# franciszzj/OpenPSG

Hardware: AMD Instinct MI355X
Metric: object-pairs/sec (relation-query + LMM decode), 1024² img × 50 masks (higher is better)
Workload: dtype fp32; 1 GPU; C3: 1024x1024, 50 masks, full path incl. LMM autoregressive relation decode (Llama-2-7B shape, top-20 pairs, 16 new tokens each, EOS suppressed); objects=50, pairs_per_image=2450, patches=256, llm_layers=32, mode=fp32s

## Files before the change

### include/psg_hip.h

```cpp
#ifndef PSG_HIP_H
#define PSG_HIP_H

#include <stdint.h>

#ifdef __cplusplus
extern "C" {
#endif

typedef struct psg_ctx psg_ctx;

enum psg_status {
  PSG_OK = 0,
  PSG_ERR_INVALID = -1,
  PSG_ERR_UNSUPPORTED = -2,
  PSG_ERR_HIP = -3,
  PSG_ERR_NO_DEVICE = -4
};

enum psg_dtype { PSG_F32 = 0, PSG_BF16 = 1, PSG_F16 = 2 };

enum psg_empty_policy { PSG_EMPTY_UNIFORM = 0, PSG_EMPTY_UNMASKED = 1 };

enum psg_xattn_variant { PSG_XATTN_MFMA = 0, PSG_XATTN_SIMPLE = 1, PSG_XATTN_MFMA_V1 = 2 };

#define PSG_ABI_VERSION 609
int psg_version(void);
const char* psg_last_error(void);
int psg_create(int device, psg_ctx** out);
int psg_destroy(psg_ctx* ctx);
int psg_device_info(psg_ctx* ctx, int* num_cu, char* arch, int arch_len);

int psg_set_option(psg_ctx* ctx, const char* name, int value);
int psg_get_option(psg_ctx* ctx, const char* name, int* value);

enum psg_trace_kind { PSG_TRACE_NONE = 0, PSG_TRACE_SKINNY_GEMM = 1, PSG_TRACE_CROSS_ATTN = 2, PSG_TRACE_DECODE_LAYER = 3 };
int psg_set_trace_buffer(psg_ctx* ctx, int kind, void* device_buffer, int64_t bytes);

int psg_patch_embed_workspace(psg_ctx*, int C, int Hf, int Wf, int Cout, int patch, int64_t* bytes);
int psg_patch_embed(psg_ctx*, const float* feat, int C, int Hf, int Wf, const float* weight,
                    const float* bias, int Cout, int patch, float* out, float* workspace,
                    int64_t workspace_bytes, void* stream);

int psg_mask_grid(psg_ctx*, const int32_t* pan, int H0, int W0, int img_h, int img_w,
                  int pad_h, int pad_w, int gh, int gw, float* grid, void* stream);

int psg_object_bitmasks(psg_ctx*, const float* grid, int L, const int32_t* object_ids, int N,
                        uint64_t* bits, int words, void* stream);

int psg_qformer_embed(psg_ctx*, const int32_t* ids, int B, int T, const float* word_emb,
                      const float* pos_emb, const float* query_rows, int nq, const float* ln_w,
                      const float* ln_b, float eps, int hidden, void* out, int dtype, void* stream);

int psg_add_layernorm(psg_ctx*, const void* x, const void* residual, const float* bias,
                      const float* gamma, const float* beta, float eps, int64_t rows, int hidden,
                      void* out, int dtype, void* stream);
int psg_add_layernorm_periodic(psg_ctx*, const void* x, const void* residual_table, int table_rows,
                               const float* bias, const float* gamma, const float* beta, float eps,
                               int64_t rows, int hidden, void* out, int dtype, void* stream);
int psg_add_layernorm_indexed(psg_ctx*, const void* x, const void* residual_table, const int32_t* block_index, int group,
                              const float* bias, const float* gamma, const float* beta, float eps, int64_t rows,
                              int hidden, void* out, int dtype, void* stream);
int psg_add_layernorm_res32(psg_ctx*, const void* x, const float* residual, int res_period, const int32_t* res_index,
                            const float* bias, const float* gamma, const float* beta, float eps, int64_t rows,
                            int hidden, void* out16, float* out32, int dtype, void* stream);

int psg_bias_gelu(psg_ctx*, const void* x, const float* bias, int64_t rows, int cols, void* out,
                  int dtype, void* stream);

int psg_qformer_self_attn(psg_ctx*, const void* qkv, const uint8_t* text_mask, int B, int T, int nq,
                          int heads, int query_rows_only, void* out, int dtype, void* stream);

int psg_qformer_self_attn_shared(psg_ctx*, const void* qkv_query, const void* qkv_text,
                                 const uint8_t* text_mask, int B, int T, int nq, int heads, void* out,
                                 int dtype, void* stream);
int psg_qformer_self_attn_cls(psg_ctx*, const void* q_cls, const void* kv, const uint8_t* text_mask, int B, int T,
                              int nq, int heads, void* out, int dtype, void* stream);
int psg_qformer_cls_attn_input(psg_ctx*, const void* x_query, const void* x_text, const int32_t* text_index,
                               const void* g, const uint8_t* text_mask, int B, int T, int nq, int heads, int hidden,
                               void* xbar, int dtype, void* stream);

int psg_qformer_cross_attn(psg_ctx*, const void* q, const void* k, const void* v,
                           const uint64_t* bits, int words, const int32_t* pair_index, int N, int P,
                           int L, int nq, int heads, int empty_policy, int variant, void* out,
                           int dtype, void* stream);
int psg_qformer_cross_attn_indexed(psg_ctx*, const void* q_u, const int32_t* q_index, const void* q_cls, const void* k,
                                   const void* v, const uint64_t* bits, int words, const int32_t* pair_index, int N, int P,
                                   int L, int heads, int empty_policy, void* out, int dtype, void* stream);

int psg_exist_head(psg_ctx*, const void* x, const float* w, const float* b, int P, int nq, int hidden,
                   float* logit, float* prob, int dtype, void* stream);

int psg_topk(psg_ctx*, const float* score, int n, int k, int32_t* out_idx, float* out_val, void* stream);

int psg_multiclass_head(psg_ctx*, const void* x, const float* w, const float* b, int P, int nq, int hidden, int R,
                        const int32_t* pair_index, int N, float* logit, float* prob, int dtype, void* stream);

int psg_topk_large_workspace(psg_ctx*, int n, int k, int64_t* bytes);
int psg_topk_large(psg_ctx*, const float* score, int n, int k, void* workspace, int64_t ws_bytes, int32_t* out_idx,
                   float* out_val, void* stream);

int psg_gather_rows(psg_ctx*, const void* src, int src_dtype, const int32_t* idx, int64_t n, int cols,
                    int64_t src_row_stride, void* dst, int dst_dtype, int64_t dst_row_stride, void* stream);
int psg_gather_pair_rows(psg_ctx*, const void* xq, const void* xt, const int32_t* text_index, const uint8_t* text_mask,
                         const int32_t* pair_index, const int32_t* sel, int K, int first, int count, int slot_off,
                         int nq, int T, int cols, void* out, uint8_t* mask_out, int32_t* pair_out, uint8_t* mine_out,
                         int dtype, void* stream);

int psg_rmsnorm(psg_ctx*, void* resid, const void* delta, int delta_splits, const float* w, float eps,
                int64_t rows, int hidden, void* out, int dtype, int resid_dtype, void* stream);

int psg_rope_kvwrite(psg_ctx*, const void* qkv, int qkv_splits, const int32_t* tok_pair, const int32_t* tok_pos,
                     const int32_t* rope_pos, const float* rope_cos, const float* rope_sin, int64_t rows, int heads,
                     int head_dim, int ctx, void* q_out, void* k_cache, void* v_cache, int dtype, void* stream);

int psg_llm_attn(psg_ctx*, const void* q, const void* k_cache, const void* v_cache,
                 const int32_t* tok_pair, const int32_t* tok_pos, int64_t rows, int heads,
                 int head_dim, int ctx, void* out, int dtype, void* stream);

int psg_prefill_attn(psg_ctx*, const void* q, const void* k_cache, const void* v_cache,
                     const int32_t* tok_pos, int pairs, int rows_per_pair, int heads, int head_dim,
                     int ctx, void* out, int dtype, void* stream);

int psg_prefill_attn_rope(psg_ctx*, const void* qkv, const int32_t* tok_pos, const float* rope_cos,
                          const float* rope_sin, int pairs, int rows_per_pair, int heads, int head_dim,
                          int ctx, void* k_cache, void* v_cache, void* out, int dtype, void* stream);

int psg_decode_attn(psg_ctx*, const void* qkv, int qkv_splits, const int32_t* tok_pair, const int32_t* tok_pos,
                    const float* rope_cos, const float* rope_sin, int rows, int heads, int head_dim, int ctx, void* k_cache,
                    void* v_cache, void* out, int dtype, void* stream);

int psg_rope_kvwrite_gqa(psg_ctx*, const void* qkv, int qkv_splits, const int32_t* tok_pair, const int32_t* tok_pos,
                         const int32_t* rope_pos, const float* rope_cos, const float* rope_sin, int64_t rows, int heads,
                         int kv_heads, int head_dim, int ctx, void* q_out, void* k_cache, void* v_cache, int dtype,
                         void* stream);
int psg_rope_kvwrite_scaled_gqa(psg_ctx*, const float* qkv, const float* row_scale, const float* col_scale,
                                const int32_t* tok_pair, const int32_t* tok_pos, const float* rope_cos,
                                const float* rope_sin, int slices, int64_t rows, int heads, int kv_heads, int head_dim,
                                int ctx, float* q_out, float* k_cache, float* v_cache, void* stream);
int psg_llm_attn_gqa(psg_ctx*, const void* q, const void* k_cache, const void* v_cache, const int32_t* tok_pair,
                     const int32_t* tok_pos, int64_t rows, int heads, int kv_heads, int head_dim, int ctx, void* out,
                     int dtype, void* stream);
int psg_prefill_attn_gqa(psg_ctx*, const void* q, const void* k_cache, const void* v_cache, const int32_t* tok_pos,
                         int pairs, int rows_per_pair, int heads, int kv_heads, int head_dim, int ctx, void* out, int dtype,
                         void* stream);
int psg_prefill_attn_rope_gqa(psg_ctx*, const void* qkv, const int32_t* tok_pos, const float* rope_cos,
                              const float* rope_sin, int pairs, int rows_per_pair, int heads, int kv_heads, int head_dim,
                              int ctx, void* k_cache, void* v_cache, void* out, int dtype, void* stream);
int psg_decode_attn_gqa(psg_ctx*, const void* qkv, int qkv_splits, const int32_t* tok_pair, const int32_t* tok_pos,
                        const float* rope_cos, const float* rope_sin, int rows, int heads, int kv_heads, int head_dim,
                        int ctx, void* k_cache, void* v_cache, void* out, int dtype, void* stream);

int psg_silu_mul(psg_ctx*, const void* gate_up, int splits, int64_t rows, int inter, void* out, int dtype,
                 void* stream);

int psg_skinny_gemm_plan(psg_ctx*, int M, int N, int K, int dtype, int* splits);
int psg_skinny_gemm(psg_ctx*, const void* x, const void* w, float* part, int M, int N, int K,
                    int splits, int dtype, void* stream);
int psg_reduce_partials(psg_ctx*, const float* part, int splits, int64_t n, void* y, int dtype,
                        void* stream);
int psg_split_f16x2(psg_ctx*, const float* x, int64_t rows, int K, int64_t row_stride, void* out2, float* inv_scale,
                    void* stream);
int psg_rmsnorm_split2(psg_ctx*, float* resid, const float* delta, int delta_splits, const float* w, float eps, int64_t rows,
                       int hidden, void* out2, float* inv_scale, void* stream);
int psg_split_gemm_w16_plan(psg_ctx*, int M, int N, int K, int mode, int* slots);
int psg_split_gemm_w16(psg_ctx*, const void* x2, const float* inv_scale, const void* w_f16, float* part, int M, int N, int K,
                       int slots, int mode, void* stream);
int psg_split_gemm_w8_plan(psg_ctx*, int M, int N, int K, int mode, int* slots);
int psg_split_gemm_w8(psg_ctx*, const void* x2, const float* inv_scale, const void* w8, const float* col_scale, float* part,
                      int M, int N, int K, int slots, int mode, void* stream);
int psg_skinny_gemm_w8_plan(psg_ctx*, int M, int N, int K, int dtype, int mode, int* slots);
int psg_skinny_gemm_w8(psg_ctx*, const void* x, const void* w8, const float* col_scale, float* part, int M, int N, int K,
                       int slots, int dtype, int mode, void* stream);
int psg_split_gemm_w4_plan(psg_ctx*, int M, int N, int K, int mode, int* slots);
int psg_split_gemm_w4(psg_ctx*, const void* x2, const float* inv_scale, const void* w4, const void* e_img, const float* col_scale,
                      float* part, int M, int N, int K, int slots, int mode, void* stream);
int psg_skinny_gemm_w4_plan(psg_ctx*, int M, int N, int K, int dtype, int mode, int* slots);
int psg_skinny_gemm_w4(psg_ctx*, const void* x, const void* w4, const void* e_img, const float* col_scale, float* part, int M,
                       int N, int K, int slots, int dtype, int mode, void* stream);
int psg_split_gemm_int4_plan(psg_ctx*, int M, int N, int K, int group, int mode, int* slots);
int psg_split_gemm_int4(psg_ctx*, const void* x2, const float* inv_scale, const void* q_img, const void* g_img, float* part,
                        int M, int N, int K, int group, int slots, int mode, void* stream);
int psg_skinny_gemm_int4_plan(psg_ctx*, int M, int N, int K, int group, int dtype, int mode, int* slots);
int psg_skinny_gemm_int4(psg_ctx*, const void* x, const void* q_img, const void* g_img, float* part, int M, int N, int K,
                         int group, int slots, int dtype, int mode, void* stream);
int psg_batch_gemm_w8_plan(psg_ctx*, int M, int N, int K, int dtype, int mode, int* slots);
int psg_batch_gemm_w8(psg_ctx*, const void* x, const void* w8, const float* col_scale, float* part, int M, int N, int K,
                      int slots, int dtype, int mode, void* stream);
int psg_batch_split_gemm_w8_plan(psg_ctx*, int M, int N, int K, int mode, int* slots);
int psg_batch_split_gemm_w8(psg_ctx*, const void* x2, const float* inv_scale, const void* w8, const float* col_scale,
                            float* part, int M, int N, int K, int slots, int mode, void* stream);
int psg_batch_gemm_w4_plan(psg_ctx*, int M, int N, int K, int dtype, int mode, int* slots);
int psg_batch_gemm_w4(psg_ctx*, const void* x, const void* w4, const void* e_img, const float* col_scale, float* part, int M,
                      int N, int K, int slots, int dtype, int mode, void* stream);
int psg_batch_split_gemm_w4_plan(psg_ctx*, int M, int N, int K, int mode, int* slots);
int psg_batch_split_gemm_w4(psg_ctx*, const void* x2, const float* inv_scale, const void* w4, const void* e_img,
                            const float* col_scale, float* part, int M, int N, int K, int slots, int mode, void* stream);
int psg_expand_w8(psg_ctx*, const void* q, const float* s, void* out, int N, int K, int out_dtype, void* stream);
int psg_expand_w4(psg_ctx*, const void* q, const void* e, const float* s, void* out, int N, int K, int out_dtype, void* stream);
int psg_skinny_gemm_w16(psg_ctx*, const float* x, const void* w_f16, float* part, int M, int N, int K, int splits,
                        void* stream);

int psg_batch_gemm_plan(psg_ctx*, int64_t M, int N, int K, int dtype, int slab_rows, int mode, int* slots);
int psg_batch_gemm(psg_ctx*, const void* x, const void* w, float* part, int64_t M, int N, int K, int slots, int dtype,
                   int slab_rows, int mode, void* stream);

enum psg_prologue_kind { PSG_PRO_NONE = 0, PSG_PRO_RMSNORM = 1, PSG_PRO_DECODE_ATTN = 2, PSG_PRO_SILU_MUL = 3 };
typedef struct psg_prologue {
  int kind;
  int in_splits;
  const void* in;
  void* resid;
  const float* norm_w;
  float eps;
  int heads;
  int ctx;
  const int32_t* tok_pair;
  const int32_t* tok_pos;
  const float* rope_cos;
  const float* rope_sin;
  void* k_cache;
  void* v_cache;
  uint32_t* sync;
} psg_prologue;
int psg_skinny_gemm_fused(psg_ctx*, const psg_prologue* pro, void* x, const void* w, float* part, int M, int N, int K,
                          int splits, int dtype, void* stream);

int psg_decode_layer_workspace(psg_ctx*, int M, int hidden, int inter, int64_t* floats, int64_t* counters);
int psg_decode_layer_supported(psg_ctx*, int M, int hidden, int inter, int heads, int dtype);
int psg_decode_layer(psg_ctx*, void* resid, const void* delta, int delta_splits, const float* ln1, const float* ln2,
                     const void* wqkv, const void* wo, const void* wgu, const void* wdown, const int32_t* tok_pair,
                     const int32_t* tok_pos, const float* rope_cos, const float* rope_sin, int M, int hidden, int inter,
                     int heads, int ctx_len, float eps, void* k_cache, void* v_cache, float* workspace, uint32_t* counters,
                     float* down_part, int dtype, void* stream);
int psg_decode_layers(psg_ctx*, void* resid, const void* delta, int delta_splits, const void* layer_table, int n_layers,
                      const int32_t* tok_pair, const int32_t* tok_pos, const float* rope_cos, const float* rope_sin, int M,
                      int hidden, int inter, int heads, int ctx_len, float eps, float* workspace, uint32_t* counters,
                      float* down_parts, int dtype, void* stream);

int psg_split_f16x3(psg_ctx*, const float* x, int64_t rows, int K, int64_t row_stride, int order, void* out,
                    float* inv_scale, void* stream);
int psg_scale_rows_cols(psg_ctx*, float* y, int64_t rows, int N, const float* row_scale, const float* col_scale,
                        void* stream);

int psg_rmsnorm_split(psg_ctx*, float* resid, const float* delta, const float* delta_row_scale, const float* delta_col_scale,
                      int delta_slices, const float* w, float eps, int64_t rows, int hidden, void* out, float* inv_scale,
                      int planes, void* stream);
int psg_rope_kvwrite_scaled(psg_ctx*, const float* qkv, const float* row_scale, const float* col_scale,
                            const int32_t* tok_pair, const int32_t* tok_pos, const float* rope_cos, const float* rope_sin,
                            int slices, int64_t rows, int heads, int head_dim, int ctx, float* q_out, float* k_cache,
                            float* v_cache, void* stream);
int psg_silu_mul_split(psg_ctx*, const float* gate_up, const float* row_scale, const float* col_scale, int slices, int64_t rows,
                       int inter, void* out, float* inv_scale, int planes, void* stream);

enum psg_epilogue { PSG_EPI_NONE = 0, PSG_EPI_GELU = 1, PSG_EPI_SWIGLU = 2 };
int psg_dense_gemm(psg_ctx*, const void* x, const void* w, const float* bias, int epilogue, void* out, int64_t M,
                   int N, int K, int dtype, void* stream);
int psg_dense_gemm_ex(psg_ctx*, const void* x, const void* w, const float* bias, int epilogue, void* out, int64_t M,
                      int N, int K, int dtype, int out_dtype, const float* row_scale, const float* col_scale,
                      void* stream);
enum psg_tile { PSG_TILE_AUTO = 0, PSG_TILE_256x256 = 1, PSG_TILE_256x192 = 2, PSG_TILE_256x128 = 3, PSG_TILE_256x64 = 4,
                PSG_TILE_128x128 = 5 };
int psg_dense_gemm_tiled(psg_ctx*, const void* x, const void* w, const float* bias, int epilogue, void* out, int64_t M,
                         int N, int K, int dtype, int out_dtype, const float* row_scale, const float* col_scale, int tile,
                         void* stream);
int psg_interleave_gate_up(psg_ctx*, const void* gate_up, void* out, int inter, int K, void* stream);
int psg_dense_gemm_split(psg_ctx*, const void* x2, const void* w2, const float* bias, int epilogue, float* out, int64_t M,
                         int N, int K2, const float* row_scale, const float* col_scale, int tile, void* stream);

int psg_greedy_step(psg_ctx*, const void* logits, int splits, int K, int vocab, int step, int max_new,
                    int eos, int suppress_token, int32_t* tokens, int32_t* done, int32_t* next_ids, int32_t* tok_pos,
                    const void* embed, int embed_dtype, int hidden, void* x_out, int x_dtype, int dtype, void* stream);

int psg_tree_attn(psg_ctx*, const void* q, const void* k_cache, const void* v_cache, const int32_t* row_pair,
                  const int32_t* row_node, const int32_t* prefix_len, const int32_t* anc, int n_int, int max_depth,
                  int trie_base, int64_t rows, int heads, int kv_heads, int pairs, int head_dim, int ctx, void* out,
                  int dtype, void* stream);
int psg_token_logprobs(psg_ctx*, const void* logits, int splits, int64_t rows, int vocab, const int32_t* row_node,
                       const int64_t* row_out, const int32_t* child_off, const int32_t* child_tok, int n_nodes,
                       int n_edges, float* out, int64_t out_len, int dtype, void* stream);

int psg_masked_mean_pool_workspace(psg_ctx*, int C, int Hf, int Wf, int N, int64_t* bytes);
int psg_masked_mean_pool(psg_ctx*, const float* feat, int C, int Hf, int Wf, const int32_t* pan, int H0,
                         int W0, int img_h, int img_w, int pad_h, int pad_w, const int32_t* object_ids,
                         int N, float* out, int32_t* workspace, int64_t workspace_bytes, void* stream);
int psg_masked_split_mean_pool(psg_ctx*, const float* feat, int C, int Hf, int Wf, const int32_t* pan, int H0,
                               int W0, int img_h, int img_w, int pad_h, int pad_w, const int32_t* object_ids, int N,
                               int output_size, float* out, int32_t* workspace, int64_t workspace_bytes, void* stream);

int psg_train_object_bitmasks(psg_ctx*, const uint8_t* thing_masks, int n_thing, const int32_t* sem, int H, int W,
                              const int32_t* is_thing, const int32_t* category, const int32_t* thing_index, int N,
                              int gh, int gw, uint64_t* bits, int words, void* stream);
int psg_bce_with_logits(psg_ctx*, const float* logit, const float* label, int n, float weight, float* out,
                        void* stream);
int psg_cross_entropy_rows(psg_ctx*, const void* logits, int64_t rows, int vocab, const int32_t* labels, float* loss,
                           int dtype, void* stream);

int psg_train_layernorm_fwd(psg_ctx*, const float* x, const float* gamma, const float* beta, float eps, int64_t rows,
                            int hidden, float* y, float* mean, float* rstd, void* stream);
int psg_train_layernorm_bwd(psg_ctx*, const float* x, const float* dy, const float* gamma, const float* mean,
                            const float* rstd, int64_t rows, int hidden, float* dx, float* dgamma, float* dbeta,
                            void* stream);
int psg_train_rmsnorm_fwd(psg_ctx*, const float* x, const float* w, float eps, int64_t rows, int hidden, float* y,
                          float* rstd, void* stream);
int psg_train_rmsnorm_bwd(psg_ctx*, const float* x, const float* dy, const float* w, const float* rstd, int64_t rows,
                          int hidden, float* dx, void* stream);
int psg_train_attn_fwd(psg_ctx*, const float* q, const float* k, const float* v, const uint8_t* keep, int B, int Bk,
                       int H, int Sq, int Sk, int D, int Mq, float scale, const uint8_t* drop, float drop_scale, float* p,
                       float* out, void* stream);
int psg_train_attn_bwd(psg_ctx*, const float* q, const float* k, const float* v, const float* p, const float* dout,
                       int B, int Bk, int H, int Sq, int Sk, int D, float scale, const uint8_t* drop, float drop_scale,
                       float* dq, float* dk, float* dv, void* stream);
int psg_train_gelu_fwd(psg_ctx*, const float* x, int64_t n, float* y, void* stream);
int psg_train_gelu_bwd(psg_ctx*, const float* x, const float* dy, int64_t n, float* dx, void* stream);
int psg_train_silu_mul_fwd(psg_ctx*, const float* gate_up, int64_t rows, int inter, float* y, void* stream);
int psg_train_silu_mul_bwd(psg_ctx*, const float* gate_up, const float* dy, int64_t rows, int inter, float* dgate_up,
                           void* stream);
int psg_train_rope(psg_ctx*, const float* x, const int32_t* pos, const float* rope_cos, const float* rope_sin,
                   int table_rows, int64_t rows, int heads, int head_dim, float sign, float* y, void* stream);
int psg_train_ce_bwd(psg_ctx*, const float* logits, int64_t rows, int vocab, const int32_t* labels, const float* dloss,
                     float* dlogits, void* stream);
int psg_train_bce_bwd(psg_ctx*, const float* logit, const float* label, int n, float weight, const float* dloss,
                      float* dlogit, void* stream);
int psg_train_mlcce_fwd(psg_ctx*, const float* logits, const float* labels, int rows, int R, float* loss, void* stream);
int psg_train_mlcce_bwd(psg_ctx*, const float* logits, const float* labels, int rows, int R, const float* dloss,
                        float* dlogits, void* stream);

int psg_train_bf16_layernorm_fwd(psg_ctx*, const float* x, const float* gamma, const float* beta, float eps, int64_t rows,
                                 int hidden, void* y, float* mean, float* rstd, void* stream);
int psg_train_bf16_layernorm_bwd(psg_ctx*, const float* x, const void* dy, const float* gamma, const float* mean,
                                 const float* rstd, int64_t rows, int hidden, float* dx, float* dgamma, float* dbeta,
                                 void* stream);
int psg_train_bf16_rmsnorm_fwd(psg_ctx*, const float* x, const float* w, float eps, int64_t rows, int hidden, void* y,
                               float* rstd, void* stream);
int psg_train_bf16_rmsnorm_bwd(psg_ctx*, const float* x, const void* dy, const float* w, const float* rstd, int64_t rows,
                               int hidden, float* dx, void* stream);
int psg_train_bf16_gelu_fwd(psg_ctx*, const void* x, int64_t n, void* y, void* stream);
int psg_train_bf16_gelu_bwd(psg_ctx*, const void* x, const void* dy, int64_t n, void* dx, void* stream);
int psg_train_bf16_silu_mul_fwd(psg_ctx*, const void* gate_up, int64_t rows, int inter, void* y, void* stream);
int psg_train_bf16_silu_mul_bwd(psg_ctx*, const void* gate_up, const void* dy, int64_t rows, int inter, void* dgate_up,
                                void* stream);
int psg_train_bf16_rope(psg_ctx*, const void* x, const int32_t* pos, const float* rope_cos, const float* rope_sin,
                        int table_rows, int64_t rows, int heads, int head_dim, float sign, void* y, void* stream);
int psg_train_bf16_attn_fwd(psg_ctx*, const void* q, const void* k, const void* v, const uint8_t* keep, int B, int Bk, int H,
                            int Sq, int Sk, int D, int Mq, float scale, const uint8_t* drop, float drop_scale, void* out,
                            float* lse, void* stream);
int psg_train_bf16_attn_bwd(psg_ctx*, const void* q, const void* k, const void* v, const uint8_t* keep, const void* dout,
                            const float* lse, int B, int Bk, int H, int Sq, int Sk, int D, int Mq, float scale,
                            const uint8_t* drop, float drop_scale, void* dq, void* dk, void* dv, float* delta, void* stream);

int psg_bilinear_scores(psg_ctx*, const float* sub, const float* obj, int B, int N, int R, int C, float* pred,
                        void* stream);

#ifdef __cplusplus
}
#endif
#endif
```

### openpsg_amd/_lib.py

```python
from __future__ import annotations

import ctypes as C
import os

_HERE = os.path.dirname(os.path.abspath(__file__))
LIB_PATH = os.path.join(_HERE, "libpsg_hip.so")

PSG_ABI_VERSION = 609
PSG_F32, PSG_BF16, PSG_F16 = 0, 1, 2
PSG_EMPTY_UNIFORM, PSG_EMPTY_UNMASKED = 0, 1
PSG_XATTN_MFMA, PSG_XATTN_SIMPLE, PSG_XATTN_MFMA_V1 = 0, 1, 2
PSG_TRACE_NONE, PSG_TRACE_SKINNY_GEMM, PSG_TRACE_CROSS_ATTN, PSG_TRACE_DECODE_LAYER = 0, 1, 2, 3


class PsgHipError(RuntimeError):
    pass


_vp, _i, _i64, _f = C.c_void_p, C.c_int, C.c_int64, C.c_float

PSG_PRO_NONE, PSG_PRO_RMSNORM, PSG_PRO_DECODE_ATTN, PSG_PRO_SILU_MUL = 0, 1, 2, 3


class Prologue(C.Structure):
    _fields_ = [("kind", _i), ("in_splits", _i), ("input", _vp), ("resid", _vp), ("norm_w", _vp), ("eps", _f),
                ("heads", _i), ("ctx", _i), ("tok_pair", _vp), ("tok_pos", _vp), ("rope_cos", _vp), ("rope_sin", _vp),
                ("k_cache", _vp), ("v_cache", _vp), ("sync", _vp)]

SIGNATURES = {
    "psg_version": [],
    "psg_create": [_i, C.POINTER(_vp)],
    "psg_destroy": [_vp],
    "psg_device_info": [_vp, C.POINTER(_i), C.c_char_p, _i],
    "psg_set_option": [_vp, C.c_char_p, _i],
    "psg_get_option": [_vp, C.c_char_p, C.POINTER(_i)],
    "psg_set_trace_buffer": [_vp, _i, _vp, _i64],
    "psg_patch_embed_workspace": [_vp, _i, _i, _i, _i, _i, C.POINTER(_i64)],
    "psg_patch_embed": [_vp, _vp, _i, _i, _i, _vp, _vp, _i, _i, _vp, _vp, _i64, _vp],
    "psg_mask_grid": [_vp, _vp, _i, _i, _i, _i, _i, _i, _i, _i, _vp, _vp],
    "psg_object_bitmasks": [_vp, _vp, _i, _vp, _i, _vp, _i, _vp],
    "psg_qformer_embed": [_vp, _vp, _i, _i, _vp, _vp, _vp, _i, _vp, _vp, _f, _i, _vp, _i, _vp],
    "psg_add_layernorm": [_vp, _vp, _vp, _vp, _vp, _vp, _f, _i64, _i, _vp, _i, _vp],
    "psg_add_layernorm_periodic": [_vp, _vp, _vp, _i, _vp, _vp, _vp, _f, _i64, _i, _vp, _i, _vp],
    "psg_add_layernorm_indexed": [_vp, _vp, _vp, _vp, _i, _vp, _vp, _vp, _f, _i64, _i, _vp, _i, _vp],
    "psg_add_layernorm_res32": [_vp, _vp, _vp, _i, _vp, _vp, _vp, _vp, _f, _i64, _i, _vp, _vp, _i, _vp],
    "psg_bias_gelu": [_vp, _vp, _vp, _i64, _i, _vp, _i, _vp],
    "psg_qformer_self_attn": [_vp, _vp, _vp, _i, _i, _i, _i, _i, _vp, _i, _vp],
    "psg_qformer_self_attn_cls": [_vp, _vp, _vp, _vp, _i, _i, _i, _i, _vp, _i, _vp],
    "psg_qformer_cls_attn_input": [_vp, _vp, _vp, _vp, _vp, _vp, _i, _i, _i, _i, _i, _vp, _i, _vp],
    "psg_qformer_self_attn_shared": [_vp, _vp, _vp, _vp, _i, _i, _i, _i, _vp, _i, _vp],
    "psg_qformer_cross_attn": [_vp, _vp, _vp, _vp, _vp, _i, _vp, _i, _i, _i, _i, _i, _i, _i, _vp, _i, _vp],
    "psg_exist_head": [_vp, _vp, _vp, _vp, _i, _i, _i, _vp, _vp, _i, _vp],
    "psg_topk": [_vp, _vp, _i, _i, _vp, _vp, _vp],
    "psg_multiclass_head": [_vp, _vp, _vp, _vp, _i, _i, _i, _i, _vp, _i, _vp, _vp, _i, _vp],
    "psg_topk_large_workspace": [_vp, _i, _i, C.POINTER(_i64)],
    "psg_topk_large": [_vp, _vp, _i, _i, _vp, _i64, _vp, _vp, _vp],
    "psg_gather_rows": [_vp, _vp, _i, _vp, _i64, _i, _i64, _vp, _i, _i64, _vp],
    "psg_gather_pair_rows": [_vp, _vp, _vp, _vp, _vp, _vp, _vp, _i, _i, _i, _i, _i, _i, _i, _vp, _vp, _vp, _vp, _i, _vp],
    "psg_rmsnorm": [_vp, _vp, _vp, _i, _vp, _f, _i64, _i, _vp, _i, _i, _vp],
    "psg_rope_kvwrite": [_vp, _vp, _i, _vp, _vp, _vp, _vp, _vp, _i64, _i, _i, _i, _vp, _vp, _vp, _i, _vp],
    "psg_train_object_bitmasks": [_vp, _vp, _i, _vp, _i, _i, _vp, _vp, _vp, _i, _i, _i, _vp, _i, _vp],
    "psg_bce_with_logits": [_vp, _vp, _vp, _i, _f, _vp, _vp],
    "psg_cross_entropy_rows": [_vp, _vp, _i64, _i, _vp, _vp, _i, _vp],
    "psg_llm_attn": [_vp, _vp, _vp, _vp, _vp, _vp, _i64, _i, _i, _i, _vp, _i, _vp],
    "psg_prefill_attn": [_vp, _vp, _vp, _vp, _vp, _i, _i, _i, _i, _i, _vp, _i, _vp],
    "psg_prefill_attn_rope": [_vp, _vp, _vp, _vp, _vp, _i, _i, _i, _i, _i, _vp, _vp, _vp, _i, _vp],
    "psg_decode_attn": [_vp, _vp, _i, _vp, _vp, _vp, _vp, _i, _i, _i, _i, _vp, _vp, _vp, _i, _vp],
    "psg_rope_kvwrite_gqa": [_vp, _vp, _i, _vp, _vp, _vp, _vp, _vp, _i64, _i, _i, _i, _i, _vp, _vp, _vp, _i, _vp],
    "psg_rope_kvwrite_scaled_gqa": [_vp, _vp, _vp, _vp, _vp, _vp, _vp, _vp, _i, _i64, _i, _i, _i, _i, _vp, _vp, _vp, _vp],
    "psg_llm_attn_gqa": [_vp, _vp, _vp, _vp, _vp, _vp, _i64, _i, _i, _i, _i, _vp, _i, _vp],
    "psg_prefill_attn_gqa": [_vp, _vp, _vp, _vp, _vp, _i, _i, _i, _i, _i, _i, _vp, _i, _vp],
    "psg_prefill_attn_rope_gqa": [_vp, _vp, _vp, _vp, _vp, _i, _i, _i, _i, _i, _i, _vp, _vp, _vp, _i, _vp],
    "psg_decode_attn_gqa": [_vp, _vp, _i, _vp, _vp, _vp, _vp, _i, _i, _i, _i, _i, _vp, _vp, _vp, _i, _vp],
    "psg_silu_mul": [_vp, _vp, _i, _i64, _i, _vp, _i, _vp],
    "psg_skinny_gemm_plan": [_vp, _i, _i, _i, _i, C.POINTER(_i)],
    "psg_skinny_gemm": [_vp, _vp, _vp, _vp, _i, _i, _i, _i, _i, _vp],
    "psg_batch_gemm_plan": [_vp, _i64, _i, _i, _i, _i, _i, C.POINTER(_i)],
    "psg_batch_gemm": [_vp, _vp, _vp, _vp, _i64, _i, _i, _i, _i, _i, _i, _vp],
    "psg_split_f16x2": [_vp, _vp, _i64, _i, _i64, _vp, _vp, _vp],
    "psg_rmsnorm_split2": [_vp, _vp, _vp, _i, _vp, _f, _i64, _i, _vp, _vp, _vp],
    "psg_split_gemm_w16_plan": [_vp, _i, _i, _i, _i, C.POINTER(_i)],
    "psg_split_gemm_w16": [_vp, _vp, _vp, _vp, _vp, _i, _i, _i, _i, _i, _vp],
    "psg_split_gemm_w8_plan": [_vp, _i, _i, _i, _i, C.POINTER(_i)],
    "psg_split_gemm_w8": [_vp, _vp, _vp, _vp, _vp, _vp, _i, _i, _i, _i, _i, _vp],
    "psg_skinny_gemm_w8_plan": [_vp, _i, _i, _i, _i, _i, C.POINTER(_i)],
    "psg_skinny_gemm_w8": [_vp, _vp, _vp, _vp, _vp, _i, _i, _i, _i, _i, _i, _vp],
    "psg_split_gemm_w4_plan": [_vp, _i, _i, _i, _i, C.POINTER(_i)],
    "psg_split_gemm_w4": [_vp, _vp, _vp, _vp, _vp, _vp, _vp, _i, _i, _i, _i, _i, _vp],
    "psg_skinny_gemm_w4_plan": [_vp, _i, _i, _i, _i, _i, C.POINTER(_i)],
    "psg_skinny_gemm_w4": [_vp, _vp, _vp, _vp, _vp, _vp, _i, _i, _i, _i, _i, _i, _vp],
    "psg_batch_gemm_w8_plan": [_vp, _i, _i, _i, _i, _i, C.POINTER(_i)],
    "psg_batch_gemm_w8": [_vp, _vp, _vp, _vp, _vp, _i, _i, _i, _i, _i, _i, _vp],
    "psg_batch_split_gemm_w8_plan": [_vp, _i, _i, _i, _i, C.POINTER(_i)],
    "psg_batch_split_gemm_w8": [_vp, _vp, _vp, _vp, _vp, _vp, _i, _i, _i, _i, _i, _vp],
    "psg_split_gemm_int4_plan": [_vp, _i, _i, _i, _i, _i, C.POINTER(_i)],
    "psg_split_gemm_int4": [_vp, _vp, _vp, _vp, _vp, _vp, _i, _i, _i, _i, _i, _i, _vp],
    "psg_skinny_gemm_int4_plan": [_vp, _i, _i, _i, _i, _i, _i, C.POINTER(_i)],
    "psg_skinny_gemm_int4": [_vp, _vp, _vp, _vp, _vp, _i, _i, _i, _i, _i, _i, _i, _vp],
    "psg_batch_gemm_w4_plan": [_vp, _i, _i, _i, _i, _i, C.POINTER(_i)],
    "psg_batch_gemm_w4": [_vp, _vp, _vp, _vp, _vp, _vp, _i, _i, _i, _i, _i, _i, _vp],
    "psg_batch_split_gemm_w4_plan": [_vp, _i, _i, _i, _i, C.POINTER(_i)],
    "psg_batch_split_gemm_w4": [_vp, _vp, _vp, _vp, _vp, _vp, _vp, _i, _i, _i, _i, _i, _vp],
    "psg_expand_w8": [_vp, _vp, _vp, _vp, _i, _i, _i, _vp],
    "psg_expand_w4": [_vp, _vp, _vp, _vp, _vp, _i, _i, _i, _vp],
    "psg_qformer_cross_attn_indexed": [_vp, _vp, _vp, _vp, _vp, _vp, _vp, _i, _vp, _i, _i, _i, _i, _i, _vp, _i, _vp],
    "psg_skinny_gemm_w16": [_vp, _vp, _vp, _vp, _i, _i, _i, _i, _vp],
    "psg_skinny_gemm_fused": [_vp, _vp, _vp, _vp, _vp, _i, _i, _i, _i, _i, _vp],
    "psg_rmsnorm_split": [_vp, _vp, _vp, _vp, _vp, _i, _vp, _f, _i64, _i, _vp, _vp, _i, _vp],
    "psg_rope_kvwrite_scaled": [_vp, _vp, _vp, _vp, _vp, _vp, _vp, _vp, _i, _i64, _i, _i, _i, _vp, _vp, _vp, _vp],
    "psg_silu_mul_split": [_vp, _vp, _vp, _vp, _i, _i64, _i, _vp, _vp, _i, _vp],
    "psg_decode_layer_workspace": [_vp, _i, _i, _i, C.POINTER(_i64), C.POINTER(_i64)],
    "psg_decode_layer_supported": [_vp, _i, _i, _i, _i, _i],
    "psg_decode_layers": [_vp, _vp, _vp, _i, _vp, _i, _vp, _vp, _vp, _vp, _i, _i, _i, _i, _i, _f, _vp, _vp, _vp, _i, _vp],
    "psg_decode_layer": [_vp, _vp, _vp, _i, _vp, _vp, _vp, _vp, _vp, _vp, _vp, _vp, _vp, _vp, _i, _i, _i, _i, _i, _f,
                         _vp, _vp, _vp, _vp, _vp, _i, _vp],
    "psg_reduce_partials": [_vp, _vp, _i, _i64, _vp, _i, _vp],
    "psg_masked_mean_pool_workspace": [_vp, _i, _i, _i, _i, C.POINTER(_i64)],
    "psg_masked_mean_pool": [_vp, _vp, _i, _i, _i, _vp, _i, _i, _i, _i, _i, _i, _vp, _i, _vp, _vp, _i64, _vp],
    "psg_masked_split_mean_pool": [_vp, _vp, _i, _i, _i, _vp, _i, _i, _i, _i, _i, _i, _vp, _i, _i, _vp, _vp, _i64, _vp],
    "psg_bilinear_scores": [_vp, _vp, _vp, _i, _i, _i, _i, _vp, _vp],
    "psg_dense_gemm": [_vp, _vp, _vp, _vp, _i, _vp, _i64, _i, _i, _i, _vp],
    "psg_dense_gemm_ex": [_vp, _vp, _vp, _vp, _i, _vp, _i64, _i, _i, _i, _i, _vp, _vp, _vp],
    "psg_dense_gemm_tiled": [_vp, _vp, _vp, _vp, _i, _vp, _i64, _i, _i, _i, _i, _vp, _vp, _i, _vp],
    "psg_interleave_gate_up": [_vp, _vp, _vp, _i, _i, _vp],
    "psg_dense_gemm_split": [_vp, _vp, _vp, _vp, _i, _vp, _i64, _i, _i, _vp, _vp, _i, _vp],
    "psg_train_layernorm_fwd": [_vp, _vp, _vp, _vp, _f, _i64, _i, _vp, _vp, _vp, _vp],
    "psg_train_layernorm_bwd": [_vp, _vp, _vp, _vp, _vp, _vp, _i64, _i, _vp, _vp, _vp, _vp],
    "psg_train_rmsnorm_fwd": [_vp, _vp, _vp, _f, _i64, _i, _vp, _vp, _vp],
    "psg_train_rmsnorm_bwd": [_vp, _vp, _vp, _vp, _vp, _i64, _i, _vp, _vp],
    "psg_split_f16x3": [_vp, _vp, _i64, _i, _i64, _i, _vp, _vp, _vp],
    "psg_scale_rows_cols": [_vp, _vp, _i64, _i, _vp, _vp, _vp],
    "psg_train_attn_fwd": [_vp, _vp, _vp, _vp, _vp, _i, _i, _i, _i, _i, _i, _i, _f, _vp, _f, _vp, _vp, _vp],
    "psg_train_attn_bwd": [_vp, _vp, _vp, _vp, _vp, _vp, _i, _i, _i, _i, _i, _i, _f, _vp, _f, _vp, _vp, _vp, _vp],
    "psg_train_gelu_fwd": [_vp, _vp, _i64, _vp, _vp],
    "psg_train_gelu_bwd": [_vp, _vp, _vp, _i64, _vp, _vp],
    "psg_train_silu_mul_fwd": [_vp, _vp, _i64, _i, _vp, _vp],
    "psg_train_silu_mul_bwd": [_vp, _vp, _vp, _i64, _i, _vp, _vp],
    "psg_train_rope": [_vp, _vp, _vp, _vp, _vp, _i, _i64, _i, _i, _f, _vp, _vp],
    "psg_train_ce_bwd": [_vp, _vp, _i64, _i, _vp, _vp, _vp, _vp],
    "psg_train_bce_bwd": [_vp, _vp, _vp, _i, _f, _vp, _vp, _vp],
    "psg_train_mlcce_fwd": [_vp, _vp, _vp, _i, _i, _vp, _vp],
    "psg_train_mlcce_bwd": [_vp, _vp, _vp, _i, _i, _vp, _vp, _vp],
    "psg_train_bf16_layernorm_fwd": [_vp, _vp, _vp, _vp, _f, _i64, _i, _vp, _vp, _vp, _vp],
    "psg_train_bf16_layernorm_bwd": [_vp, _vp, _vp, _vp, _vp, _vp, _i64, _i, _vp, _vp, _vp, _vp],
    "psg_train_bf16_rmsnorm_fwd": [_vp, _vp, _vp, _f, _i64, _i, _vp, _vp, _vp],
    "psg_train_bf16_rmsnorm_bwd": [_vp, _vp, _vp, _vp, _vp, _i64, _i, _vp, _vp],
    "psg_train_bf16_gelu_fwd": [_vp, _vp, _i64, _vp, _vp],
    "psg_train_bf16_gelu_bwd": [_vp, _vp, _vp, _i64, _vp, _vp],
    "psg_train_bf16_silu_mul_fwd": [_vp, _vp, _i64, _i, _vp, _vp],
    "psg_train_bf16_silu_mul_bwd": [_vp, _vp, _vp, _i64, _i, _vp, _vp],
    "psg_train_bf16_rope": [_vp, _vp, _vp, _vp, _vp, _i, _i64, _i, _i, _f, _vp, _vp],
    "psg_train_bf16_attn_fwd": [_vp, _vp, _vp, _vp, _vp, _i, _i, _i, _i, _i, _i, _i, _f, _vp, _f, _vp, _vp, _vp],
    "psg_train_bf16_attn_bwd": [_vp, _vp, _vp, _vp, _vp, _vp, _vp, _i, _i, _i, _i, _i, _i, _i, _f, _vp, _f, _vp, _vp, _vp,
                                _vp, _vp],
    "psg_greedy_step": [_vp, _vp, _i, _i, _i, _i, _i, _i, _i, _vp, _vp, _vp, _vp, _vp, _i, _i, _vp, _i, _i, _vp],
    "psg_tree_attn": [_vp, _vp, _vp, _vp, _vp, _vp, _vp, _vp, _i, _i, _i, _i64, _i, _i, _i, _i, _i, _vp, _i, _vp],
    "psg_token_logprobs": [_vp, _vp, _i, _i64, _i, _vp, _vp, _vp, _vp, _i, _i, _vp, _i64, _i, _vp],
}

_lib = None
_ctx = {}


def load():
    global _lib
    if _lib is not None:
        return _lib
    import torch
    if not os.path.exists(LIB_PATH):
        raise PsgHipError(
            f"{LIB_PATH} is missing: build it with `python -m openpsg_amd.csrc.build` "
            "(hipcc --offload-arch=gfx950). There is no CPU fallback for this path.")
    lib = C.CDLL(LIB_PATH)
    lib.psg_last_error.restype = C.c_char_p
    lib.psg_last_error.argtypes = []
    for name, argtypes in SIGNATURES.items():
        fn = getattr(lib, name, None)
        if fn is None:
            raise PsgHipError(f"{LIB_PATH} does not export {name}; rebuild the library")
        fn.restype = _i
        fn.argtypes = argtypes
    built = lib.psg_version()
    if built != PSG_ABI_VERSION:
        raise PsgHipError(f"{LIB_PATH} was built with ABI version {built}, this binding is written against "
                          f"{PSG_ABI_VERSION} (include/psg_hip.h): rebuild with `python -m openpsg_amd.csrc.build --force`")
    _lib = lib
    return lib


def last_error() -> str:
    return load().psg_last_error().decode("utf-8", "replace")


def check(rc: int, what: str):
    if rc != 0:
        raise PsgHipError(f"{what} failed (status {rc}): {last_error()}")


def ctx(device_index: int):
    if device_index not in _ctx:
        lib = load()
        h = _vp()
        check(lib.psg_create(int(device_index), C.byref(h)), "psg_create")
        _ctx[device_index] = h
    return _ctx[device_index]


def device_info(device_index: int):
    n = _i(0)
    buf = C.create_string_buffer(64)
    check(load().psg_device_info(ctx(device_index), C.byref(n), buf, 64), "psg_device_info")
    return n.value, buf.value.decode()


def set_option(device_index: int, name: str, value: int):
    check(load().psg_set_option(ctx(device_index), name.encode(), int(value)), f"psg_set_option({name})")


def get_option(device_index: int, name: str) -> int:
    v = _i(0)
    check(load().psg_get_option(ctx(device_index), name.encode(), C.byref(v)), f"psg_get_option({name})")
    return v.value


def set_trace_buffer(device_index: int, kind: int, tensor=None):
    if tensor is None or kind == PSG_TRACE_NONE:
        check(load().psg_set_trace_buffer(ctx(device_index), PSG_TRACE_NONE, None, 0), "psg_set_trace_buffer")
    else:
        check(load().psg_set_trace_buffer(ctx(device_index), int(kind), tensor.data_ptr(),
                                          tensor.numel() * tensor.element_size()), "psg_set_trace_buffer")
```

### openpsg_amd/csrc/build.py

```python
from __future__ import annotations

import argparse
import os
import subprocess
import sys

HERE = os.path.dirname(os.path.abspath(__file__))
PKG = os.path.dirname(HERE)
LIB = os.path.join(PKG, "libpsg_hip.so")
SOURCES = ["psg_core.hip", "psg_rowops.hip", "psg_attn.hip", "psg_attn_f32.hip", "psg_xattn_mfma.hip", "psg_xattn_dma.hip", "psg_gemm.hip", "psg_gemm_f32.hip", "psg_batch_gemm.hip", "psg_gemm_w8.hip", "psg_gemm_w4.hip", "psg_gemm_int4.hip", "psg_batch_gemm_q.hip", "psg_expand.hip", "psg_decode_layer.hip", "psg_split.hip", "psg_dense_gemm.hip", "psg_patch_embed.hip", "psg_selfattn_mfma.hip", "psg_prefill_attn_mfma.hip", "psg_pool.hip", "psg_train.hip", "psg_train_bwd.hip", "psg_train_bf16.hip", "psg_tree.hip"]
HEADERS = ["psg_common.h", "psg_wave.h", "psg_decode_math.h", "psg_train_rows.h", "psg_xattn_tile.h", os.path.join("..", "..", "include", "psg_hip.h")]


def _hipcc() -> str:
    for cand in (os.environ.get("HIPCC"), "/opt/rocm/bin/hipcc", "hipcc"):
        if cand and (os.path.isabs(cand) and os.path.exists(cand) or not os.path.isabs(cand)):
            return cand
    raise RuntimeError("hipcc not found")


def needs_build() -> bool:
    if not os.path.exists(LIB):
        return True
    t = os.path.getmtime(LIB)
    deps = [os.path.join(HERE, s) for s in SOURCES + HEADERS if os.path.exists(os.path.join(HERE, s))]
    return any(os.path.getmtime(d) > t for d in deps)


def build(force: bool = False, save_temps: bool = False, verbose: bool = True) -> str:
    if not force and not needs_build():
        return LIB
    from concurrent.futures import ThreadPoolExecutor
    obj_dir = os.path.join(HERE, "_obj")
    os.makedirs(obj_dir, exist_ok=True)
    flags = ["--offload-arch=gfx950", "-O3", "-std=c++17", "-fPIC", "-fno-gpu-rdc", "-Wno-unused-result"]
    if save_temps:
        os.makedirs(os.path.join(HERE, "_temps"), exist_ok=True)
        flags += ["-save-temps=obj", "-Rpass-analysis=kernel-resource-usage"]
    hdr_t = max(os.path.getmtime(os.path.join(HERE, h)) for h in HEADERS)
    jobs, objs = [], []
    for s in SOURCES:
        src = os.path.join(HERE, s)
        if not os.path.exists(src):
            continue
        obj = os.path.join(obj_dir, os.path.splitext(s)[0] + ".o")
        objs.append(obj)
        if force or save_temps or not os.path.exists(obj) or os.path.getmtime(obj) < max(os.path.getmtime(src), hdr_t):
            jobs.append([_hipcc()] + flags + ["-c", src, "-o", obj])

    def run(cmd):
        if verbose:
            print(" ".join(cmd), flush=True)
        subprocess.run(cmd, check=True, cwd=HERE)
    with ThreadPoolExecutor(max_workers=min(8, max(1, (os.cpu_count() or 2) - 1))) as ex:
        list(ex.map(run, jobs))
    run([_hipcc(), "--offload-arch=gfx950", "-shared", "-fPIC", "-fno-gpu-rdc", "-o", LIB] + objs)
    return LIB


if __name__ == "__main__":
    ap = argparse.ArgumentParser()
    ap.add_argument("--force", action="store_true")
    ap.add_argument("--save-temps", action="store_true")
    a = ap.parse_args()
    print(build(force=a.force, save_temps=a.save_temps))
```

### openpsg_amd/csrc/psg_core.hip

```cpp
#include <ctype.h>
#include <stdarg.h>
#include <stdlib.h>

#include "psg_common.h"

static thread_local char g_err[512] = "";

void psg_set_error(const char* fmt, ...) {
  va_list ap;
  va_start(ap, fmt);
  vsnprintf(g_err, sizeof(g_err), fmt, ap);
  va_end(ap);
}

extern "C" const char* psg_last_error(void) { return g_err; }
extern "C" int psg_version(void) { return PSG_ABI_VERSION; }

struct OptName {
  const char* name;
  int psg_opts::*field;
};
static const OptName kOpts[] = {
    {"skinny_splits", &psg_opts::skinny_splits},       {"skinny_balance", &psg_opts::skinny_balance},
    {"skinny_wg_per_cu", &psg_opts::skinny_wg_per_cu}, {"skinny_dma", &psg_opts::skinny_dma},
    {"skinny_nt", &psg_opts::skinny_nt},               {"skinny_xdma", &psg_opts::skinny_xdma},
    {"skinny_wide", &psg_opts::skinny_wide},           {"skinny_f32_slots", &psg_opts::skinny_f32_slots},
    {"skinny_f32_waves", &psg_opts::skinny_f32_waves}, {"decode_persistent", &psg_opts::decode_persistent},
    {"llm_fuse_split", &psg_opts::llm_fuse_split},
    {"split_i2", &psg_opts::split_i2},
    {"qformer_split_cls_input_space", &psg_opts::qformer_split_cls_input_space},
    {"wt_stores", &psg_opts::wt_stores},
    {"selfattn_scalar", &psg_opts::selfattn_scalar},   {"decode_attn_1wave", &psg_opts::decode_attn_1wave},
    {"xattn_dma", &psg_opts::xattn_dma},               {"xattn_waves", &psg_opts::xattn_waves},
    {"dense_gemm_var", &psg_opts::dense_gemm_var},     {"qformer_own_gemm", &psg_opts::qformer_own_gemm},
    {"ln_half_wave", &psg_opts::ln_half_wave},         {"xattn_poll", &psg_opts::xattn_poll},
    {"xattn_wt", &psg_opts::xattn_wt},
    {"xattn_dynamic", &psg_opts::xattn_dynamic},
    {"llm_w16", &psg_opts::llm_w16},                   {"decode_gqa_qparts", &psg_opts::decode_gqa_qparts},
    {"batch_gemm_bn", &psg_opts::batch_gemm_bn},       {"decode_batch_gemm", &psg_opts::decode_batch_gemm},
    {"batch_gemm_var", &psg_opts::batch_gemm_var},     {"batch_gemm_mode", &psg_opts::batch_gemm_mode},
    {"batch_gemm_grid", &psg_opts::batch_gemm_grid},
    {"qformer_share_qkv", &psg_opts::qformer_share_qkv},
    {"qformer_cls_input_space", &psg_opts::qformer_cls_input_space},
    {"qformer_dedup_prompts", &psg_opts::qformer_dedup_prompts},
    {"llm_fuse_rmsnorm", &psg_opts::llm_fuse_rmsnorm}, {"prefill_attn_scalar", &psg_opts::prefill_attn_scalar},
};

static int parse_opt(const char* name, const char* text) {
  int a = 0, b = 0, c = 3;
  if (!strcmp(name, "skinny_dma") && sscanf(text, "%dx%dx%d", &a, &b, &c) >= 2) return a * 100 + b * 10 + c;
  return atoi(text);
}

extern "C" int psg_set_option(psg_ctx* ctx, const char* name, int value) {
  PSG_REQUIRE(ctx && name, PSG_ERR_INVALID, "psg_set_option: NULL argument");
  for (const OptName& o : kOpts)
    if (!strcmp(o.name, name)) {
      ctx->opt.*(o.field) = value;
      return PSG_OK;
    }
  psg_set_error("psg_set_option: unknown option '%s'", name);
  return PSG_ERR_INVALID;
}

extern "C" int psg_get_option(psg_ctx* ctx, const char* name, int* value) {
  PSG_REQUIRE(ctx && name && value, PSG_ERR_INVALID, "psg_get_option: NULL argument");
  for (const OptName& o : kOpts)
    if (!strcmp(o.name, name)) {
      *value = ctx->opt.*(o.field);
      return PSG_OK;
    }
  psg_set_error("psg_get_option: unknown option '%s'", name);
  return PSG_ERR_INVALID;
}

extern "C" int psg_set_trace_buffer(psg_ctx* ctx, int kind, void* device_buffer, int64_t bytes) {
  PSG_REQUIRE(ctx, PSG_ERR_INVALID, "psg_set_trace_buffer: ctx is NULL");
  PSG_REQUIRE(kind == PSG_TRACE_NONE || (device_buffer && bytes >= 8), PSG_ERR_INVALID,
              "psg_set_trace_buffer: kind=%d needs a device buffer", kind);
  ctx->trace_kind = kind;
  ctx->trace = kind == PSG_TRACE_NONE ? nullptr : (long long*)device_buffer;
  ctx->trace_words = kind == PSG_TRACE_NONE ? 0 : bytes / 8;
  return PSG_OK;
}

extern "C" int psg_create(int device, psg_ctx** out) {
  PSG_REQUIRE(out != nullptr, PSG_ERR_INVALID, "psg_create: out is NULL");
  int n = 0;
  hipError_t e = hipGetDeviceCount(&n);
  if (e != hipSuccess || n <= 0) {
    psg_set_error("psg_create: no HIP device visible (%s)", e == hipSuccess ? "count=0" : hipGetErrorString(e));
    return PSG_ERR_NO_DEVICE;
  }
  PSG_REQUIRE(device >= 0 && device < n, PSG_ERR_INVALID, "psg_create: device %d out of range [0,%d)", device, n);
  hipDeviceProp_t prop;
  e = hipGetDeviceProperties(&prop, device);
  if (e != hipSuccess) {
    psg_set_error("psg_create: hipGetDeviceProperties: %s", hipGetErrorString(e));
    return PSG_ERR_HIP;
  }
  psg_ctx* c = new psg_ctx();
  for (const OptName& o : kOpts) {
    std::string env = "PSG_";
    for (const char* q = o.name; *q; ++q) env += (char)toupper(*q);
    if (const char* e = getenv(env.c_str())) c->opt.*(o.field) = parse_opt(o.name, e);
  }
  c->device = device;
  c->num_cu = prop.multiProcessorCount;
  strncpy(c->arch, prop.gcnArchName, sizeof(c->arch) - 1);
  c->arch[sizeof(c->arch) - 1] = 0;
  *out = c;
  return PSG_OK;
}

extern "C" int psg_destroy(psg_ctx* ctx) {
  delete ctx;
  return PSG_OK;
}

extern "C" int psg_device_info(psg_ctx* ctx, int* num_cu, char* arch, int arch_len) {
  PSG_REQUIRE(ctx != nullptr, PSG_ERR_INVALID, "psg_device_info: ctx is NULL");
  if (num_cu) *num_cu = ctx->num_cu;
  if (arch && arch_len > 0) {
    strncpy(arch, ctx->arch, arch_len - 1);
    arch[arch_len - 1] = 0;
  }
  return PSG_OK;
}

__global__ void mask_grid_kernel(const int32_t* __restrict__ pan, int H0, int W0, int img_h, int img_w,
                                 int pad_h, int pad_w, int gh, int gw, float* __restrict__ grid) {
  int idx = blockIdx.x * blockDim.x + threadIdx.x;
  if (idx >= gh * gw) return;
  int r = idx / gw, c = idx % gw;
  const float sy2 = (float)pad_h / (float)gh, sx2 = (float)pad_w / (float)gw;
  const float sy1 = (float)H0 / (float)img_h, sx1 = (float)W0 / (float)img_w;
  int y1 = min((int)floorf((float)r * sy2), pad_h - 1);
  int x1 = min((int)floorf((float)c * sx2), pad_w - 1);
  float v = 0.0f;
  if (y1 < img_h && x1 < img_w) {
    int y0 = min((int)floorf((float)y1 * sy1), H0 - 1);
    int x0 = min((int)floorf((float)x1 * sx1), W0 - 1);
    v = (float)pan[(int64_t)y0 * W0 + x0];
  }
  grid[idx] = v;
}

extern "C" int psg_mask_grid(psg_ctx* ctx, const int32_t* pan, int H0, int W0, int img_h, int img_w, int pad_h,
                             int pad_w, int gh, int gw, float* grid, void* stream) {
  PSG_REQUIRE(ctx && pan && grid, PSG_ERR_INVALID, "psg_mask_grid: NULL argument");
  PSG_REQUIRE(H0 > 0 && W0 > 0 && img_h > 0 && img_w > 0 && pad_h >= img_h && pad_w >= img_w && gh > 0 && gw > 0,
              PSG_ERR_INVALID, "psg_mask_grid: bad shapes ori %dx%d img %dx%d pad %dx%d grid %dx%d", H0, W0, img_h,
              img_w, pad_h, pad_w, gh, gw);
  int n = gh * gw;
  mask_grid_kernel<<<(n + 255) / 256, 256, 0, (hipStream_t)stream>>>(pan, H0, W0, img_h, img_w, pad_h, pad_w, gh, gw,
                                                                     grid);
  PSG_CHECK_LAUNCH("psg_mask_grid");
  return PSG_OK;
}

__global__ void object_bitmasks_kernel(const float* __restrict__ grid, int L, const int32_t* __restrict__ ids, int N,
                                       uint64_t* __restrict__ bits, int words) {
  int wave = (blockIdx.x * blockDim.x + threadIdx.x) >> 6;
  int lane = threadIdx.x & 63;
  if (wave >= N * words) return;
  int n = wave / words, w = wave % words;
  int l = w * 64 + lane;
  bool hit = (l < L) && (grid[l] == (float)ids[n]);
  unsigned long long m = __ballot(hit);
  if (lane == 0) bits[(int64_t)n * words + w] = (uint64_t)m;
}

extern "C" int psg_object_bitmasks(psg_ctx* ctx, const float* grid, int L, const int32_t* object_ids, int N,
                                   uint64_t* bits, int words, void* stream) {
  PSG_REQUIRE(ctx && grid && object_ids && bits, PSG_ERR_INVALID, "psg_object_bitmasks: NULL argument");
  PSG_REQUIRE(L > 0 && N > 0 && words * 64 >= L, PSG_ERR_INVALID, "psg_object_bitmasks: L=%d N=%d words=%d", L, N,
              words);
  int waves = N * words;
  int blocks = (waves + 3) / 4;
  object_bitmasks_kernel<<<blocks, 256, 0, (hipStream_t)stream>>>(grid, L, object_ids, N, bits, words);
  PSG_CHECK_LAUNCH("psg_object_bitmasks");
  return PSG_OK;
}

__device__ __forceinline__ bool topk_better(float a, int ia, float b, int ib) {
  return (a > b) || (a == b && ia < ib);
}

__global__ void __launch_bounds__(1024) topk_kernel(const float* __restrict__ score, int n, int k,
                                                    int32_t* __restrict__ out_idx, float* __restrict__ out_val) {
  __shared__ float s_val[16];
  __shared__ int s_idx[16];
  __shared__ float prev_val;
  __shared__ int prev_idx;
  const int tid = threadIdx.x, lane = tid & 63, wid = tid >> 6;
  if (tid == 0) {
    prev_val = INFINITY;
    prev_idx = -1;
  }
  __syncthreads();
  for (int round = 0; round < k; ++round) {
    const float pv = prev_val;
    const int pi = prev_idx;
    float best = -INFINITY;
    int bi = 0x7fffffff;
    for (int i = tid; i < n; i += blockDim.x) {
      float v = score[i];
      if (v != v) v = -INFINITY;
      bool after = (v < pv) || (v == pv && i > pi);
      if (after && topk_better(v, i, best, bi)) {
        best = v;
        bi = i;
      }
    }
#pragma unroll
    for (int o = 32; o > 0; o >>= 1) {
      float ov = __shfl_xor(best, o, 64);
      int oi = __shfl_xor(bi, o, 64);
      if (topk_better(ov, oi, best, bi)) {
        best = ov;
        bi = oi;
      }
    }
    if (lane == 0) {
// ... 331 lines not shown
```

### openpsg_amd/csrc/psg_dense_gemm.hip

```cpp
#include "psg_common.h"
#include "psg_wave.h"

#define DG_BK 64

__device__ __forceinline__ float dg_gelu(float v) {
  const float x = v * 0.70710678118654752440f;
  const float ax = fabsf(x);
  const float t = __builtin_amdgcn_rcpf(fmaf(0.3275911f, ax, 1.0f));
  float poly = fmaf(1.061405429f, t, -1.453152027f);
  poly = fmaf(poly, t, 1.421413741f);
  poly = fmaf(poly, t, -0.284496736f);
  poly = fmaf(poly, t, 0.254829592f);
  const float e = __builtin_amdgcn_exp2f(-1.4426950408889634f * ax * ax);
  const float erf_abs = fmaf(-poly * t, e, 1.0f);
  return 0.5f * v * (1.0f + copysignf(erf_abs, x));
}

template <typename E, int EPI, int VAR, int OUT32, int WM, int WN, int TI, int TJ, int SPL = 0>
__global__ void __launch_bounds__(WM * WN * 64, (WM * WN >= 8 ? 2 : 1))
dense_gemm_kernel(const uint16_t* __restrict__ x, const uint16_t* __restrict__ w, const float* __restrict__ bias,
                  uint16_t* __restrict__ out, int M, int N, int K, const float* __restrict__ row_scale,
                  const float* __restrict__ col_scale) {
  using v8 = typename E::v8;
  constexpr int NW = WM * WN, BM = WM * TI * 32, BN = WN * TJ * 32;
  constexpr int A_BYTES = BM * 128, BUF_BYTES = (BM + BN) * 128;
  constexpr int AI = BM / 8 / NW, BI = BN / 8 / NW;
  static_assert(BM % (8 * NW) == 0 && BN % (8 * NW) == 0, "tile rows must split into 8-row DMA instructions per wave");
  constexpr bool GELU = EPI == PSG_EPI_GELU, SWIGLU = EPI == PSG_EPI_SWIGLU;
  static_assert(!(SWIGLU && OUT32), "the SwiGLU epilogue writes the 16-bit activation");
  extern __shared__ __attribute__((aligned(16))) unsigned char smem[];
  const int tid = threadIdx.x, lane = tid & 63;
  const int wid = __builtin_amdgcn_readfirstlane(tid >> 6);
  const uint32_t smem_lds = (uint32_t)(uintptr_t)(__attribute__((address_space(3))) unsigned char*)smem;
  const int NB = (N + BN - 1) / BN, MB = (M + BM - 1) / BM;
  const int MB8 = (MB + 7) / 8 * 8, NB8 = (NB + 7) / 8 * 8;
  const int ntile = MB >= 8 ? MB8 * NB : MB * NB8;
  const int wm = wid / WN, wn = wid % WN;
  auto tile_mn = [&](int t, int& mb, int& nb) {
    const int xcd = t & 7, idx = t >> 3;
    if (MB < 8) {
      mb = idx % MB;
      nb = (idx / MB) * 8 + xcd;
      return;
    }
    mb = (idx / NB) * 8 + xcd;
    nb = idx % NB;
  };

  const int srow = lane >> 3, sslot = lane & 7;
  auto stage_x = [&](int m0, int kt, int buf) {
    unsigned char* ab = smem + buf * BUF_BYTES;
#pragma unroll
    for (int i = 0; i < AI; ++i) {
      const int r = (wid * AI + i) * 8 + srow;
      const int piece = sslot ^ ((r >> 1) & 7);
      int gr = m0 + r;
      gr = gr < M ? gr : M - 1;
      __builtin_amdgcn_global_load_lds(
          (const __attribute__((address_space(1))) void*)(x + (int64_t)gr * K + kt * DG_BK + piece * 8),
          (__attribute__((address_space(3))) void*)(ab + (wid * AI + i) * 1024), 16, 0, 0);
    }
  };
  auto stage_w = [&](int n0, int kt, int buf) {
    unsigned char* ab = smem + buf * BUF_BYTES + A_BYTES;
#pragma unroll
    for (int i = 0; i < BI; ++i) {
      const int r = (wid * BI + i) * 8 + srow;
      const int piece = sslot ^ ((r >> 1) & 7);
      int gr = n0 + r;
      gr = gr < N ? gr : N - 1;
      __builtin_amdgcn_global_load_lds(
          (const __attribute__((address_space(1))) void*)(w + (int64_t)gr * K + kt * DG_BK + piece * 8),
          (__attribute__((address_space(3))) void*)(ab + (wid * BI + i) * 1024), 16, 0, 0);
    }
  };

  const int l31 = lane & 31, hi = lane >> 5;
  const int nk = K / DG_BK;
  int t = blockIdx.x, mb, nb;
  for (;; t += gridDim.x) {
    if (t >= ntile) return;
    tile_mn(t, mb, nb);
    if (mb < MB && nb < NB) break;
  }
  int par = 0;
  stage_x(mb * BM, 0, 0);
  stage_w(nb * BN, 0, 0);
  uint32_t arow[TI], brow[TJ], aswz[TI], bswz[TJ];
#pragma unroll
  for (int i = 0; i < TI; ++i) {
    const int r = wm * (TI * 32) + i * 32 + l31;
    arow[i] = (uint32_t)(r * 128);
    aswz[i] = (uint32_t)((r >> 1) & 7);
  }
#pragma unroll
  for (int j = 0; j < TJ; ++j) {
    const int r = wn * (TJ * 32) + j * 32 + l31;
    brow[j] = (uint32_t)(A_BYTES + r * 128);
    bswz[j] = (uint32_t)((r >> 1) & 7);
  }
  union Frag {
    psg_u32x4 u;
    v8 v;
  };
  for (;;) {
    const int m0 = mb * BM, n0 = nb * BN;
    int tn = t + gridDim.x, mbn = 0, nbn = 0;
    for (; tn < ntile; tn += gridDim.x) {
      tile_mn(tn, mbn, nbn);
      if (mbn < MB && nbn < NB) break;
    }
    const bool has_next = tn < ntile;

    psg_f32x16 acc[TI][TJ];
#pragma unroll
    for (int i = 0; i < TI; ++i)
#pragma unroll
      for (int j = 0; j < TJ; ++j) acc[i][j] = (psg_f32x16){0};

    for (int kt = 0; kt < nk; ++kt) {
      const int buf = par;
      par ^= 1;
      const bool more_k = kt + 1 < nk;
      const bool pf = VAR != 2 && (more_k || has_next);
      const int pm0 = more_k ? m0 : mbn * BM, pn0 = more_k ? n0 : nbn * BN, pkt = more_k ? kt + 1 : 0;
      psg_vmwait<0>();
      psg_lds_barrier();
      const uint32_t base = smem_lds + (uint32_t)(buf * BUF_BYTES);
      Frag af[2][TI], bf[2][TJ];
      auto read_frags = [&](int sub, Frag (&a_)[TI], Frag (&b_)[TJ]) {
        const uint32_t piece = (uint32_t)(2 * sub + hi);
#pragma unroll
        for (int j = 0; j < TJ; ++j) b_[j].u = psg_lds_read128(base + brow[j] + ((piece ^ bswz[j]) << 4));
#pragma unroll
        for (int i = 0; i < TI; ++i) a_[i].u = psg_lds_read128(base + arow[i] + ((piece ^ aswz[i]) << 4));
      };
#define DG_MMA(AF, BF)                                                                            \
  _Pragma("unroll") for (int i = 0; i < TI; ++i) _Pragma("unroll") for (int j = 0; j < TJ; ++j) {  \
    if (VAR == 1) {                                                                               \
      asm volatile("" ::"v"(BF[j].u), "v"(AF[i].u));                                              \
    } else {                                                                                      \
      acc[i][j] = E::mfma32(BF[j].v, AF[i].v, acc[i][j]);          \
    }                                                                                             \
  }
      if constexpr (SPL) {
        Frag bl[2][TJ];
        auto read_a = [&](int sub, Frag (&a_)[TI]) {
          const uint32_t piece = (uint32_t)(2 * sub + hi);
#pragma unroll
          for (int i = 0; i < TI; ++i) a_[i].u = psg_lds_read128(base + arow[i] + ((piece ^ aswz[i]) << 4));
        };
        auto read_b = [&](int sub, Frag (&b_)[TJ]) {
          const uint32_t piece = (uint32_t)(2 * sub + hi);
#pragma unroll
          for (int j = 0; j < TJ; ++j) b_[j].u = psg_lds_read128(base + brow[j] + ((piece ^ bswz[j]) << 4));
        };
        read_frags(0, af[0], bf[0]);
        read_frags(1, af[1], bf[1]);
        if (pf) stage_x(pm0, pkt, buf ^ 1);
        psg_lgkmwait<TI + TJ>();
        __builtin_amdgcn_sched_barrier(0);
        __builtin_amdgcn_s_setprio(1);
        DG_MMA(af[0], bf[0])
        __builtin_amdgcn_sched_barrier(0);
        read_b(2, bl[0]);
        if (pf) stage_w(pn0, pkt, buf ^ 1);
        psg_lgkmwait<TJ>();
        __builtin_amdgcn_sched_barrier(0);
        DG_MMA(af[1], bf[1])
        __builtin_amdgcn_sched_barrier(0);
        read_b(3, bl[1]);
        psg_lgkmwait<TJ>();
        __builtin_amdgcn_sched_barrier(0);
        DG_MMA(af[0], bl[0])
        __builtin_amdgcn_sched_barrier(0);
        read_a(2, af[0]);
        psg_lgkmwait<TI>();
        __builtin_amdgcn_sched_barrier(0);
        DG_MMA(af[1], bl[1])
        __builtin_amdgcn_sched_barrier(0);
        read_a(3, af[1]);
        psg_lgkmwait<TI>();
        __builtin_amdgcn_sched_barrier(0);
        DG_MMA(af[0], bf[0])
        psg_lgkmwait<0>();
        __builtin_amdgcn_sched_barrier(0);
        DG_MMA(af[1], bf[1])
        __builtin_amdgcn_s_setprio(0);
      } else {
      read_frags(0, af[0], bf[0]);
      read_frags(1, af[1], bf[1]);
      if (pf) stage_x(pm0, pkt, buf ^ 1);
      psg_lgkmwait<TI + TJ>();
      __builtin_amdgcn_sched_barrier(0);
      __builtin_amdgcn_s_setprio(1);
      DG_MMA(af[0], bf[0])
      __builtin_amdgcn_sched_barrier(0);
      read_frags(2, af[0], bf[0]);
      if (pf) stage_w(pn0, pkt, buf ^ 1);
      psg_lgkmwait<TI + TJ>();
      __builtin_amdgcn_sched_barrier(0);
      DG_MMA(af[1], bf[1])
      __builtin_amdgcn_sched_barrier(0);
      read_frags(3, af[1], bf[1]);
      psg_lgkmwait<TI + TJ>();
      __builtin_amdgcn_sched_barrier(0);
      DG_MMA(af[0], bf[0])
      psg_lgkmwait<0>();
      __builtin_amdgcn_sched_barrier(0);
      DG_MMA(af[1], bf[1])
      __builtin_amdgcn_s_setprio(0);
      }
#undef DG_MMA
    }

    const int cw = n0 + wn * (TJ * 32);
    if constexpr (SWIGLU) {
      const int No = N >> 1;
#pragma unroll
      for (int i = 0; i < TI; ++i) {
        const int m = m0 + wm * (TI * 32) + i * 32 + l31;
#pragma unroll
        for (int j = 0; j < TJ; ++j) {
          uint32_t pk[2][2];
#pragma unroll
          for (int p = 0; p < 2; ++p) {
            uint16_t h[4];
#pragma unroll
            for (int e = 0; e < 4; ++e) {
              const float g = E::to_f32(E::from_f32(acc[i][j][8 * p + e]));
              const float u = E::to_f32(E::from_f32(acc[i][j][8 * p + 4 + e]));
              const float sg = E::to_f32(E::from_f32(g / (1.0f + expf(-g))));
              h[e] = E::from_f32(sg * u);
            }
            pk[p][0] = (uint32_t)h[0] | ((uint32_t)h[1] << 16);
            pk[p][1] = (uint32_t)h[2] | ((uint32_t)h[3] << 16);
          }
          auto r0 = __builtin_amdgcn_permlane32_swap(pk[0][0], pk[1][0], false, false);
          auto r1 = __builtin_amdgcn_permlane32_swap(pk[0][1], pk[1][1], false, false);
          const int nin = cw + j * 32 + 16 * hi;
          if (m < M && nin + 16 <= N)
            *reinterpret_cast<uint4*>(out + (int64_t)m * No + (nin >> 1)) = make_uint4(r0[0], r1[0], r0[1], r1[1]);
        }
      }
    } else {
    float4 bv[TJ][4];
#pragma unroll
    for (int j = 0; j < TJ; ++j)
#pragma unroll
      for (int q = 0; q < 4; ++q) {
        const int n = cw + j * 32 + 8 * q + 4 * hi;
        bv[j][q] = (bias && n + 4 <= N) ? *reinterpret_cast<const float4*>(bias + n) : make_float4(0.f, 0.f, 0.f, 0.f);
      }
    if constexpr (OUT32) {
      float* out32 = reinterpret_cast<float*>(out);
      float4 cs[TJ][4];
#pragma unroll
      for (int j = 0; j < TJ; ++j)
#pragma unroll
        for (int q = 0; q < 4; ++q) {
          const int n = cw + j * 32 + 8 * q + 4 * hi;
          cs[j][q] = (col_scale && n + 4 <= N) ? *reinterpret_cast<const float4*>(col_scale + n)
                                               : make_float4(1.f, 1.f, 1.f, 1.f);
        }
#pragma unroll
      for (int i = 0; i < TI; ++i) {
        const int m = m0 + wm * (TI * 32) + i * 32 + l31;
        const float rs = (row_scale && m < M) ? row_scale[m] : 1.f;
#pragma unroll
        for (int j = 0; j < TJ; ++j)
#pragma unroll
          for (int q = 0; q < 4; ++q) {
            float v[4] = {acc[i][j][4 * q] * (rs * cs[j][q].x) + bv[j][q].x, acc[i][j][4 * q + 1] * (rs * cs[j][q].y) + bv[j][q].y,
                          acc[i][j][4 * q + 2] * (rs * cs[j][q].z) + bv[j][q].z, acc[i][j][4 * q + 3] * (rs * cs[j][q].w) + bv[j][q].w};
            if (GELU) {
#pragma unroll
              for (int e = 0; e < 4; ++e) v[e] = dg_gelu(v[e]);
            }
            const int n = cw + j * 32 + 8 * q + 4 * hi;
            if (m < M && n + 4 <= N)
              *reinterpret_cast<float4*>(out32 + (int64_t)m * N + n) = make_float4(v[0], v[1], v[2], v[3]);
          }
      }
    } else {
#pragma unroll
    for (int i = 0; i < TI; ++i) {
      const int m = m0 + wm * (TI * 32) + i * 32 + l31;
#pragma unroll
      for (int j = 0; j < TJ; ++j) {
        uint32_t pk[4][2];
#pragma unroll
        for (int q = 0; q < 4; ++q) {
          float v[4] = {acc[i][j][4 * q] + bv[j][q].x, acc[i][j][4 * q + 1] + bv[j][q].y,
                        acc[i][j][4 * q + 2] + bv[j][q].z, acc[i][j][4 * q + 3] + bv[j][q].w};
          if (GELU) {
#pragma unroll
            for (int e = 0; e < 4; ++e) v[e] = dg_gelu(v[e]);
          }
          pk[q][0] = (uint32_t)E::from_f32(v[0]) | ((uint32_t)E::from_f32(v[1]) << 16);
          pk[q][1] = (uint32_t)E::from_f32(v[2]) | ((uint32_t)E::from_f32(v[3]) << 16);
        }
#pragma unroll
        for (int q2 = 0; q2 < 2; ++q2) {
          uint32_t a0 = pk[2 * q2][0], a1 = pk[2 * q2][1], b0 = pk[2 * q2 + 1][0], b1 = pk[2 * q2 + 1][1];
          auto r0 = __builtin_amdgcn_permlane32_swap(a0, b0, false, false);
          auto r1 = __builtin_amdgcn_permlane32_swap(a1, b1, false, false);
          const int n = cw + j * 32 + 16 * q2 + 8 * hi;
          if (m < M && n + 8 <= N)
            *reinterpret_cast<uint4*>(out + (int64_t)m * N + n) = make_uint4(r0[0], r1[0], r0[1], r1[1]);
        }
      }
    }
    }
    }
    if (!has_next) return;
    t = tn;
    mb = mbn;
    nb = nbn;
  }
}

struct dg_geom {
  int id, wm, wn, ti, tj;
};
static const dg_geom DG_GEOMS[] = {
    {PSG_TILE_256x256, 2, 4, 4, 2}, {PSG_TILE_256x192, 4, 2, 2, 3}, {PSG_TILE_256x128, 4, 2, 2, 2},
    {PSG_TILE_256x64, 8, 1, 1, 2},  {PSG_TILE_128x128, 2, 2, 2, 2},
};

template <typename E, int EPI, int VAR, int OUT32, int WM, int WN, int TI, int TJ, int SPL = 0>
static int dg_launch(psg_ctx* ctx, const void* x, const void* w, const float* bias, void* out, int64_t M, int N, int K,
                     const float* row_scale, const float* col_scale, void* stream) {
  constexpr int BM = WM * TI * 32, BN = WN * TJ * 32;
  const int NB = (N + BN - 1) / BN, MB = (int)((M + BM - 1) / BM);
  const int ntile = MB >= 8 ? (MB + 7) / 8 * 8 * NB : MB * ((NB + 7) / 8 * 8);
  int grid_i = ctx->num_cu / 8 * 8;
  if (grid_i > ntile) grid_i = ntile;
  const size_t lds = 2 * (size_t)(BM + BN) * 128;
  auto k = dense_gemm_kernel<E, EPI, VAR, OUT32, WM, WN, TI, TJ, SPL>;
  hipError_t e = hipFuncSetAttribute((const void*)k, hipFuncAttributeMaxDynamicSharedMemorySize, (int)lds);
  if (e != hipSuccess) {
    psg_set_error("psg_dense_gemm: hipFuncSetAttribute: %s", hipGetErrorString(e));
    return PSG_ERR_HIP;
  }
  k<<<(unsigned)grid_i, WM * WN * 64, lds, (hipStream_t)stream>>>((const uint16_t*)x, (const uint16_t*)w, bias,
                                                                   (uint16_t*)out, (int)M, N, K, row_scale, col_scale);
  PSG_CHECK_LAUNCH("psg_dense_gemm");
  return PSG_OK;
}

static int dg_auto_tile(const psg_ctx* ctx, int64_t M, int N, bool o32 = false) {
  int best = PSG_TILE_256x256;
  double best_cost = 1e300;
  const int cus = ctx->num_cu / 8 * 8;
  for (const dg_geom& g : DG_GEOMS) {
    if (g.id == PSG_TILE_128x128) continue;
    if (o32 && g.id == PSG_TILE_256x192) continue;
    const int BM = g.wm * g.ti * 32, BN = g.wn * g.tj * 32;
    const int64_t tiles = ((M + BM - 1) / BM) * ((N + BN - 1) / BN);
    const int64_t rounds = (tiles + cus - 1) / cus;
    const double pen = BN >= 256 ? 1.0 : BN >= 192 ? 1.04 : BN >= 128 ? 1.1 : 1.5;
    const double cost = (double)rounds * BM * BN * pen;
    if (cost < best_cost * 0.999) {
      best_cost = cost;
      best = g.id;
    }
  }
  return best;
}

extern "C" int psg_dense_gemm_tiled(psg_ctx* ctx, const void* x, const void* w, const float* bias, int epilogue,
                                    void* out, int64_t M, int N, int K, int dtype, int out_dtype, const float* row_scale,
                                    const float* col_scale, int tile, void* stream);
extern "C" int psg_dense_gemm_ex(psg_ctx* ctx, const void* x, const void* w, const float* bias, int epilogue, void* out,
                                 int64_t M, int N, int K, int dtype, int out_dtype, const float* row_scale,
                                 const float* col_scale, void* stream) {
  return psg_dense_gemm_tiled(ctx, x, w, bias, epilogue, out, M, N, K, dtype, out_dtype, row_scale, col_scale,
                              PSG_TILE_256x256, stream);
}
extern "C" int psg_dense_gemm(psg_ctx* ctx, const void* x, const void* w, const float* bias, int epilogue, void* out,
                              int64_t M, int N, int K, int dtype, void* stream) {
  return psg_dense_gemm_tiled(ctx, x, w, bias, epilogue, out, M, N, K, dtype, dtype, nullptr, nullptr,
                              PSG_TILE_256x256, stream);
}

extern "C" int psg_dense_gemm_tiled(psg_ctx* ctx, const void* x, const void* w, const float* bias, int epilogue,
                                    void* out, int64_t M, int N, int K, int dtype, int out_dtype, const float* row_scale,
                                    const float* col_scale, int tile, void* stream) {
  PSG_REQUIRE(ctx && x && w && out, PSG_ERR_INVALID, "psg_dense_gemm: NULL argument");
  PSG_REQUIRE(out_dtype == dtype || out_dtype == PSG_F32, PSG_ERR_UNSUPPORTED,
              "psg_dense_gemm: output dtype %d (the operand dtype %d or fp32)", out_dtype, dtype);
  PSG_REQUIRE(out_dtype == PSG_F32 || (!row_scale && !col_scale), PSG_ERR_UNSUPPORTED,
              "psg_dense_gemm: row / column scales need the fp32 output");
  PSG_REQUIRE(M >= 0 && N > 0 && K > 0 && M < (1ll << 31), PSG_ERR_INVALID, "psg_dense_gemm: M=%lld N=%d K=%d",
              (long long)M, N, K);
  PSG_REQUIRE(N % 16 == 0 && K % DG_BK == 0, PSG_ERR_UNSUPPORTED,
              "psg_dense_gemm: N=%d must be a multiple of 16 and K=%d of %d", N, K, DG_BK);
  PSG_REQUIRE(epilogue == PSG_EPI_NONE || epilogue == PSG_EPI_GELU || epilogue == PSG_EPI_SWIGLU, PSG_ERR_INVALID,
              "psg_dense_gemm: epilogue=%d", epilogue);
  PSG_REQUIRE(epilogue != PSG_EPI_SWIGLU || (out_dtype == dtype && !bias), PSG_ERR_UNSUPPORTED,
              "psg_dense_gemm: the SwiGLU epilogue takes no bias and writes the operand dtype");
  if (M == 0) return PSG_OK;
  if (tile == PSG_TILE_AUTO) tile = dg_auto_tile(ctx, M, N, out_dtype == PSG_F32 && dtype != PSG_F32);
  const int var = ctx->opt.dense_gemm_var;
  const bool o32 = out_dtype == PSG_F32 && dtype != PSG_F32;
  PSG_REQUIRE(tile == PSG_TILE_256x256 || var == 0, PSG_ERR_UNSUPPORTED, "psg_dense_gemm: ablation builds exist for the 256 x 256 tile");
  PSG_REQUIRE(tile == PSG_TILE_256x256 || epilogue != PSG_EPI_GELU || o32, PSG_ERR_UNSUPPORTED,
              "psg_dense_gemm: tile %d with the GELU epilogue is built for the fp32 output (the split products)", tile);
  PSG_REQUIRE(!(o32 && tile == PSG_TILE_256x192), PSG_ERR_UNSUPPORTED, "psg_dense_gemm: the 256 x 192 tile has no fp32 output");
#define DGL(EPI, V, O, WM, WN, TI, TJ) \
  return dg_launch<E, EPI, V, O, WM, WN, TI, TJ>(ctx, x, w, bias, out, M, N, K, row_scale, col_scale, stream)
#define DG_TILE(WM, WN, TI, TJ)                                                        \
  PSG_DISPATCH_E16(dtype, "psg_dense_gemm", if (epilogue == PSG_EPI_SWIGLU) DGL(PSG_EPI_SWIGLU, 0, 0, WM, WN, TI, TJ); \
                   else DGL(PSG_EPI_NONE, 0, 0, WM, WN, TI, TJ))
#define DG_TILE32(WM, WN, TI, TJ)                                                      \
  PSG_DISPATCH_E16(dtype, "psg_dense_gemm", if (epilogue == PSG_EPI_GELU) DGL(PSG_EPI_GELU, 0, 1, WM, WN, TI, TJ); \
                   else DGL(PSG_EPI_NONE, 0, 1, WM, WN, TI, TJ))
  switch (tile) {
    case PSG_TILE_256x256:
      if (o32) {
        PSG_REQUIRE(epilogue != PSG_EPI_SWIGLU, PSG_ERR_UNSUPPORTED, "psg_dense_gemm: SwiGLU with fp32 output");
        PSG_DISPATCH_E16(dtype, "psg_dense_gemm",
                         if (epilogue == PSG_EPI_GELU) DGL(PSG_EPI_GELU, 0, 1, 2, 4, 4, 2); else DGL(PSG_EPI_NONE, 0, 1, 2, 4, 4, 2));
      } else {
        PSG_DISPATCH_E16(dtype, "psg_dense_gemm",
                         if (var == 1) DGL(PSG_EPI_NONE, 1, 0, 2, 4, 4, 2); else if (var == 2) DGL(PSG_EPI_NONE, 2, 0, 2, 4, 4, 2);
                         else if (epilogue == PSG_EPI_GELU) DGL(PSG_EPI_GELU, 0, 0, 2, 4, 4, 2);
                         else if (epilogue == PSG_EPI_SWIGLU) DGL(PSG_EPI_SWIGLU, 0, 0, 2, 4, 4, 2);
                         else DGL(PSG_EPI_NONE, 0, 0, 2, 4, 4, 2));
      }
      break;
    case PSG_TILE_256x192: DG_TILE(4, 2, 2, 3); break;
    case PSG_TILE_256x128:
      if (o32) { PSG_REQUIRE(epilogue != PSG_EPI_SWIGLU, PSG_ERR_UNSUPPORTED, "psg_dense_gemm: SwiGLU with fp32 output"); DG_TILE32(4, 2, 2, 2); }
      else DG_TILE(4, 2, 2, 2);
      break;
    case PSG_TILE_256x64:
      if (o32) { PSG_REQUIRE(epilogue != PSG_EPI_SWIGLU, PSG_ERR_UNSUPPORTED, "psg_dense_gemm: SwiGLU with fp32 output"); DG_TILE32(8, 1, 1, 2); }
      else DG_TILE(8, 1, 1, 2);
      break;
    case PSG_TILE_128x128:
      if (o32) { PSG_REQUIRE(epilogue != PSG_EPI_SWIGLU, PSG_ERR_UNSUPPORTED, "psg_dense_gemm: SwiGLU with fp32 output"); DG_TILE32(2, 2, 2, 2); }
      else DG_TILE(2, 2, 2, 2);
      break;
    default: break;
  }
#undef DG_TILE
#undef DG_TILE32
#undef DGL
  psg_set_error("psg_dense_gemm: unknown tile %d", tile);
  return PSG_ERR_INVALID;
}

extern "C" int psg_dense_gemm_split(psg_ctx* ctx, const void* x2, const void* w2, const float* bias, int epilogue, float* out,
                                    int64_t M, int N, int K2, const float* row_scale, const float* col_scale, int tile,
                                    void* stream) {
  PSG_REQUIRE(ctx && x2 && w2 && out && row_scale && col_scale, PSG_ERR_INVALID, "psg_dense_gemm_split: NULL argument");
  PSG_REQUIRE(M >= 0 && N > 0 && K2 > 0 && M < (1ll << 31), PSG_ERR_INVALID, "psg_dense_gemm_split: M=%lld N=%d K2=%d",
              (long long)M, N, K2);
  PSG_REQUIRE(N % 16 == 0 && K2 % DG_BK == 0, PSG_ERR_UNSUPPORTED,
              "psg_dense_gemm_split: N=%d must be a multiple of 16 and K2=%d (= 2 K) of %d", N, K2, DG_BK);
  PSG_REQUIRE(epilogue == PSG_EPI_NONE || epilogue == PSG_EPI_GELU, PSG_ERR_INVALID, "psg_dense_gemm_split: epilogue=%d",
              epilogue);
  if (M == 0) return PSG_OK;
  if (tile == PSG_TILE_AUTO) tile = dg_auto_tile(ctx, M, N, true);
  const void* x = x2;
  const void* w = w2;
  const int K = K2;
#define DGS(WM, WN, TI, TJ)                                                                                              \
  do {                                                                                                                   \
    if (epilogue == PSG_EPI_GELU)                                                                                        \
      return dg_launch<EF16, PSG_EPI_GELU, 0, 1, WM, WN, TI, TJ, 1>(ctx, x, w, bias, out, M, N, K, row_scale, col_scale, stream); \
    return dg_launch<EF16, PSG_EPI_NONE, 0, 1, WM, WN, TI, TJ, 1>(ctx, x, w, bias, out, M, N, K, row_scale, col_scale, stream);   \
  } while (0)
  switch (tile) {
    case PSG_TILE_256x256: DGS(2, 4, 4, 2);
    case PSG_TILE_256x128: DGS(4, 2, 2, 2);
    case PSG_TILE_256x64: DGS(8, 1, 1, 2);
    case PSG_TILE_128x128: DGS(2, 2, 2, 2);
    default: break;
  }
#undef DGS
  psg_set_error("psg_dense_gemm_split: tile %d (256x256, 256x128, 256x64, 128x128 or auto)", tile);
  return PSG_ERR_INVALID;
}

__global__ void __launch_bounds__(256) interleave_gate_up_kernel(const uint16_t* __restrict__ gu, uint16_t* __restrict__ out,
                                                                 int inter, int K) {
  const int orow = blockIdx.x;
  const int p = orow >> 4, r = orow & 15;
  const int srow = r < 8 ? 8 * p + r : inter + 8 * p + (r - 8);
  const uint4* s = reinterpret_cast<const uint4*>(gu + (int64_t)srow * K);
  uint4* d = reinterpret_cast<uint4*>(out + (int64_t)orow * K);
  for (int c = threadIdx.x; c < K / 8; c += 256) d[c] = s[c];
}

extern "C" int psg_interleave_gate_up(psg_ctx* ctx, const void* gate_up, void* out, int inter, int K, void* stream) {
  PSG_REQUIRE(ctx && gate_up && out, PSG_ERR_INVALID, "psg_interleave_gate_up: NULL argument");
  PSG_REQUIRE(inter > 0 && inter % 8 == 0 && K > 0 && K % 8 == 0, PSG_ERR_UNSUPPORTED,
              "psg_interleave_gate_up: inter=%d and K=%d must be multiples of 8", inter, K);
  interleave_gate_up_kernel<<<2 * inter, 256, 0, (hipStream_t)stream>>>((const uint16_t*)gate_up, (uint16_t*)out, inter, K);
  PSG_CHECK_LAUNCH("psg_interleave_gate_up");
  return PSG_OK;
}
```

### openpsg_amd/csrc/psg_rowops.hip

```cpp
#include <type_traits>

#include "psg_common.h"
#include "psg_decode_math.h"

template <int NCH>
__device__ __forceinline__ void ln_row(float (&v)[NCH][4], int hidden, float eps, const float* __restrict__ gamma,
                                       const float* __restrict__ beta, int lane) {
  float s = 0.f;
#pragma unroll
  for (int c = 0; c < NCH; ++c) s += (v[c][0] + v[c][1]) + (v[c][2] + v[c][3]);
  const float mean = wave_sum(s) / (float)hidden;
  float q = 0.f;
#pragma unroll
  for (int c = 0; c < NCH; ++c)
#pragma unroll
    for (int e = 0; e < 4; ++e) {
      float d = v[c][e] - mean;
      q += d * d;
    }
  const float rstd = 1.0f / sqrtf(wave_sum(q) / (float)hidden + eps);
#pragma unroll
  for (int c = 0; c < NCH; ++c) {
    const int col = c * 256 + lane * 4;
    const float4 g = *reinterpret_cast<const float4*>(gamma + col);
    const float4 b = *reinterpret_cast<const float4*>(beta + col);
    v[c][0] = (v[c][0] - mean) * rstd * g.x + b.x;
    v[c][1] = (v[c][1] - mean) * rstd * g.y + b.y;
    v[c][2] = (v[c][2] - mean) * rstd * g.z + b.z;
    v[c][3] = (v[c][3] - mean) * rstd * g.w + b.w;
  }
}

template <typename T, int NCH>
__global__ void qformer_embed_kernel(const int32_t* __restrict__ ids, int B, int Tt, const float* __restrict__ word,
                                     const float* __restrict__ pos, const float* __restrict__ query, int nq,
                                     const float* __restrict__ gamma, const float* __restrict__ beta, float eps,
                                     int hidden, T* __restrict__ out) {
  const int64_t row = ((int64_t)blockIdx.x * blockDim.x + threadIdx.x) >> 6;
  const int lane = threadIdx.x & 63;
  const int64_t nqrows = (int64_t)B * nq;
  if (row >= nqrows + (int64_t)B * Tt) return;
  float v[NCH][4];
  if (row < nqrows) {
    const int r = (int)(row % nq);
#pragma unroll
    for (int c = 0; c < NCH; ++c) Act<float>::ld4(query, (int64_t)r * hidden + c * 256 + lane * 4, v[c]);
  } else {
    const int64_t tr = row - nqrows;
    const int t = (int)(tr % Tt);
    const int id = ids[tr];
#pragma unroll
    for (int c = 0; c < NCH; ++c) {
      float a[4], b[4];
      Act<float>::ld4(word, (int64_t)id * hidden + c * 256 + lane * 4, a);
      Act<float>::ld4(pos, (int64_t)t * hidden + c * 256 + lane * 4, b);
#pragma unroll
      for (int e = 0; e < 4; ++e) v[c][e] = a[e] + b[e];
    }
  }
  ln_row<NCH>(v, hidden, eps, gamma, beta, lane);
#pragma unroll
  for (int c = 0; c < NCH; ++c) Act<T>::st4(out, row * hidden + c * 256 + lane * 4, v[c]);
}

extern "C" int psg_qformer_embed(psg_ctx* ctx, const int32_t* ids, int B, int T_, const float* word_emb,
                                 const float* pos_emb, const float* query_rows, int nq, const float* ln_w,
                                 const float* ln_b, float eps, int hidden, void* out, int dtype, void* stream) {
  PSG_REQUIRE(ctx && word_emb && pos_emb && query_rows && ln_w && ln_b && out && (ids || T_ == 0), PSG_ERR_INVALID,
              "psg_qformer_embed: NULL argument");
  PSG_REQUIRE(hidden == 768, PSG_ERR_UNSUPPORTED, "psg_qformer_embed: hidden=%d (kernel is built for 768)", hidden);
  PSG_REQUIRE(B > 0 && T_ >= 0 && nq >= 0 && nq + T_ > 0, PSG_ERR_INVALID, "psg_qformer_embed: B=%d T=%d nq=%d", B, T_,
              nq);
  int64_t rows = (int64_t)B * (nq + T_);
  dim3 grid((unsigned)((rows + 3) / 4));
  PSG_DISPATCH_DTYPE(dtype, "psg_qformer_embed",
                     (qformer_embed_kernel<T, 3><<<grid, 256, 0, (hipStream_t)stream>>>(
                         ids, B, T_, word_emb, pos_emb, query_rows, nq, ln_w, ln_b, eps, hidden, (T*)out)));
  PSG_CHECK_LAUNCH("psg_qformer_embed");
  return PSG_OK;
}

template <typename T, int NCH>
__global__ void add_layernorm_kernel(const T* __restrict__ x, const T* __restrict__ res, const float* __restrict__ bias,
                                     const float* __restrict__ gamma, const float* __restrict__ beta, float eps,
                                     int64_t rows, int hidden, T* __restrict__ out, int res_period,
                                     const int32_t* __restrict__ res_index) {
  const int64_t row = ((int64_t)blockIdx.x * blockDim.x + threadIdx.x) >> 6;
  const int lane = threadIdx.x & 63;
  if (row >= rows) return;
  int64_t rrow = res_period > 0 ? row % res_period : row;
  if (res_index) rrow += (int64_t)res_index[row / res_period] * res_period;
  float v[NCH][4];
#pragma unroll
  for (int c = 0; c < NCH; ++c) {
    const int col = c * 256 + lane * 4;
    Act<T>::ld4(x, row * hidden + col, v[c]);
    if (bias) {
      const float4 b = *reinterpret_cast<const float4*>(bias + col);
      v[c][0] += b.x; v[c][1] += b.y; v[c][2] += b.z; v[c][3] += b.w;
    }
    if (res) {
      float r[4];
      Act<T>::ld4(res, rrow * hidden + col, r);
#pragma unroll
      for (int e = 0; e < 4; ++e) v[c][e] += r[e];
    }
  }
  ln_row<NCH>(v, hidden, eps, gamma, beta, lane);
#pragma unroll
  for (int c = 0; c < NCH; ++c) Act<T>::st4(out, row * hidden + c * 256 + lane * 4, v[c]);
}

template <typename E>
__global__ void __launch_bounds__(256) add_layernorm16_kernel(const uint16_t* __restrict__ x, const uint16_t* __restrict__ res,
                                                              const float* __restrict__ bias, const float* __restrict__ gamma,
                                                              const float* __restrict__ beta, float eps, int64_t rows,
                                                              uint16_t* __restrict__ out, int res_period,
                                                              const int32_t* __restrict__ res_index) {
  constexpr int H = 768;
  const int lane = threadIdx.x & 63, hl = lane & 31;
  int64_t row = ((((int64_t)blockIdx.x * blockDim.x + threadIdx.x) >> 6) << 1) + (lane >> 5);
  const bool live = row < rows;
  if (!live) row = rows - 1;
  int64_t rrow = res_period > 0 ? row % res_period : row;
  if (res_index) rrow += (int64_t)res_index[row / res_period] * res_period;
  float v[3][8];
  uint4 xw[3], rw[3];
#pragma unroll
  for (int c = 0; c < 3; ++c) {
    const int col = (c * 32 + hl) * 8;
    xw[c] = *reinterpret_cast<const uint4*>(x + row * H + col);
    if (res) rw[c] = *reinterpret_cast<const uint4*>(res + rrow * H + col);
  }
  auto unpack = [](const uint4& w, float (&f)[8]) {
    const uint32_t u[4] = {w.x, w.y, w.z, w.w};
#pragma unroll
    for (int i = 0; i < 4; ++i) {
      f[2 * i] = E::to_f32((uint16_t)(u[i] & 0xffffu));
      f[2 * i + 1] = E::to_f32((uint16_t)(u[i] >> 16));
    }
  };
  float s = 0.f;
#pragma unroll
  for (int c = 0; c < 3; ++c) {
    const int col = (c * 32 + hl) * 8;
    unpack(xw[c], v[c]);
    if (bias) {
      const float4 b0 = *reinterpret_cast<const float4*>(bias + col), b1 = *reinterpret_cast<const float4*>(bias + col + 4);
      v[c][0] += b0.x; v[c][1] += b0.y; v[c][2] += b0.z; v[c][3] += b0.w;
      v[c][4] += b1.x; v[c][5] += b1.y; v[c][6] += b1.z; v[c][7] += b1.w;
    }
    if (res) {
      float r[8];
      unpack(rw[c], r);
#pragma unroll
      for (int e = 0; e < 8; ++e) v[c][e] += r[e];
    }
#pragma unroll
    for (int e = 0; e < 8; ++e) s += v[c][e];
  }
  auto half_sum = [&](float t) {
    t += psg_dpp<0x111, 0xf>(0.f, t);
    t += psg_dpp<0x112, 0xf>(0.f, t);
    t += psg_dpp<0x114, 0xf>(0.f, t);
    t += psg_dpp<0x118, 0xf>(0.f, t);
    t += psg_dpp<0x142, 0xa>(0.f, t);
    const float lo = __builtin_bit_cast(float, __builtin_amdgcn_readlane(__builtin_bit_cast(int, t), 31));
    const float hi = __builtin_bit_cast(float, __builtin_amdgcn_readlane(__builtin_bit_cast(int, t), 63));
    return lane < 32 ? lo : hi;
  };
  const float mean = half_sum(s) * (1.0f / H);
  float q = 0.f;
#pragma unroll
  for (int c = 0; c < 3; ++c)
#pragma unroll
    for (int e = 0; e < 8; ++e) {
      const float d = v[c][e] - mean;
      q += d * d;
    }
  const float rstd = 1.0f / sqrtf(half_sum(q) * (1.0f / H) + eps);
#pragma unroll
  for (int c = 0; c < 3; ++c) {
    const int col = (c * 32 + hl) * 8;
    const float4 g0 = *reinterpret_cast<const float4*>(gamma + col), g1 = *reinterpret_cast<const float4*>(gamma + col + 4);
    const float4 b0 = *reinterpret_cast<const float4*>(beta + col), b1 = *reinterpret_cast<const float4*>(beta + col + 4);
    const float g[8] = {g0.x, g0.y, g0.z, g0.w, g1.x, g1.y, g1.z, g1.w};
    const float b[8] = {b0.x, b0.y, b0.z, b0.w, b1.x, b1.y, b1.z, b1.w};
    float o[8];
#pragma unroll
    for (int e = 0; e < 8; ++e) o[e] = (v[c][e] - mean) * rstd * g[e] + b[e];
    if (live)
      *reinterpret_cast<uint4*>(out + row * H + col) =
          make_uint4(E::pack(o[0], o[1]), E::pack(o[2], o[3]), E::pack(o[4], o[5]), E::pack(o[6], o[7]));
  }
}

template <typename E>
__global__ void __launch_bounds__(256) add_layernorm_res32_kernel(const uint16_t* __restrict__ x, const float* __restrict__ res,
                                                                  const float* __restrict__ bias, const float* __restrict__ gamma,
                                                                  const float* __restrict__ beta, float eps, int64_t rows,
                                                                  uint16_t* __restrict__ out16, float* __restrict__ out32,
                                                                  int res_period, const int32_t* __restrict__ res_index) {
  constexpr int H = 768;
  const int64_t row = ((int64_t)blockIdx.x * blockDim.x + threadIdx.x) >> 6;
  const int lane = threadIdx.x & 63;
  if (row >= rows) return;
  int64_t rrow = res_period > 0 ? row % res_period : row;
  if (res_index) rrow += (int64_t)res_index[row / res_period] * res_period;
  float v[3][4];
  uint2 xw[3];
  float4 rw[3];
#pragma unroll
  for (int c = 0; c < 3; ++c) {
    const int col = c * 256 + lane * 4;
    xw[c] = *reinterpret_cast<const uint2*>(x + row * H + col);
    if (res) rw[c] = *reinterpret_cast<const float4*>(res + rrow * H + col);
  }
#pragma unroll
  for (int c = 0; c < 3; ++c) {
    const int col = c * 256 + lane * 4;
    v[c][0] = E::to_f32((uint16_t)(xw[c].x & 0xffffu));
    v[c][1] = E::to_f32((uint16_t)(xw[c].x >> 16));
    v[c][2] = E::to_f32((uint16_t)(xw[c].y & 0xffffu));
    v[c][3] = E::to_f32((uint16_t)(xw[c].y >> 16));
    if (bias) {
      const float4 b = *reinterpret_cast<const float4*>(bias + col);
      v[c][0] += b.x; v[c][1] += b.y; v[c][2] += b.z; v[c][3] += b.w;
    }
    if (res) {
      v[c][0] += rw[c].x; v[c][1] += rw[c].y; v[c][2] += rw[c].z; v[c][3] += rw[c].w;
    }
  }
  ln_row<3>(v, H, eps, gamma, beta, lane);
#pragma unroll
  for (int c = 0; c < 3; ++c) {
    const int col = c * 256 + lane * 4;
    if (out32) *reinterpret_cast<float4*>(out32 + row * H + col) = make_float4(v[c][0], v[c][1], v[c][2], v[c][3]);
    if (out16)
      *reinterpret_cast<uint2*>(out16 + row * H + col) = make_uint2(E::pack(v[c][0], v[c][1]), E::pack(v[c][2], v[c][3]));
  }
}

extern "C" int psg_add_layernorm_res32(psg_ctx* ctx, const void* x, const float* residual, int res_period,
                                       const int32_t* res_index, const float* bias, const float* gamma, const float* beta,
                                       float eps, int64_t rows, int hidden, void* out16, float* out32, int dtype,
                                       void* stream) {
  PSG_REQUIRE(ctx && x && gamma && beta && (out16 || out32), PSG_ERR_INVALID, "psg_add_layernorm_res32: NULL argument");
  PSG_REQUIRE(hidden == 768, PSG_ERR_UNSUPPORTED, "psg_add_layernorm_res32: hidden=%d (kernel is built for 768)", hidden);
  PSG_REQUIRE(res_period >= 0 && (!res_index || (res_period > 0 && rows % res_period == 0)), PSG_ERR_INVALID,
              "psg_add_layernorm_res32: res_period=%d rows=%lld", res_period, (long long)rows);
  if (rows == 0) return PSG_OK;
  dim3 grid((unsigned)((rows + 3) / 4));
  PSG_DISPATCH_E16(dtype, "psg_add_layernorm_res32",
                   (add_layernorm_res32_kernel<E><<<grid, 256, 0, (hipStream_t)stream>>>(
                       (const uint16_t*)x, residual, bias, gamma, beta, eps, rows, (uint16_t*)out16, out32, res_period,
                       res_index)));
  PSG_CHECK_LAUNCH("psg_add_layernorm_res32");
  return PSG_OK;
}

static int add_layernorm_launch(const char* who, psg_ctx* ctx, const void* x, const void* residual, int res_period,
                                const int32_t* res_index, const float* bias, const float* gamma, const float* beta, float eps, int64_t rows,
                                int hidden, void* out, int dtype, void* stream) {
  PSG_REQUIRE(ctx && x && gamma && beta && out, PSG_ERR_INVALID, "%s: NULL argument", who);
  PSG_REQUIRE(hidden == 768, PSG_ERR_UNSUPPORTED, "%s: hidden=%d (kernel is built for 768)", who, hidden);
  if (rows == 0) return PSG_OK;
  if ((dtype == PSG_BF16 || dtype == PSG_F16) && ctx->opt.ln_half_wave) {
    dim3 grid16((unsigned)((rows + 7) / 8));
    PSG_DISPATCH_E16(dtype, who,
                     (add_layernorm16_kernel<E><<<grid16, 256, 0, (hipStream_t)stream>>>(
                         (const uint16_t*)x, (const uint16_t*)residual, bias, gamma, beta, eps, rows, (uint16_t*)out,
                         res_period, res_index)));
    PSG_CHECK_LAUNCH(who);
    return PSG_OK;
  }
  dim3 grid((unsigned)((rows + 3) / 4));
  PSG_DISPATCH_DTYPE(dtype, who,
                     (add_layernorm_kernel<T, 3><<<grid, 256, 0, (hipStream_t)stream>>>(
                         (const T*)x, (const T*)residual, bias, gamma, beta, eps, rows, hidden, (T*)out, res_period,
                         res_index)));
  PSG_CHECK_LAUNCH(who);
  return PSG_OK;
}

extern "C" int psg_add_layernorm(psg_ctx* ctx, const void* x, const void* residual, const float* bias,
                                 const float* gamma, const float* beta, float eps, int64_t rows, int hidden, void* out,
                                 int dtype, void* stream) {
  return add_layernorm_launch("psg_add_layernorm", ctx, x, residual, 0, nullptr, bias, gamma, beta, eps, rows, hidden, out,
                              dtype, stream);
}

extern "C" int psg_add_layernorm_periodic(psg_ctx* ctx, const void* x, const void* residual_table, int table_rows,
                                          const float* bias, const float* gamma, const float* beta, float eps,
                                          int64_t rows, int hidden, void* out, int dtype, void* stream) {
  PSG_REQUIRE(residual_table && table_rows > 0, PSG_ERR_INVALID, "psg_add_layernorm_periodic: table_rows=%d", table_rows);
  return add_layernorm_launch("psg_add_layernorm_periodic", ctx, x, residual_table, table_rows, nullptr, bias, gamma, beta,
                              eps, rows, hidden, out, dtype, stream);
}

extern "C" int psg_add_layernorm_indexed(psg_ctx* ctx, const void* x, const void* residual_table, const int32_t* block_index,
                                         int group, const float* bias, const float* gamma, const float* beta, float eps,
                                         int64_t rows, int hidden, void* out, int dtype, void* stream) {
  PSG_REQUIRE(residual_table && block_index && group > 0 && rows % group == 0, PSG_ERR_INVALID,
              "psg_add_layernorm_indexed: group=%d rows=%lld", group, (long long)rows);
  return add_layernorm_launch("psg_add_layernorm_indexed", ctx, x, residual_table, group, block_index, bias, gamma, beta,
                              eps, rows, hidden, out, dtype, stream);
}

template <typename T>
__global__ void bias_gelu_kernel(const T* __restrict__ x, const float* __restrict__ bias, int64_t n4, int cols,
                                 T* __restrict__ out) {
  for (int64_t i = (int64_t)blockIdx.x * blockDim.x + threadIdx.x; i < n4; i += (int64_t)gridDim.x * blockDim.x) {
    float v[4];
    Act<T>::ld4(x, i * 4, v);
    if (bias) {
      const int col = (int)((i * 4) % cols);
      const float4 b = *reinterpret_cast<const float4*>(bias + col);
      v[0] += b.x; v[1] += b.y; v[2] += b.z; v[3] += b.w;
    }
#pragma unroll
    for (int e = 0; e < 4; ++e) v[e] = 0.5f * v[e] * (1.0f + erff(v[e] * 0.70710678118654752440f));
    Act<T>::st4(out, i * 4, v);
  }
}

__device__ __forceinline__ float gelu_erf_as(float v) {
  const float x = v * 0.70710678118654752440f;
  const float ax = fabsf(x);
  const float t = __builtin_amdgcn_rcpf(fmaf(0.3275911f, ax, 1.0f));
  float poly = fmaf(1.061405429f, t, -1.453152027f);
  poly = fmaf(poly, t, 1.421413741f);
  poly = fmaf(poly, t, -0.284496736f);
  poly = fmaf(poly, t, 0.254829592f);
  const float e = __builtin_amdgcn_exp2f(-1.4426950408889634f * ax * ax);
  const float erf_abs = fmaf(-poly * t, e, 1.0f);
  return 0.5f * v * (1.0f + copysignf(erf_abs, x));
}

template <typename E>
__global__ void __launch_bounds__(256) bias_gelu_rows_bf16_kernel(const uint16_t* __restrict__ x,
                                                                   const float* __restrict__ bias, int64_t rows,
                                                                   int cols, uint16_t* __restrict__ out) {
  const int c = (blockIdx.x * 256 + threadIdx.x) * 8;
  if (c >= cols) return;
  float b[8] = {0, 0, 0, 0, 0, 0, 0, 0};
  if (bias) {
    *reinterpret_cast<float4*>(b) = *reinterpret_cast<const float4*>(bias + c);
    *reinterpret_cast<float4*>(b + 4) = *reinterpret_cast<const float4*>(bias + c + 4);
  }
  for (int64_t r = blockIdx.y; r < rows; r += gridDim.y) {
    const uint4 xv = *reinterpret_cast<const uint4*>(x + r * cols + c);
    const uint32_t xw[4] = {xv.x, xv.y, xv.z, xv.w};
    uint32_t ow[4];
#pragma unroll
    for (int e = 0; e < 4; ++e) {
      const float v0 = E::to_f32((uint16_t)(xw[e] & 0xffffu)) + b[2 * e];
      const float v1 = E::to_f32((uint16_t)(xw[e] >> 16)) + b[2 * e + 1];
      ow[e] = (uint32_t)E::from_f32(gelu_erf_as(v0)) | ((uint32_t)E::from_f32(gelu_erf_as(v1)) << 16);
    }
    *reinterpret_cast<uint4*>(out + r * cols + c) = make_uint4(ow[0], ow[1], ow[2], ow[3]);
  }
}

extern "C" int psg_bias_gelu(psg_ctx* ctx, const void* x, const float* bias, int64_t rows, int cols, void* out,
                             int dtype, void* stream) {
  PSG_REQUIRE(ctx && x && out, PSG_ERR_INVALID, "psg_bias_gelu: NULL argument");
  PSG_REQUIRE(cols > 0 && cols % 4 == 0, PSG_ERR_INVALID, "psg_bias_gelu: cols=%d must be a multiple of 4", cols);
  if (rows == 0) return PSG_OK;
  if ((dtype == PSG_BF16 || dtype == PSG_F16) && rows >= 256 && cols % 8 == 0) {
    const dim3 grid((unsigned)((cols / 8 + 255) / 256), (unsigned)(rows < 16384 ? rows : 16384));
    PSG_DISPATCH_E16(dtype, "psg_bias_gelu",
                     (bias_gelu_rows_bf16_kernel<E><<<grid, 256, 0, (hipStream_t)stream>>>(
                         (const uint16_t*)x, bias, rows, cols, (uint16_t*)out)));
    PSG_CHECK_LAUNCH("psg_bias_gelu");
    return PSG_OK;
  }
  int64_t n4 = rows * cols / 4;
  int64_t blocks = (n4 + 255) / 256;
  if (blocks > 256 * 16) blocks = 256 * 16;
  PSG_DISPATCH_DTYPE(dtype, "psg_bias_gelu",
                     (bias_gelu_kernel<T><<<(unsigned)blocks, 256, 0, (hipStream_t)stream>>>((const T*)x, bias, n4,
                                                                                           cols, (T*)out)));
  PSG_CHECK_LAUNCH("psg_bias_gelu");
  return PSG_OK;
}

template <typename T>
__global__ void exist_head_kernel(const T* __restrict__ x, const float* __restrict__ w, const float* __restrict__ b,
                                  int P, int nq, int hidden, float* __restrict__ logit, float* __restrict__ prob) {
  const int p = (int)(((int64_t)blockIdx.x * blockDim.x + threadIdx.x) >> 6);
  const int lane = threadIdx.x & 63;
  if (p >= P) return;
  const int64_t base = (int64_t)p * nq * hidden;
  float acc = 0.f;
  for (int c = lane * 4; c < hidden; c += 256) {
    float v[4];
    Act<T>::ld4(x, base + c, v);
    const float4 ww = *reinterpret_cast<const float4*>(w + c);
    acc += v[0] * ww.x + v[1] * ww.y + v[2] * ww.z + v[3] * ww.w;
  }
  acc = wave_sum(acc);
  if (lane == 0) {
    const float l = acc + b[0];
    logit[p] = l;
    if (prob) prob[p] = 1.0f / (1.0f + expf(-l));
  }
}

extern "C" int psg_exist_head(psg_ctx* ctx, const void* x, const float* w, const float* b, int P, int nq, int hidden,
                              float* logit, float* prob, int dtype, void* stream) {
  PSG_REQUIRE(hidden % 4 == 0 && P >= 0 && nq > 0, PSG_ERR_INVALID, "psg_exist_head: P=%d nq=%d hidden=%d", P, nq,
              hidden);
  PSG_REQUIRE(ctx && w && b, PSG_ERR_INVALID, "psg_exist_head: NULL argument");
  if (P == 0) return PSG_OK;
  PSG_REQUIRE(x && logit, PSG_ERR_INVALID, "psg_exist_head: NULL argument");
  PSG_DISPATCH_DTYPE(dtype, "psg_exist_head",
                     (exist_head_kernel<T><<<(P + 3) / 4, 256, 0, (hipStream_t)stream>>>((const T*)x, w, b, P, nq,
                                                                                       hidden, logit, prob)));
  PSG_CHECK_LAUNCH("psg_exist_head");
  return PSG_OK;
}

constexpr int MC_TP = 64, MC_KC = 64, MC_RMAX = 128;
template <typename T, int CG>
__global__ void __launch_bounds__(256) multiclass_head_kernel(const T* __restrict__ x, const float* __restrict__ w,
                                                              const float* __restrict__ b, int P, int nq, int hidden,
                                                              int R, const int32_t* __restrict__ pair_index, int N,
                                                              float* __restrict__ logit, float* __restrict__ prob) {
  __shared__ float xs[MC_KC][MC_TP + 4];
  __shared__ float ws[MC_KC][CG * 16 + 1];
  const int tid = threadIdx.x, tx = tid & 15, ty = tid >> 4;
  const int p0 = blockIdx.x * MC_TP;
  float acc[4][CG];
#pragma unroll
  for (int a = 0; a < 4; ++a)
#pragma unroll
    for (int c = 0; c < CG; ++c) acc[a][c] = 0.f;
  for (int k0 = 0; k0 < hidden; k0 += MC_KC) {
    for (int e = tid; e < MC_TP * (MC_KC / 4); e += 256) {
      const int pp = e / (MC_KC / 4), cc = (e % (MC_KC / 4)) * 4;
      float v[4] = {0.f, 0.f, 0.f, 0.f};
      if (p0 + pp < P) Act<T>::ld4(x, (int64_t)(p0 + pp) * nq * hidden + k0 + cc, v);
#pragma unroll
      for (int u = 0; u < 4; ++u) xs[cc + u][pp] = v[u];
    }
    for (int e = tid; e < CG * 16 * (MC_KC / 4); e += 256) {
      const int r = e / (MC_KC / 4), cc = (e % (MC_KC / 4)) * 4;
      float4 v = make_float4(0.f, 0.f, 0.f, 0.f);
      if (r < R) v = *reinterpret_cast<const float4*>(w + (int64_t)r * hidden + k0 + cc);
      ws[cc][r] = v.x;
      ws[cc + 1][r] = v.y;
      ws[cc + 2][r] = v.z;
      ws[cc + 3][r] = v.w;
    }
    __syncthreads();
#pragma unroll 8
    for (int kk = 0; kk < MC_KC; ++kk) {
      const float4 xv = *reinterpret_cast<const float4*>(&xs[kk][ty * 4]);
#pragma unroll
// ... 560 lines not shown
```

### openpsg_amd/csrc/psg_split.hip

```cpp
#include "psg_common.h"

#define SP_ORDER_HHL 0
#define SP_ORDER_HLH 1
#define SP_ORDER_I2 2

__global__ void __launch_bounds__(256) split_f16x3_kernel(const float* __restrict__ x, int64_t row_stride, int K, int order,
                                                          uint16_t* __restrict__ out, float* __restrict__ inv_scale) {
  __shared__ float s_max[4];
  const int64_t row = blockIdx.x;
  const float* xr = x + row * row_stride;
  const int tid = threadIdx.x;
  float mx = 0.f;
  for (int c = tid * 4; c < K; c += 256 * 4) {
    const float4 v = *reinterpret_cast<const float4*>(xr + c);
    mx = fmaxf(fmaxf(mx, fmaxf(fabsf(v.x), fabsf(v.y))), fmaxf(fabsf(v.z), fabsf(v.w)));
  }
  mx = wave_max(mx);
  if ((tid & 63) == 0) s_max[tid >> 6] = mx;
  __syncthreads();
  mx = fmaxf(fmaxf(s_max[0], s_max[1]), fmaxf(s_max[2], s_max[3]));
  int e = (int)((__float_as_uint(mx) >> 23) & 255u) - 127;
  if (!(mx > 0.f) || e == 128) e = 13;
  int se = 127 + 13 - e;
  se = se < 1 ? 1 : (se > 253 ? 253 : se);
  const float scale = __uint_as_float((uint32_t)se << 23);
  if (tid == 0) inv_scale[row] = __uint_as_float((uint32_t)(254 - se) << 23);
  uint16_t* o0 = out + row * (order == SP_ORDER_I2 ? 2 : 3) * (int64_t)K;
  uint16_t* oh2 = o0 + (order == SP_ORDER_HHL ? K : 2 * (int64_t)K);
  uint16_t* ol = o0 + (order == SP_ORDER_HHL ? 2 * (int64_t)K : K);
  for (int c = tid * 4; c < K; c += 256 * 4) {
    const float4 v = *reinterpret_cast<const float4*>(xr + c);
    const float s[4] = {v.x * scale, v.y * scale, v.z * scale, v.w * scale};
    ushort4 h, l;
    uint16_t* hp = &h.x;
    uint16_t* lp = &l.x;
#pragma unroll
    for (int i = 0; i < 4; ++i) {
      const uint16_t hb = f32_to_f16(s[i]);
      hp[i] = hb;
      lp[i] = f32_to_f16(s[i] - f16_to_f32(hb));
    }
    if (order == SP_ORDER_I2) {
      uint16_t* ob = o0 + (c >> 5) * 64 + (c & 31);
      *reinterpret_cast<ushort4*>(ob) = h;
      *reinterpret_cast<ushort4*>(ob + 32) = l;
      continue;
    }
    *reinterpret_cast<ushort4*>(o0 + c) = h;
    *reinterpret_cast<ushort4*>(oh2 + c) = h;
    *reinterpret_cast<ushort4*>(ol + c) = l;
  }
}

extern "C" int psg_split_f16x3(psg_ctx* ctx, const float* x, int64_t rows, int K, int64_t row_stride, int order,
                               void* out, float* inv_scale, void* stream) {
  PSG_REQUIRE(ctx && x && out && inv_scale, PSG_ERR_INVALID, "psg_split_f16x3: NULL argument");
  PSG_REQUIRE(rows >= 0 && K > 0 && K % 4 == 0 && row_stride >= K && row_stride % 4 == 0 &&
                  (order == SP_ORDER_HHL || order == SP_ORDER_HLH || (order == SP_ORDER_I2 && K % 32 == 0)) &&
                  rows < (1ll << 31),
              PSG_ERR_INVALID, "psg_split_f16x3: rows=%lld K=%d stride=%lld order=%d", (long long)rows, K,
              (long long)row_stride, order);
  if (rows == 0) return PSG_OK;
  split_f16x3_kernel<<<(unsigned)rows, 256, 0, (hipStream_t)stream>>>(x, row_stride, K, order, (uint16_t*)out, inv_scale);
  PSG_CHECK_LAUNCH("psg_split_f16x3");
  return PSG_OK;
}

__global__ void __launch_bounds__(256) split_f16x2_kernel(const float* __restrict__ x, int64_t row_stride, int K, int64_t rows,
                                                          uint16_t* __restrict__ out, float* __restrict__ inv_scale) {
  __shared__ float s_max[4];
  const int64_t row = blockIdx.x;
  const float* xr = x + row * row_stride;
  const int tid = threadIdx.x;
  float mx = 0.f;
  for (int c = tid * 4; c < K; c += 256 * 4) {
    const float4 v = *reinterpret_cast<const float4*>(xr + c);
    mx = fmaxf(fmaxf(mx, fmaxf(fabsf(v.x), fabsf(v.y))), fmaxf(fabsf(v.z), fabsf(v.w)));
  }
  mx = wave_max(mx);
  if ((tid & 63) == 0) s_max[tid >> 6] = mx;
  __syncthreads();
  mx = fmaxf(fmaxf(s_max[0], s_max[1]), fmaxf(s_max[2], s_max[3]));
  int e = (int)((__float_as_uint(mx) >> 23) & 255u) - 127;
  if (!(mx > 0.f) || e == 128) e = 13;
  int se = 127 + 13 - e;
  se = se < 1 ? 1 : (se > 253 ? 253 : se);
  const float scale = __uint_as_float((uint32_t)se << 23);
  if (tid == 0) inv_scale[row] = __uint_as_float((uint32_t)(254 - se) << 23);
  uint16_t* oh = out + row * (int64_t)K;
  uint16_t* ol = out + (rows + row) * (int64_t)K;
  for (int c = tid * 4; c < K; c += 256 * 4) {
    const float4 v = *reinterpret_cast<const float4*>(xr + c);
    const float s[4] = {v.x * scale, v.y * scale, v.z * scale, v.w * scale};
    ushort4 h, l;
    uint16_t* hp = &h.x;
    uint16_t* lp = &l.x;
#pragma unroll
    for (int i = 0; i < 4; ++i) {
      const uint16_t hb = f32_to_f16(s[i]);
      hp[i] = hb;
      lp[i] = f32_to_f16(s[i] - f16_to_f32(hb));
    }
    *reinterpret_cast<ushort4*>(oh + c) = h;
    *reinterpret_cast<ushort4*>(ol + c) = l;
  }
}

__device__ __forceinline__ float sp_row_scale(float mx, float* inv_scale_out);
__device__ __forceinline__ void sp_store2(uint16_t* oh, uint16_t* ol, int c, const float (&x)[4], float scale, int wt = 0);
template <int NCH>
__global__ void __launch_bounds__(1024) split_f16x2_small_kernel(const float* __restrict__ x, int64_t row_stride, int K,
                                                                 int64_t rows, uint16_t* __restrict__ out,
                                                                 float* __restrict__ inv_scale, int wt) {
  __shared__ float s_max[16];
  const int64_t row = blockIdx.x;
  const float* xr = x + row * row_stride;
  const int tid = threadIdx.x;
  float v[NCH][4];
  float mx = 0.f;
#pragma unroll
  for (int c = 0; c < NCH; ++c) {
    const int col = (c * 1024 + tid) * 4;
    if (col < K) {
      const float4 t = *reinterpret_cast<const float4*>(xr + col);
      v[c][0] = t.x; v[c][1] = t.y; v[c][2] = t.z; v[c][3] = t.w;
      mx = fmaxf(fmaxf(mx, fmaxf(fabsf(t.x), fabsf(t.y))), fmaxf(fabsf(t.z), fabsf(t.w)));
    }
  }
  mx = wave_max(mx);
  if ((tid & 63) == 0) s_max[tid >> 6] = mx;
  __syncthreads();
  mx = 0.f;
  for (int i = 0; i < 16; ++i) mx = fmaxf(mx, s_max[i]);
  const float scale = sp_row_scale(mx, tid == 0 ? inv_scale + row : nullptr);
  uint16_t* oh = out + row * (int64_t)K;
  uint16_t* ol = out + (rows + row) * (int64_t)K;
#pragma unroll
  for (int c = 0; c < NCH; ++c) {
    const int col = (c * 1024 + tid) * 4;
    if (col < K) sp_store2(oh, ol, col, v[c], scale, wt);
  }
}

extern "C" int psg_split_f16x2(psg_ctx* ctx, const float* x, int64_t rows, int K, int64_t row_stride, void* out,
                               float* inv_scale, void* stream) {
  PSG_REQUIRE(ctx && x && out && inv_scale, PSG_ERR_INVALID, "psg_split_f16x2: NULL argument");
  PSG_REQUIRE(rows >= 0 && K > 0 && K % 4 == 0 && row_stride >= K && row_stride % 4 == 0 && rows < (1ll << 31),
              PSG_ERR_INVALID, "psg_split_f16x2: rows=%lld K=%d stride=%lld", (long long)rows, K, (long long)row_stride);
  if (rows == 0) return PSG_OK;
  if (rows <= 64 && K <= 16384) {
    hipStream_t st = (hipStream_t)stream;
    if (K <= 4096) split_f16x2_small_kernel<1><<<(unsigned)rows, 1024, 0, st>>>(x, row_stride, K, rows, (uint16_t*)out, inv_scale, (ctx->opt.wt_stores >> 2) & 1);
    else if (K <= 12288) split_f16x2_small_kernel<3><<<(unsigned)rows, 1024, 0, st>>>(x, row_stride, K, rows, (uint16_t*)out, inv_scale, (ctx->opt.wt_stores >> 2) & 1);
    else split_f16x2_small_kernel<4><<<(unsigned)rows, 1024, 0, st>>>(x, row_stride, K, rows, (uint16_t*)out, inv_scale, (ctx->opt.wt_stores >> 2) & 1);
    PSG_CHECK_LAUNCH("psg_split_f16x2");
    return PSG_OK;
  }
  split_f16x2_kernel<<<(unsigned)rows, 256, 0, (hipStream_t)stream>>>(x, row_stride, K, rows, (uint16_t*)out, inv_scale);
  PSG_CHECK_LAUNCH("psg_split_f16x2");
  return PSG_OK;
}

__global__ void __launch_bounds__(256) scale_rows_cols_kernel(float* __restrict__ y, int64_t rows, int N,
                                                              const float* __restrict__ row_scale,
                                                              const float* __restrict__ col_scale) {
  const int64_t n4 = N / 4;
  for (int64_t i = (int64_t)blockIdx.x * blockDim.x + threadIdx.x; i < rows * n4; i += (int64_t)gridDim.x * blockDim.x) {
    const int64_t m = i / n4;
    const int c = (int)(i - m * n4) * 4;
    const float rs = row_scale[m];
    const float4 cs = *reinterpret_cast<const float4*>(col_scale + c);
    float4 v = *reinterpret_cast<float4*>(y + m * N + c);
    v.x *= rs * cs.x; v.y *= rs * cs.y; v.z *= rs * cs.z; v.w *= rs * cs.w;
    *reinterpret_cast<float4*>(y + m * N + c) = v;
  }
}

extern "C" int psg_scale_rows_cols(psg_ctx* ctx, float* y, int64_t rows, int N, const float* row_scale,
                                   const float* col_scale, void* stream) {
  PSG_REQUIRE(ctx && y && row_scale && col_scale, PSG_ERR_INVALID, "psg_scale_rows_cols: NULL argument");
  PSG_REQUIRE(rows >= 0 && N > 0 && N % 4 == 0, PSG_ERR_INVALID, "psg_scale_rows_cols: rows=%lld N=%d", (long long)rows, N);
  if (rows == 0) return PSG_OK;
  int64_t blocks = (rows * (N / 4) + 255) / 256;
  if (blocks > 4096) blocks = 4096;
  scale_rows_cols_kernel<<<(unsigned)blocks, 256, 0, (hipStream_t)stream>>>(y, rows, N, row_scale, col_scale);
  PSG_CHECK_LAUNCH("psg_scale_rows_cols");
  return PSG_OK;
}

#include "psg_decode_math.h"

__device__ __forceinline__ float sp_row_scale(float mx, float* inv_scale_out) {
  int e = (int)((__float_as_uint(mx) >> 23) & 255u) - 127;
  if (!(mx > 0.f) || e == 128) e = 13;
  int se = 127 + 13 - e;
  se = se < 1 ? 1 : (se > 253 ? 253 : se);
  if (inv_scale_out) *inv_scale_out = __uint_as_float((uint32_t)(254 - se) << 23);
  return __uint_as_float((uint32_t)se << 23);
}
__device__ __forceinline__ void sp_store2(uint16_t* oh, uint16_t* ol, int c, const float (&x)[4], float scale, int wt);
__device__ __forceinline__ void sp_store3(uint16_t* o0, int K, int c, const float (&x)[4], float scale) {
  ushort4 h, l;
  uint16_t* hp = &h.x;
  uint16_t* lp = &l.x;
#pragma unroll
  for (int i = 0; i < 4; ++i) {
    const float s = x[i] * scale;
    const uint16_t hb = f32_to_f16(s);
    hp[i] = hb;
    lp[i] = f32_to_f16(s - f16_to_f32(hb));
  }
  *reinterpret_cast<ushort4*>(o0 + c) = h;
  *reinterpret_cast<ushort4*>(o0 + K + c) = h;
  *reinterpret_cast<ushort4*>(o0 + 2 * (int64_t)K + c) = l;
}

template <int NCH, int NTHR>
__global__ void __launch_bounds__(NTHR) rmsnorm_split_kernel(float* __restrict__ resid, const float* __restrict__ delta,
                                                            const float* __restrict__ d_rs, const float* __restrict__ d_cs,
                                                            const float* __restrict__ w, float eps, int hidden,
                                                            uint16_t* __restrict__ out3, float* __restrict__ inv_scale,
                                                            int dslices, int64_t dstride, int planes) {
  __shared__ float s_part[NTHR / 64], s_max[NTHR / 64];
  const int64_t row = blockIdx.x;
  const int tid = threadIdx.x, lane = tid & 63, wid = tid >> 6;
  float v[NCH][4];
  float4 g[NCH];
  const float rs = delta ? d_rs[row] : 0.f;
#pragma unroll
  for (int c = 0; c < NCH; ++c) {
    const int col = (c * NTHR + tid) * 4;
    if (col < hidden) {
      const float4 r = *reinterpret_cast<const float4*>(resid + row * hidden + col);
      g[c] = *reinterpret_cast<const float4*>(w + col);
      v[c][0] = r.x; v[c][1] = r.y; v[c][2] = r.z; v[c][3] = r.w;
      if (delta) {
        float4 d = *reinterpret_cast<const float4*>(delta + row * hidden + col);
        for (int sl = 1; sl < dslices; ++sl) {
          const float4 e = *reinterpret_cast<const float4*>(delta + sl * dstride + row * hidden + col);
          d.x += e.x; d.y += e.y; d.z += e.z; d.w += e.w;
        }
        const float4 cs = *reinterpret_cast<const float4*>(d_cs + col);
        v[c][0] += d.x * (rs * cs.x); v[c][1] += d.y * (rs * cs.y); v[c][2] += d.z * (rs * cs.z); v[c][3] += d.w * (rs * cs.w);
      }
    }
  }
  float ss = 0.f;
#pragma unroll
  for (int c = 0; c < NCH; ++c)
    if ((c * NTHR + tid) * 4 < hidden) ss = psg_sumsq4(v[c], ss);
  ss = wave_sum(ss);
  if (lane == 0) s_part[wid] = ss;
  __syncthreads();
  ss = 0.f;
  for (int i = 0; i < NTHR / 64; ++i) ss += s_part[i];
  const float inv = 1.0f / sqrtf(ss / (float)hidden + eps);
  float x[NCH][4];
  float mx = 0.f;
#pragma unroll
  for (int c = 0; c < NCH; ++c) {
    const int col = (c * NTHR + tid) * 4;
    if (col < hidden) {
      if (delta) *reinterpret_cast<float4*>(resid + row * hidden + col) = make_float4(v[c][0], v[c][1], v[c][2], v[c][3]);
      x[c][0] = g[c].x * (v[c][0] * inv); x[c][1] = g[c].y * (v[c][1] * inv);
      x[c][2] = g[c].z * (v[c][2] * inv); x[c][3] = g[c].w * (v[c][3] * inv);
      mx = fmaxf(fmaxf(mx, fmaxf(fabsf(x[c][0]), fabsf(x[c][1]))), fmaxf(fabsf(x[c][2]), fabsf(x[c][3])));
    }
  }
  mx = wave_max(mx);
  if (lane == 0) s_max[wid] = mx;
  __syncthreads();
  mx = s_max[0];
#pragma unroll
  for (int i = 1; i < NTHR / 64; ++i) mx = fmaxf(mx, s_max[i]);
  const float scale = sp_row_scale(mx, tid == 0 ? inv_scale + row : nullptr);
  uint16_t* o0 = out3 + row * 3 * (int64_t)hidden;
  uint16_t* oh = out3 + row * (int64_t)hidden;
  uint16_t* ol = oh + dstride;
#pragma unroll
  for (int c = 0; c < NCH; ++c) {
    const int col = (c * NTHR + tid) * 4;
    if (col < hidden) {
      if (planes == 2) sp_store2(oh, ol, col, x[c], scale);
      else sp_store3(o0, hidden, col, x[c], scale);
    }
  }
}

extern "C" int psg_rmsnorm_split(psg_ctx* ctx, float* resid, const float* delta, const float* delta_row_scale,
                                 const float* delta_col_scale, int delta_slices, const float* w, float eps, int64_t rows,
                                 int hidden, void* out3, float* inv_scale, int planes, void* stream) {
  PSG_REQUIRE(ctx && resid && w && out3 && inv_scale && (!delta || (delta_row_scale && delta_col_scale)), PSG_ERR_INVALID,
              "psg_rmsnorm_split: NULL argument");
  PSG_REQUIRE(hidden % 4 == 0 && hidden > 0 && hidden <= 8192 && rows >= 0 && rows < (1ll << 31), PSG_ERR_UNSUPPORTED,
              "psg_rmsnorm_split: hidden=%d rows=%lld", hidden, (long long)rows);
  if (rows == 0) return PSG_OK;
  const int nthr = (rows <= 64 && hidden >= 4096) ? 1024 : 256;
  const int nch = (hidden + 4 * nthr - 1) / (4 * nthr);
  hipStream_t st = (hipStream_t)stream;
#define RNS(N, T)                                                                                                   \
  rmsnorm_split_kernel<N, T><<<(unsigned)rows, T, 0, st>>>(resid, delta, delta_row_scale, delta_col_scale, w, eps, hidden, \
                                                          (uint16_t*)out3, inv_scale, delta_slices, rows * (int64_t)hidden, planes)
  if (nthr == 1024) {
    if (nch <= 1) RNS(1, 1024);
    else RNS(2, 1024);
  } else switch (nch) {
    case 1: RNS(1, 256); break;
    case 2: RNS(2, 256); break;
    case 3: RNS(3, 256); break;
    case 4: RNS(4, 256); break;
    case 5: RNS(5, 256); break;
    case 6: RNS(6, 256); break;
    case 7: RNS(7, 256); break;
    default: RNS(8, 256); break;
  }
#undef RNS
  PSG_CHECK_LAUNCH("psg_rmsnorm_split");
  return PSG_OK;
}

#define SP_MAXCH 16
__global__ void __launch_bounds__(256) silu_mul_split_kernel(const float* __restrict__ gu, const float* __restrict__ rsv,
                                                             const float* __restrict__ csv, int inter,
                                                             uint16_t* __restrict__ out3, float* __restrict__ inv_scale,
                                                             int slices, int64_t rows, int planes) {
  __shared__ float s_max[4];
  const int64_t row = blockIdx.x;
  const int tid = threadIdx.x, lane = tid & 63, wid = tid >> 6;
  const float rs = rsv[row];
  const float* gr = gu + row * 2 * (int64_t)inter;
  float o[SP_MAXCH][4];
  float mx = 0.f;
#pragma unroll
  for (int c = 0; c < SP_MAXCH; ++c) {
    const int col = (c * 256 + tid) * 4;
    if (col < inter) {
      float4 g4 = *reinterpret_cast<const float4*>(gr + col), u4 = *reinterpret_cast<const float4*>(gr + inter + col);
      for (int sl = 1; sl < slices; ++sl) {
        const float* gs = gr + sl * rows * 2 * (int64_t)inter;
        const float4 g5 = *reinterpret_cast<const float4*>(gs + col), u5 = *reinterpret_cast<const float4*>(gs + inter + col);
        g4.x += g5.x; g4.y += g5.y; g4.z += g5.z; g4.w += g5.w;
        u4.x += u5.x; u4.y += u5.y; u4.z += u5.z; u4.w += u5.w;
      }
      const float4 cg = *reinterpret_cast<const float4*>(csv + col), cu = *reinterpret_cast<const float4*>(csv + inter + col);
      const float g[4] = {g4.x * (rs * cg.x), g4.y * (rs * cg.y), g4.z * (rs * cg.z), g4.w * (rs * cg.w)};
      const float u[4] = {u4.x * (rs * cu.x), u4.y * (rs * cu.y), u4.z * (rs * cu.z), u4.w * (rs * cu.w)};
#pragma unroll
      for (int e = 0; e < 4; ++e) {
        const float s = g[e] / (1.0f + expf(-g[e]));
        o[c][e] = s * u[e];
        mx = fmaxf(mx, fabsf(o[c][e]));
      }
// ... 236 lines not shown
```

### openpsg_amd/csrc/psg_wave.h

```cpp
#pragma once
#include "psg_common.h"

template <int N_>
__device__ __forceinline__ void psg_vmwait() {
  asm volatile("s_waitcnt vmcnt(%0)" ::"n"(N_) : "memory");
}
template <int N_>
__device__ __forceinline__ void psg_lgkmwait() {
  asm volatile("s_waitcnt lgkmcnt(%0)" ::"n"(N_) : "memory");
}
__device__ __forceinline__ void psg_lds_barrier() { asm volatile("s_waitcnt lgkmcnt(0)\n\ts_barrier" ::: "memory"); }

template <int PER, int MAXN>
struct PsgDmaWait {
  static __device__ __forceinline__ void go(int newer) {
    if (newer >= MAXN) psg_vmwait<(MAXN * PER < 63 ? MAXN * PER : 63)>();
    else PsgDmaWait<PER, MAXN - 1>::go(newer);
  }
};
template <int PER>
struct PsgDmaWait<PER, 0> {
  static __device__ __forceinline__ void go(int) { psg_vmwait<0>(); }
};

__device__ __forceinline__ psg_u32x4 psg_lds_read128(uint32_t a) {
  psg_u32x4 v;
  asm volatile("ds_read_b128 %0, %1" : "=v"(v) : "v"(a) : "memory");
  return v;
}
__device__ __forceinline__ uint32_t psg_lds_read32(uint32_t a) {
  uint32_t v;
  asm volatile("ds_read_b32 %0, %1" : "=v"(v) : "v"(a) : "memory");
  return v;
}
__device__ __forceinline__ psg_u32x2 psg_lds_read64(uint32_t a) {
  psg_u32x2 v;
  asm volatile("ds_read_b64 %0, %1" : "=v"(v) : "v"(a) : "memory");
  return v;
}
__device__ __forceinline__ void psg_lds_write64(uint32_t a, psg_u32x2 v) {
  asm volatile("ds_write_b64 %0, %1" ::"v"(a), "v"(v) : "memory");
}
__device__ __forceinline__ void psg_lds_write32(uint32_t a, uint32_t v) {
  asm volatile("ds_write_b32 %0, %1" ::"v"(a), "v"(v) : "memory");
}
__device__ __forceinline__ psg_f32x4 psg_lds_read128_wait(uint32_t a) {
  psg_f32x4 v;
  asm volatile("ds_read_b128 %0, %1\n\ts_waitcnt lgkmcnt(0)" : "=v"(v) : "v"(a) : "memory");
  return v;
}
__device__ __forceinline__ void psg_lds_write128_mfma(uint32_t a, psg_f32x4 v) {
  asm volatile("s_nop 15\n\tds_write_b128 %0, %1" ::"v"(a), "v"(v) : "memory");
}

__device__ __forceinline__ float psg_xchg32_max(float x) {
  const auto r = __builtin_amdgcn_permlane32_swap(__float_as_uint(x), __float_as_uint(x), false, false);
  return fmaxf(__uint_as_float(r[0]), __uint_as_float(r[1]));
}
__device__ __forceinline__ float psg_xchg32_sum(float x) {
  const auto r = __builtin_amdgcn_permlane32_swap(__float_as_uint(x), __float_as_uint(x), false, false);
  return __uint_as_float(r[0]) + __uint_as_float(r[1]);
}
template <int NOP16 = 3, int NOP32 = 3>
__device__ __forceinline__ float psg_rows4_sum(float v) {
  float a = v, b = v;
  asm volatile("s_nop %2\n\tv_permlane16_swap_b32 %0, %1" : "+v"(a), "+v"(b) : "n"(NOP16));
  const float s = a + b;
  float c = s, d = s;
  asm volatile("s_nop %2\n\tv_permlane32_swap_b32 %0, %1" : "+v"(c), "+v"(d) : "n"(NOP32));
  return c + d;
}
__device__ __forceinline__ float psg_rows4_sum_mfma(float v) { return psg_rows4_sum<7, 1>(v); }
__device__ __forceinline__ float psg_rows4_max(float v) {
  float a = v, b = v;
  asm volatile("s_nop 3\n\tv_permlane16_swap_b32 %0, %1" : "+v"(a), "+v"(b));
  const float s = fmaxf(a, b);
  float c = s, d = s;
  asm volatile("s_nop 3\n\tv_permlane32_swap_b32 %0, %1" : "+v"(c), "+v"(d));
  return fmaxf(c, d);
}
```

### openpsg_amd/ops.py

```python
from __future__ import annotations

import torch

from . import _lib
from ._lib import PSG_PRO_RMSNORM, PSG_PRO_DECODE_ATTN, PSG_PRO_SILU_MUL
from ._lib import (PSG_BF16, PSG_F16, PSG_F32, PSG_EMPTY_UNIFORM, PSG_EMPTY_UNMASKED, PSG_XATTN_MFMA,
                   PSG_XATTN_SIMPLE, PsgHipError, check)

_DT = {torch.float32: PSG_F32, torch.bfloat16: PSG_BF16, torch.float16: PSG_F16}


def _dt(t: torch.Tensor) -> int:
    try:
        return _DT[t.dtype]
    except KeyError:
        raise PsgHipError(f"unsupported activation dtype {t.dtype}") from None


def _p(t, dtype=None, name="tensor"):
    if t is None:
        return None
    if not t.is_cuda:
        raise PsgHipError(f"{name} must live in HBM (got a {t.device} tensor); this path has no CPU fallback")
    if not t.is_contiguous():
# ... 908 lines not shown
                    M, N, K, mode)


def batch_split_gemm_w4(x2, inv_scale, w4, e_img, col_scale, mode=0) -> Partials:
    M, K = _x2_args("batch_split_gemm_w4", x2, inv_scale)
    N = _w4_args("batch_split_gemm_w4", w4, e_img, col_scale, K)
    return _batch_q("batch_split_gemm_w4", x2, True,
                    (_p(x2), _p(inv_scale), _p(w4, name="w4"), _p(e_img, name="e_img"), _p(col_scale)), M, N, K, mode)


def skinny_gemm_fused(kind, x_out, w, sync, *, inp=None, resid=None, norm_w=None, eps=0.0, attn=None, splits=None):
    import ctypes
    from ._lib import Prologue
    lib, ctx, st = _env(x_out)
    M, K = x_out.shape
    N = w.shape[0]
    assert w.shape[1] == K and w.dtype == x_out.dtype and sync.dtype == torch.int32 and sync.numel() >= 2
    if splits is None:
        s = ctypes.c_int(0)
        check(lib.psg_skinny_gemm_plan(ctx, M, N, K, _dt(x_out), ctypes.byref(s)), "psg_skinny_gemm_plan")
        splits = s.value
    pro = Prologue()
    pro.kind = int(kind)
    if inp is not None:
        pro.input, pro.in_splits = _in(inp, x_out.dtype)
    if resid is not None:
        pro.resid = _p(resid, x_out.dtype)
        pro.norm_w = _p(norm_w, torch.float32)
        pro.eps = float(eps)
    if attn is not None:
        tok_pair, tok_pos, rope, heads, ctx_len, kc, vc = attn
        pro.tok_pair, pro.tok_pos = _p(tok_pair, torch.int32), _p(tok_pos, torch.int32)
        pro.rope_cos, pro.rope_sin = _p(rope[0], torch.float32), _p(rope[1], torch.float32)
        pro.heads, pro.ctx = int(heads), int(ctx_len)
        pro.k_cache, pro.v_cache = _p(kc, x_out.dtype), _p(vc, x_out.dtype)
    pro.sync = sync.data_ptr()
    part = torch.empty((splits, M, N), device=x_out.device, dtype=torch.float32)
    check(lib.psg_skinny_gemm_fused(ctx, ctypes.byref(pro), _p(x_out), _p(w), _p(part), M, N, K, splits, _dt(x_out), st),
          "psg_skinny_gemm_fused")
    return Partials(part)


def masked_mean_pool(feat, pan, img_hw, pad_hw, object_ids):
    import ctypes
    lib, ctx, st = _env(feat)
    _, Cc, Hf, Wf = feat.shape
    N = object_ids.numel()
    nbytes = ctypes.c_int64(0)
    check(lib.psg_masked_mean_pool_workspace(ctx, Cc, Hf, Wf, N, ctypes.byref(nbytes)),
          "psg_masked_mean_pool_workspace")
    ws = torch.empty(nbytes.value // 4, device=feat.device, dtype=torch.int32)
    out = torch.empty((N, Cc), device=feat.device, dtype=torch.float32)
    check(lib.psg_masked_mean_pool(ctx, _p(feat, torch.float32), Cc, Hf, Wf, _p(pan, torch.int32, "pan_results"),
                                   pan.shape[0], pan.shape[1], int(img_hw[0]), int(img_hw[1]), int(pad_hw[0]),
                                   int(pad_hw[1]), _p(object_ids, torch.int32), N, _p(out), _p(ws), nbytes.value, st),
          "psg_masked_mean_pool")
    return out


def masked_split_mean_pool(feat, pan, img_hw, pad_hw, object_ids, output_size):
    import ctypes
    lib, ctx, st = _env(feat)
    _, Cc, Hf, Wf = feat.shape
    N = object_ids.numel()
    nbytes = ctypes.c_int64(0)
    check(lib.psg_masked_mean_pool_workspace(ctx, Cc, Hf, Wf, N, ctypes.byref(nbytes)), "psg_masked_mean_pool_workspace")
    ws = torch.empty(nbytes.value // 4, device=feat.device, dtype=torch.int32)
    out = torch.empty((N, int(output_size), Cc), device=feat.device, dtype=torch.float32)
    check(lib.psg_masked_split_mean_pool(ctx, _p(feat, torch.float32), Cc, Hf, Wf, _p(pan, torch.int32, "pan_results"),
                                         pan.shape[0], pan.shape[1], int(img_hw[0]), int(img_hw[1]), int(pad_hw[0]),
                                         int(pad_hw[1]), _p(object_ids, torch.int32), N, int(output_size), _p(out), _p(ws),
                                         nbytes.value, st), "psg_masked_split_mean_pool")
    return out


def bilinear_scores(sub, obj, num_relations):
    lib, ctx, st = _env(sub)
    B, N, RC = sub.shape
    assert obj.shape == sub.shape and RC % num_relations == 0
    pred = torch.empty((B, num_relations, N, N), device=sub.device, dtype=torch.float32)
    check(lib.psg_bilinear_scores(ctx, _p(sub, torch.float32, "sub"), _p(obj, torch.float32, "obj"), B, N,
                                  num_relations, RC // num_relations, _p(pred), st), "psg_bilinear_scores")
    return pred


def train_object_bitmasks(thing_masks, sem, is_thing, category, thing_index, grid_hw):
    lib, ctx, st = _env(sem)
    H, W = sem.shape
    N = is_thing.numel()
    gh, gw = int(grid_hw[0]), int(grid_hw[1])
    words = (gh * gw + 63) // 64
    bits = torch.empty((N, words), device=sem.device, dtype=torch.int64)
    n_thing = 0 if thing_masks is None else thing_masks.shape[0]
    if n_thing and tuple(thing_masks.shape[1:]) != (H, W):
        raise PsgHipError(f"train_object_bitmasks: thing masks are {tuple(thing_masks.shape[1:])}, the semantic map is "
                          f"{(H, W)}; both must be at the padded image resolution (V4:371-399)")
    check(lib.psg_train_object_bitmasks(ctx, _p(thing_masks, torch.uint8, "thing_masks") if n_thing else None, n_thing,
                                        _p(sem, torch.int32, "sem"), H, W, _p(is_thing, torch.int32),
                                        _p(category, torch.int32), _p(thing_index, torch.int32), N, gh, gw, _p(bits),
                                        words, st), "psg_train_object_bitmasks")
    return bits


def bce_with_logits(logit, label, weight=1.0):
    lib, ctx, st = _env(logit)
    out = torch.empty(1, device=logit.device, dtype=torch.float32)
    check(lib.psg_bce_with_logits(ctx, _p(logit, torch.float32, "logit"), _p(label, torch.float32, "label"),
                                  logit.numel(), float(weight), _p(out), st), "psg_bce_with_logits")
    return out[0]


def cross_entropy_rows(logits, labels):
    lib, ctx, st = _env(logits)
    rows, vocab = logits.shape
    loss = torch.empty(rows, device=logits.device, dtype=torch.float32)
    check(lib.psg_cross_entropy_rows(ctx, _p(logits), rows, vocab, _p(labels, torch.int32, "labels"), _p(loss),
                                     _dt(logits), st), "psg_cross_entropy_rows")
    return loss


TILES = {"auto": 0, "256x256": 1, "256x192": 2, "256x128": 3, "256x64": 4, "128x128": 5}


def dense_gemm(x, w, bias=None, gelu=False, out=None, out_dtype=None, row_scale=None, col_scale=None, tile="256x256",
               swiglu=False):
    lib, ctx, st = _env(x)
    M, K = x.shape
    N = w.shape[0]
    assert w.shape[1] == K and w.dtype == x.dtype
    odt = x.dtype if out_dtype is None else out_dtype
    out = torch.empty((M, N // 2 if swiglu else N), device=x.device, dtype=odt) if out is None else out
    assert out.shape == (M, N // 2 if swiglu else N)
    assert not (swiglu and gelu)
    check(lib.psg_dense_gemm_tiled(ctx, _p(x, name="x"), _p(w, name="w"), _p(bias, torch.float32, "bias"),
                                   2 if swiglu else 1 if gelu else 0, _p(out, odt), M, N, K, _dt(x), _DT[odt],
                                   _p(row_scale, torch.float32, "row_scale"), _p(col_scale, torch.float32, "col_scale"),
                                   TILES[tile], st), "psg_dense_gemm")
    return out


def dense_gemm_split(x2, w2, bias, row_scale, col_scale, gelu=False, out=None, tile="auto"):
    lib, ctx, st = _env(x2)
    M, K2 = x2.shape
    N = w2.shape[0]
    assert w2.shape[1] == K2 and x2.dtype == torch.float16 and w2.dtype == torch.float16
    out = torch.empty((M, N), device=x2.device, dtype=torch.float32) if out is None else out
    assert out.shape == (M, N) and out.dtype == torch.float32
    check(lib.psg_dense_gemm_split(ctx, _p(x2, name="x2"), _p(w2, name="w2"), _p(bias, torch.float32, "bias"),
                                   1 if gelu else 0, _p(out, torch.float32), M, N, K2, _p(row_scale, torch.float32, "row_scale"),
                                   _p(col_scale, torch.float32, "col_scale"), TILES[tile], st), "psg_dense_gemm_split")
    return out


def interleave_gate_up(w_gate_up):
    lib, ctx, st = _env(w_gate_up)
    n2, K = w_gate_up.shape
    out = torch.empty_like(w_gate_up)
    check(lib.psg_interleave_gate_up(ctx, _p(w_gate_up, name="gate_up"), _p(out), n2 // 2, K, st), "psg_interleave_gate_up")
    return out


def split_f16x3(x, weights=False):
    lib, ctx, st = _env(x)
    assert x.dim() == 2 and x.dtype == torch.float32 and x.stride(1) == 1
    rows, K = x.shape
    out = torch.empty((rows, 3 * K), device=x.device, dtype=torch.float16)
    inv = torch.empty(rows, device=x.device, dtype=torch.float32)
    check(lib.psg_split_f16x3(ctx, x.data_ptr(), rows, K, x.stride(0), 1 if weights else 0, _p(out), _p(inv), st),
          "psg_split_f16x3")
    return out, inv


def split_f16i2(x):
    lib, ctx, st = _env(x)
    assert x.dim() == 2 and x.dtype == torch.float32 and x.stride(1) == 1 and x.shape[1] % 32 == 0
    rows, K = x.shape
    out = torch.empty((rows, 2 * K), device=x.device, dtype=torch.float16)
    inv = torch.empty(rows, device=x.device, dtype=torch.float32)
    check(lib.psg_split_f16x3(ctx, x.data_ptr(), rows, K, x.stride(0), 2, _p(out), _p(inv), st), "psg_split_f16x3")
    return out, inv


def scale_rows_cols(y, row_scale, col_scale):
    lib, ctx, st = _env(y)
    rows, N = y.shape
    assert row_scale.numel() == rows and col_scale.numel() == N
    check(lib.psg_scale_rows_cols(ctx, _p(y, torch.float32, "y"), rows, N, _p(row_scale, torch.float32),
                                  _p(col_scale, torch.float32), st), "psg_scale_rows_cols")
    return y


class Scaled:
    __slots__ = ("y", "row_scale", "col_scale")

    def __init__(self, y, row_scale, col_scale):
        assert y.dtype == torch.float32 and y.dim() in (2, 3) and y.is_contiguous()
        assert row_scale.numel() == y.shape[-2] and col_scale.numel() == y.shape[-1]
        self.y, self.row_scale, self.col_scale = y, row_scale, col_scale

    def dense(self):
        y = self.y if self.y.dim() == 2 else self.y.sum(0)
        return scale_rows_cols(y, self.row_scale, self.col_scale)


def rmsnorm_split(resid, delta, w, eps, planes=3):
    lib, ctx, st = _env(resid)
    rows, hidden = resid.shape
    out = torch.empty((rows, 3 * hidden) if planes == 3 else (2, rows, hidden), device=resid.device, dtype=torch.float16)
    inv = torch.empty(rows, device=resid.device, dtype=torch.float32)
    dp, rp, cp = (None, None, None) if delta is None else (_p(delta.y), _p(delta.row_scale, torch.float32),
                                                           _p(delta.col_scale, torch.float32))
    nsl = 1 if delta is None or delta.y.dim() == 2 else delta.y.shape[0]
    assert delta is None or delta.y.shape[-2:] == (rows, hidden)
    check(lib.psg_rmsnorm_split(ctx, _p(resid, torch.float32, "resid"), dp, rp, cp, nsl, _p(w, torch.float32), float(eps),
                                rows, hidden, _p(out), _p(inv), int(planes), st), "psg_rmsnorm_split")
    return out, inv


def rope_kvwrite_scaled(qkv, tok_pair, tok_pos, rope, heads, head_dim, ctx_len, q_out, k_cache, v_cache, kv_heads=None):
    lib, ctx, st = _env(q_out)
    rows = q_out.shape[0]
    kv = heads if kv_heads is None else int(kv_heads)
    assert isinstance(qkv, Scaled) and qkv.y.shape[-2:] == (rows, (heads + 2 * kv) * head_dim)
    nsl = 1 if qkv.y.dim() == 2 else qkv.y.shape[0]
    if _gqa(heads, kv_heads):
        check(lib.psg_rope_kvwrite_scaled_gqa(ctx, _p(qkv.y), _p(qkv.row_scale, torch.float32),
                                              _p(qkv.col_scale, torch.float32), _p(tok_pair, torch.int32),
                                              _p(tok_pos, torch.int32), _p(rope[0], torch.float32),
                                              _p(rope[1], torch.float32), nsl, rows, heads, kv, head_dim, ctx_len,
                                              _p(q_out, torch.float32), _p(k_cache, torch.float32),
                                              _p(v_cache, torch.float32), st), "psg_rope_kvwrite_scaled_gqa")
        return
    check(lib.psg_rope_kvwrite_scaled(ctx, _p(qkv.y), _p(qkv.row_scale, torch.float32), _p(qkv.col_scale, torch.float32),
                                      _p(tok_pair, torch.int32), _p(tok_pos, torch.int32), _p(rope[0], torch.float32),
                                      _p(rope[1], torch.float32), nsl, rows, heads, head_dim, ctx_len, _p(q_out, torch.float32),
                                      _p(k_cache, torch.float32), _p(v_cache, torch.float32), st), "psg_rope_kvwrite_scaled")


def silu_mul_split(gate_up, inter, planes=3):
    lib, ctx, st = _env(gate_up.y)
    rows = gate_up.y.shape[-2]
    nsl = 1 if gate_up.y.dim() == 2 else gate_up.y.shape[0]
    assert gate_up.y.shape[-1] == 2 * inter
    out = torch.empty((rows, 3 * inter) if planes == 3 else (2, rows, inter), device=gate_up.y.device, dtype=torch.float16)
    inv = torch.empty(rows, device=gate_up.y.device, dtype=torch.float32)
    check(lib.psg_silu_mul_split(ctx, _p(gate_up.y), _p(gate_up.row_scale, torch.float32), _p(gate_up.col_scale, torch.float32),
                                 nsl, rows, inter, _p(out), _p(inv), int(planes), st), "psg_silu_mul_split")
    return out, inv
```

### openpsg_amd/qformer.py

```python
from __future__ import annotations

import torch
import torch.nn.functional as F

from . import _lib, ops
from ._lib import PSG_EMPTY_UNIFORM, PSG_EMPTY_UNMASKED, PsgHipError
from .config import PSGConfig


class RelationQueryEngine:
    def __init__(self, weights: dict, cfg: PSGConfig, device, dtype=torch.bfloat16, xattn_variant=None, resid_dtype=None,
                 split=False):
        if dtype not in (torch.float32, torch.bfloat16, torch.float16):
            raise PsgHipError(f"activation dtype must be float32, bfloat16 or float16, got {dtype}")
        self.cfg, self.device, self.dtype = cfg, torch.device(device), dtype
        self.res32 = resid_dtype == torch.float32 and dtype != torch.float32
        self.split = bool(split) and dtype == torch.float32
        self.split_i2 = bool(_lib.get_option(self.device.index or 0, "split_i2")) if self.split else False
        self._split_w, self._bias32 = {}, {}
        self.own_gemm = int(_lib.get_option(self.device.index or 0, "qformer_own_gemm"))
        self.xattn_variant = xattn_variant
        self._xidx_cache = {}
        self.index_xattn = True
        q = cfg.qformer
        f32 = lambda k: weights[k].to(device=self.device, dtype=torch.float32).contiguous()
        act = lambda t: t.to(device=self.device, dtype=dtype).contiguous()
        pre = "relation_qformer.embeddings."
        self.word_emb = f32(pre + "word_embeddings.weight")
        self.pos_emb = f32(pre + "position_embeddings.weight")
        self.emb_ln = (f32(pre + "layernorm.weight"), f32(pre + "layernorm.bias"))
        self.query_rows = torch.cat([f32("rel_cls_query")[0], f32("relation_query")[0]], dim=0).contiguous()
        self.patch_w = f32("patch_embed.proj.weight")
        self.patch_b = f32("patch_embed.proj.bias")
        self.exist_w = self.exist_b = self.mc_w = self.mc_b = None
        if "binary_rel_cls_pred.weight" in weights:
            self.exist_w = f32("binary_rel_cls_pred.weight").reshape(-1).contiguous()
            self.exist_b = f32("binary_rel_cls_pred.bias")
        if "multiclass_rel_cls_pred.weight" in weights:
            self.mc_w = f32("multiclass_rel_cls_pred.weight")
            self.mc_b = f32("multiclass_rel_cls_pred.bias")
        self.layers = []
        for l in range(q.layers):
            p = f"relation_qformer.encoder.layer.{l}."
            a, x = p + "attention.", p + "crossattention."
            L = dict(
                wqkv=act(torch.cat([weights[a + f"attention.{n}.weight"] for n in ("query", "key", "value")], 0)),
                bqkv=act(torch.cat([weights[a + f"attention.{n}.bias"] for n in ("query", "key", "value")], 0)),
                wo=act(weights[a + "output.dense.weight"]), bo=f32(a + "output.dense.bias"),
                ln_a=(f32(a + "output.LayerNorm.weight"), f32(a + "output.LayerNorm.bias")),
                wq_x=act(weights[x + "attention.query.weight"]), bq_x=act(weights[x + "attention.query.bias"]),
                wk_x=act(weights[x + "attention.key.weight"]), bk_x=act(weights[x + "attention.key.bias"]),
                wv_x=act(weights[x + "attention.value.weight"]), bv_x=act(weights[x + "attention.value.bias"]),
                wo_x=act(weights[x + "output.dense.weight"]), bo_x=f32(x + "output.dense.bias"),
                ln_x=(f32(x + "output.LayerNorm.weight"), f32(x + "output.LayerNorm.bias")),
                w1q=act(weights[p + "intermediate_query.dense.weight"]), b1q=f32(p + "intermediate_query.dense.bias"),
                w2q=act(weights[p + "output_query.dense.weight"]), b2q=f32(p + "output_query.dense.bias"),
                ln_q=(f32(p + "output_query.LayerNorm.weight"), f32(p + "output_query.LayerNorm.bias")),
                w1t=act(weights[p + "intermediate.dense.weight"]), b1t=f32(p + "intermediate.dense.bias"),
                w2t=act(weights[p + "output.dense.weight"]), b2t=f32(p + "output.dense.bias"),
                ln_t=(f32(p + "output.LayerNorm.weight"), f32(p + "output.LayerNorm.bias")),
            )
            if l == q.layers - 1:
                H, hd = q.hidden, q.hidden // q.heads
                L["wk"] = L["wqkv"][H:2 * H].view(q.heads, hd, H)
                L["wk32"] = L["wk"].float().contiguous()
                L["wv32t"] = L["wqkv"][2 * H:].float().view(q.heads, hd, H).transpose(1, 2).contiguous()
            self.layers.append(L)
        self.empty_policy = PSG_EMPTY_UNIFORM if cfg.empty_row_policy == "uniform" else PSG_EMPTY_UNMASKED
        opt = lambda name: bool(_lib.get_option(self.device.index or 0, name))
        self.share_query_qkv = opt("qformer_share_qkv")
        self.cls_input_space = opt("qformer_cls_input_space") and not (self.own_gemm >= 2) and (
            not self.split or (self.split_i2 and opt("qformer_split_cls_input_space")))
        self._cls_big = None
        self._bmm_out_dtype = None
        self.dedup_prompts = opt("qformer_dedup_prompts")

    def patch_embed(self, mask_features: torch.Tensor) -> torch.Tensor:
        if self.cfg.patch_size == 16 and mask_features.shape[-1] % 4 == 0 and self.patch_w.shape[0] % 128 == 0:
            return ops.patch_embed(mask_features.contiguous(), self.patch_w, self.patch_b, 16)
        x = F.conv2d(mask_features, self.patch_w, self.patch_b, stride=self.cfg.patch_size)
        return x.flatten(2).transpose(1, 2)[0].contiguous()

    def object_bitmasks(self, pan: torch.Tensor, img_meta: dict, object_ids: torch.Tensor, feat_hw) -> torch.Tensor:
        gh, gw = feat_hw[0] // self.cfg.patch_size, feat_hw[1] // self.cfg.patch_size
        grid = ops.mask_grid(pan, img_meta["img_shape"][:2], img_meta["pad_shape"][:2], (gh, gw))
        return ops.object_bitmasks(grid, object_ids)

    def cross_kv(self, patches: torch.Tensor):
        pa = patches.to(self.dtype)
        return [(self._lin(pa, L["wk_x"], L["bk_x"]), self._lin(pa, L["wv_x"], L["bv_x"])) for L in self.layers]

    def _embed(self, ids):
        q = self.cfg.qformer
        nq, H = q.q_rows, q.hidden
        P, T = ids.shape
        R, RQ = P * (nq + T), P * nq
        X = torch.empty((R, H), device=self.device, dtype=self.dtype)
        X32 = torch.empty((R, H), device=self.device, dtype=torch.float32) if self.res32 else None
        first = X32 if self.res32 else X
        shared0 = len(self.layers) > 1 and T > 0 and self.share_query_qkv
        if shared0:
            ops.qformer_embed_split(ids, self.word_emb, self.pos_emb, self.query_rows, self.emb_ln[0], self.emb_ln[1],
                                    q.ln_eps, first[:nq], first[RQ:])
            if self.res32:
                X[:nq].copy_(X32[:nq])
                X[RQ:].copy_(X32[RQ:])
        else:
            ops.qformer_embed(ids, self.word_emb, self.pos_emb, self.query_rows, self.emb_ln[0], self.emb_ln[1],
                              q.ln_eps, first)
            if self.res32:
                X.copy_(X32)
        return X, X32, shared0

    def _ln(self, x, r16, r32, bias, ln, out16=None, out32=None, period=0, index=None, want32=True):
        eps = self.cfg.qformer.ln_eps
        if self.res32:
            return ops.add_layernorm_res32(x, r32, bias, ln[0], ln[1], eps, out16=out16, out32=out32, period=period,
                                           index=index, want32=want32)
        if index is not None:
            return ops.add_layernorm_indexed(x, r16, index, period, bias, ln[0], ln[1], eps, out=out16), None
        if period:
            return ops.add_layernorm_periodic(x, r16, bias, ln[0], ln[1], eps, out=out16), None
        return ops.add_layernorm(x, r16, bias, ln[0], ln[1], eps, out=out16), None

    @staticmethod
    def _s(t, a, b=None):
        return None if t is None else (t[a:] if b is None else t[a:b])

    def _cross(self, li, qx, nq, img):
        q = self.cfg.qformer
        kv, bits, num_objects, pair_index, segments = img
        if segments is None:
            return ops.qformer_cross_attn(qx, kv[li][0], kv[li][1], bits, pair_index, num_objects, nq, q.heads,
                                          empty_policy=self.empty_policy, variant=self.xattn_variant)
        cx = torch.empty_like(qx)
        for ps, pc, kv_m, bits_m, n_m in segments:
            ops.qformer_cross_attn(qx[ps * nq:(ps + pc) * nq], kv_m[li][0], kv_m[li][1], bits_m,
                                   pair_index[ps:ps + pc], n_m, nq, q.heads, out=cx[ps * nq:(ps + pc) * nq],
                                   empty_policy=self.empty_policy, variant=self.xattn_variant)
        return cx

    def _cross_prompt(self, qx_u, nq, img, inv, rows):
        q = self.cfg.qformer
        H = q.hidden
        kv, bits, num_objects, pair_index, _ = img
        P = inv.numel()
        cached = rows is not None
        if not cached:
            rows = (inv.to(torch.int64)[:, None] * nq + torch.arange(nq, device=self.device)[None, :]).reshape(-1).to(torch.int32)
        cx = None
        if (self.index_xattn and self.dtype in (torch.bfloat16, torch.float16) and nq == 33
                and self.xattn_variant in (None, ops.PSG_XATTN_MFMA)):
            if cached:
                key = (rows.data_ptr(), inv.data_ptr(), P)
                ent = self._xidx_cache.get(key)
                if ent is None:
                    if len(self._xidx_cache) > 64:
                        self._xidx_cache.clear()
                    ent = self._xidx_cache[key] = (rows[::nq].contiguous(), inv.to(torch.int32).contiguous(), rows, inv)
            else:
                ent = (rows[::nq].contiguous(), inv.to(torch.int32).contiguous())
            q_cls = torch.empty((P, H), device=self.device, dtype=self.dtype)
            ops.gather_rows(qx_u, ent[0], q_cls)
            cx = ops.qformer_cross_attn_indexed(qx_u, ent[1], q_cls, kv[0][0], kv[0][1], bits, pair_index,
                                                num_objects, q.heads, empty_policy=self.empty_policy)
        if cx is None:
            qx = torch.empty((P * nq, H), device=self.device, dtype=self.dtype)
            ops.gather_rows(qx_u, rows, qx)
            cx = self._cross(0, qx, nq, img)
        return cx

    def _self_block(self, L, X, X32, G, T, mask, shared0=False, last=False):
        q = self.cfg.qformer
        nq, H = q.q_rows, q.hidden
        R, RQ = G * (nq + T), G * nq
        ctx = torch.empty((R, H), device=self.device, dtype=self.dtype)
        if shared0:
            qkv_q = self._lin(X[:nq], L["wqkv"], L["bqkv"])
            qkv = self._lin(X[RQ:], L["wqkv"], L["bqkv"])
            ops.qformer_self_attn_shared(qkv_q, qkv, mask, G, T, nq, q.heads, ctx)
        else:
            qkv = self._lin(X, L["wqkv"], L["bqkv"])
            ops.qformer_self_attn(qkv, mask, G, T, nq, q.heads, last, ctx)
        del qkv
        ra = RQ if last else R
        A = self._lin(ctx[:ra], L["wo"])
        A32 = torch.empty((ra, H), device=self.device, dtype=torch.float32) if self.res32 else None
        if shared0:
            self._ln(A[:RQ], X[:nq], self._s(X32, 0, nq), L["bo"], L["ln_a"], out32=self._s(A32, 0, RQ), period=nq)
            self._ln(A[RQ:], X[RQ:], self._s(X32, RQ), L["bo"], L["ln_a"], out32=self._s(A32, RQ))
        else:
            self._ln(A, X[:ra], self._s(X32, 0, ra), L["bo"], L["ln_a"], out32=A32)
        return A, A32

    def _query_tail(self, li, A, A32, nq, img, prompt=None, out16=None, out32=None):
        L = self.layers[li]
        qx = self._lin(A, L["wq_x"], L["bq_x"])
        if prompt is None:
            cx, period, index = self._cross(li, qx, nq, img), 0, None
        else:
            cx, period, index = self._cross_prompt(qx, nq, img, *prompt), nq, prompt[0]
        Cq = self._lin(cx, L["wo_x"])
        _, Cq32 = self._ln(Cq, A, A32, L["bo_x"], L["ln_x"], period=period, index=index)
        del qx, cx
        iq = self._ffn1(Cq, L["w1q"], L["b1q"])
        hq = self._lin(iq, L["w2q"])
        return self._ln(hq, Cq, Cq32, L["b2q"], L["ln_q"], out16=out16, out32=out32)

    def _text_ffn(self, L, A, A32, out16=None, out32=None):
        it = self._ffn1(A, L["w1t"], L["b1t"])
        ht = self._lin(it, L["w2t"])
        return self._ln(ht, A, A32, L["b2t"], L["ln_t"], out16=out16, out32=out32)

    def _layer(self, li, X, X32, P, T, text_mask, img, shared0=False, hidden_out=None):
        q = self.cfg.qformer
        nq, H = q.q_rows, q.hidden
        R, RQ = P * (nq + T), P * nq
        L = self.layers[li]
        last = li == len(self.layers) - 1
        A, A32 = self._self_block(L, X, X32, P, T, text_mask, shared0 and li == 0, last)
        if last and hidden_out is not None:
            assert hidden_out.shape == (RQ, H) and hidden_out.dtype == self.dtype and hidden_out.is_contiguous()
            Xn = hidden_out
        else:
            Xn = torch.empty((RQ if last else R, H), device=self.device, dtype=self.dtype)
        Xn32 = torch.empty((Xn.shape[0], H), device=self.device, dtype=torch.float32) if self.res32 else None
        self._query_tail(li, A[:RQ], self._s(A32, 0, RQ), nq, img, out16=Xn[:RQ], out32=self._s(Xn32, 0, RQ))
        if not last and T > 0:
            self._text_ffn(L, A[RQ:], self._s(A32, RQ), out16=Xn[RQ:], out32=self._s(Xn32, RQ))
        return Xn, Xn32

    def _cls_heads(self, x, P, nq, img, mc):
        _, _, num_objects, pair_index, segments = img
        logit = prob = None
        if self.exist_w is not None:
            logit, prob = ops.exist_head(x, self.exist_w, self.exist_b, P, nq)
        if mc is not None:
            if self.mc_w is None:
                raise PsgHipError("multiclass outputs requested from an engine without multiclass_rel_cls_pred")
            if segments is not None:
                raise PsgHipError("the multiclass head does not run over pair-sharded segments of several images")
            ops.multiclass_head(x, self.mc_w, self.mc_b, P, nq, pair_index, num_objects, logit=mc[0], prob=mc[1])
        return logit, prob

    def forward_pairs(self, kv, bits, num_objects, pair_index, ids, text_mask, hidden_out=None, segments=None, mc=None):
        P, T = ids.shape
        img = (kv, bits, num_objects, pair_index, segments)
        X, X32, shared0 = self._embed(ids)
        for li in range(len(self.layers)):
            X, X32 = self._layer(li, X, X32, P, T, text_mask, img, shared0,
                                 hidden_out if li == len(self.layers) - 1 else None)
        logit, prob = self._cls_heads(X32 if X32 is not None else X, P, self.cfg.qformer.q_rows, img, mc)
        return X, logit, prob

    def _cls_in_space(self, T):
        q = self.cfg.qformer
        wide = self.dtype == torch.float32
        lds = (q.q_rows + T) * (q.hidden + (0 if wide else 8)) * (4 if wide else 2) + q.heads * 256
        return self.cls_input_space and q.hidden == 768 and q.heads == 12 and lds <= 160 * 1024

    def forward_pairs_cls(self, kv, bits, num_objects, pair_index, ids, text_mask, segments=None, prompts=None, mc=None):
        P, T = ids.shape
        RQ = P * self.cfg.qformer.q_rows
        nl = len(self.layers)
        img = (kv, bits, num_objects, pair_index, segments)
        in_space = self._cls_in_space(T)
        if (prompts is not None and segments is None and nl == 2 and T > 0 and in_space and self.dedup_prompts
                and prompts[0].shape[0] <= 0.9 * P):
            return self._forward_pairs_cls_dedup(img, text_mask, prompts, mc)
        X, X32, shared0 = self._embed(ids)
        for li in range(nl - 1):
            X, X32 = self._layer(li, X, X32, P, T, text_mask, img, shared0)
        state = self._state(X[:RQ], self._s(X32, 0, RQ), X[RQ:], self._s(X32, RQ), None, P, T, text_mask, img, X, X32)
        logit, prob = self._cls_phase(state, text_mask, in_space, mc)
        return state, logit, prob

    @staticmethod
    def _state(Xq, Xq32, Xt, Xt32, tix, P, T, text_mask, img, X=None, X32=None):
        kv, bits, num_objects, pair_index, segments = img
        return dict(Xq=Xq, Xq32=Xq32, Xt=Xt, Xt32=Xt32, tix=tix, X=X, X32=X32, P=P, T=T, text_mask=text_mask,
                    pair_index=pair_index, kv=kv, bits=bits, num_objects=num_objects, segments=segments)

    @staticmethod
    def _state_rows(state, segments=None):
        return (state["Xq"], state["Xq32"], state["Xt"], state["Xt32"], state["tix"],
                (state["kv"], state["bits"], state["num_objects"], state["pair_index"], segments))

    def _cls_phase(self, state, mask, in_space, mc=None):
        q = self.cfg.qformer
        nq, H = q.q_rows, q.hidden
        P, T, X = state["P"], state["T"], state["X"]
        Xq, Xq32, Xt, _, tix, img = self._state_rows(state, state["segments"])
        li, L = len(self.layers) - 1, self.layers[-1]
        x_cls = Xq.view(P, nq, H)[:, 0].contiguous()
        x_cls32 = Xq32.view(P, nq, H)[:, 0].contiguous() if Xq32 is not None else None
        q_cls = self._lin(x_cls, L["wqkv"][:H], L["bqkv"][:H])
        hd = H // q.heads
        if in_space:
            if self.split:
                g = self._cls_keys_split(q_cls, L)
            else:
                g = self._bmm_f32(q_cls.view(P, q.heads, hd).transpose(0, 1), L["wk"], L["wk32"])
            if X is not None:
                xbar = ops.qformer_cls_attn_input(X, g, mask, P, T, nq, q.heads)
            else:
                xbar = ops.qformer_cls_attn_input(Xq, g, mask, P, T, nq, q.heads, x_text=Xt, text_index=tix)
            if self.split:
                ctx = self._cls_values_split(xbar, L)
            else:
                ctx = (torch.bmm(xbar, L["wv32t"]).permute(1, 0, 2).reshape(P, H) + L["bqkv"][2 * H:].float()).to(self.dtype)
            del g, xbar
        else:
            assert X is not None
            kvs = self._lin(X, L["wqkv"][H:], L["bqkv"][H:])
            ctx = ops.qformer_self_attn_cls(q_cls, kvs, mask, P, T, nq, q.heads)
            del kvs
        A = self._lin(ctx, L["wo"])
        _, A32 = self._ln(A, x_cls, x_cls32, L["bo"], L["ln_a"])
        Xc, Xc32 = self._query_tail(li, A, A32, 1, img)
        return self._cls_heads(Xc32 if Xc32 is not None else Xc, P, 1, img, mc)

    def _forward_pairs_cls_dedup(self, img, text_mask, prompts, mc=None):
        nq = self.cfg.qformer.q_rows
        ids_u, mask_u, inv = prompts[:3]
        U, T = ids_u.shape
        P = inv.numel()
        RQu = U * nq
        L = self.layers[0]
        Xu, Xu32, shared0 = self._embed(ids_u)
        A, A32 = self._self_block(L, Xu, Xu32, U, T, mask_u, shared0)
        Xt_u, Xt_u32 = self._text_ffn(L, A[RQu:], self._s(A32, RQu))
        Xq, Xq32 = self._query_tail(0, A[:RQu], self._s(A32, 0, RQu), nq, img,
                                    prompt=(inv, prompts[3] if len(prompts) > 3 else None))
        state = self._state(Xq, Xq32, Xt_u, Xt_u32, inv, P, T, text_mask, img)
        logit, prob = self._cls_phase(state, mask_u, True, mc)
        return state, logit, prob

    def pair_hidden(self, state, sel, segments=None):
        nq = self.cfg.qformer.q_rows
        P, T = state["P"], state["T"]
        assert segments is not None or state["segments"] is None, "pair_hidden: pass the slots' segments"
        xq, xq32, xt, xt32, tix, img = self._state_rows(state, segments)
        s64 = sel.to(torch.int64).clamp(min=0)
        K = s64.numel()
        ar = torch.arange(nq, device=self.device)
        rows = [(s64[:, None] * nq + ar[None, :]).reshape(-1)]
        Xs32 = None
        if tix is not None:
            trows = (tix.to(torch.int64).index_select(0, s64)[:, None] * T
                     + torch.arange(T, device=self.device)[None, :]).reshape(-1)
            Xs = torch.cat([xq.index_select(0, rows[0]), xt.index_select(0, trows)])
            if xq32 is not None:
                Xs32 = torch.cat([xq32.index_select(0, rows[0]), xt32.index_select(0, trows)])
        else:
            if T > 0:
                rows.append((P * nq + s64[:, None] * T + torch.arange(T, device=self.device)[None, :]).reshape(-1))
            allrows = torch.cat(rows)
            Xs = state["X"].index_select(0, allrows)
            if state["X32"] is not None:
                Xs32 = state["X32"].index_select(0, allrows)
        tm = state["text_mask"].index_select(0, s64) if T > 0 else state["text_mask"]
        img = img[:3] + (img[3].index_select(0, s64), segments)
        return self._layer(len(self.layers) - 1, Xs, Xs32, K, T, tm, img)[0]

    def pair_hidden_sel(self, state, sel, first, count, slot_off=0):
        nq = self.cfg.qformer.q_rows
        T = state["T"]
        assert state["segments"] is None
        xq, xq32, xt, xt32, tix, img = self._state_rows(state)
        sel = sel.to(torch.int32).contiguous()
        Xs, tm, pi, mine = ops.gather_pair_rows(xq, xt, tix, state["text_mask"], img[3], sel, first, count, slot_off, nq, T)
        Xs32 = None
        if xq32 is not None:
            Xs32 = ops.gather_pair_rows(xq32, xt32, tix, None, None, sel, first, count, slot_off, nq, T, want_aux=False)[0]
        if T == 0:
            tm = state["text_mask"]
        hk = self._layer(len(self.layers) - 1, Xs, Xs32, sel.numel(), T, tm, img[:3] + (pi, None))[0]
        return hk, mine

    def _cls_big_weights(self, L):
        if self._cls_big is None:
            q = self.cfg.qformer
            H, heads = q.hidden, q.heads
            hd = H // heads
            wk = L["wqkv"][H:2 * H].float()
            wv = L["wqkv"][2 * H:].float()
            kbig = torch.zeros((heads * H, H), device=self.device, dtype=torch.float32)
            vbig = torch.zeros((H, heads * H), device=self.device, dtype=torch.float32)
            for h in range(heads):
                kbig[h * H:(h + 1) * H, h * hd:(h + 1) * hd] = wk[h * hd:(h + 1) * hd].t()
                vbig[h * hd:(h + 1) * hd, h * H:(h + 1) * H] = wv[h * hd:(h + 1) * hd]
            self._cls_big = (ops.split_f16i2(kbig), ops.split_f16i2(vbig), L["bqkv"][2 * H:].float().contiguous())
        return self._cls_big

    def _cls_keys_split(self, q_cls, L):
        q = self.cfg.qformer
        P = q_cls.shape[0]
        kb, _, _ = self._cls_big_weights(L)
        a2, inv_r = ops.split_f16i2(q_cls.contiguous())
        g = ops.dense_gemm_split(a2, kb[0], None, inv_r, kb[1], tile=self._tile(P))
        return g.view(P, q.heads, q.hidden).permute(1, 0, 2).contiguous()

    def _cls_values_split(self, xbar, L):
        q = self.cfg.qformer
        P = xbar.shape[1]
        _, vb, bias = self._cls_big_weights(L)
        x2, inv_r = ops.split_f16i2(xbar.permute(1, 0, 2).reshape(P, q.heads * q.hidden).contiguous())
        return ops.dense_gemm_split(x2, vb[0], bias, inv_r, vb[1], tile=self._tile(P))

    def _bmm_f32(self, a, b, b32):
        if a.dtype == torch.float32:
            return torch.bmm(a, b32)
        if self._bmm_out_dtype is None:
            try:
                torch.bmm(a[:, :1], b, out_dtype=torch.float32)
                self._bmm_out_dtype = True
            except (TypeError, RuntimeError):
                self._bmm_out_dtype = False
        if self._bmm_out_dtype:
            return torch.bmm(a, b, out_dtype=torch.float32)
        return torch.bmm(a.float(), b32)

    @staticmethod
    def _tile(rows):
        return "auto" if rows < 16384 else "256x256"

    def _lin(self, x, w, b=None, gelu=False):
        N, K = w.shape
        fits = N % 256 == 0 and K % 64 == 0 and x.shape[0] > 0
        if self.split and fits and x.dtype == torch.float32:
            i2 = self.split_i2 and K % 32 == 0
            key = (w.data_ptr(), N, K, i2)
            ws = self._split_w.get(key)
            if ws is None:
                ws = self._split_w[key] = ops.split_f16i2(w) if i2 else ops.split_f16x3(w, weights=True)
            tile = self._tile(x.shape[0])
            if i2:
                a2, inv_r = ops.split_f16i2(x)
                return ops.dense_gemm_split(a2, ws[0], b, inv_r, ws[1], gelu=gelu, tile=tile)
            a3, inv_r = ops.split_f16x3(x)
            return ops.dense_gemm(a3, ws[0], b, gelu=gelu, out_dtype=torch.float32, row_scale=inv_r, col_scale=ws[1],
                                  tile=tile)
        if self.own_gemm >= 2 and fits and x.dtype != torch.float32 and x.is_contiguous():
            if b is not None and b.dtype != torch.float32:
                key = (b.data_ptr(), N)
                b32 = self._bias32.get(key)
                if b32 is None:
                    b32 = self._bias32[key] = b.float().contiguous()
                b = b32
            return ops.dense_gemm(x, w, b, gelu=gelu)
        if gelu:
            y = F.linear(x, w)
            ops.bias_gelu(y, b)
            return y
        return F.linear(x, w, b)

    def _ffn1(self, x, w, b):
        if self.split or self.own_gemm >= 2:
            return self._lin(x, w, b, gelu=True)
        if (self.dtype != torch.float32 and w.shape[0] % 256 == 0 and w.shape[1] % 64 == 0 and x.shape[0] >= 256
                and self.own_gemm):
            return ops.dense_gemm(x, w, b, gelu=True)
        y = F.linear(x, w)
        ops.bias_gelu(y, b)
        return y

    def select(self, prob: torch.Tensor, k: int):
        return ops.topk(prob, k)[0]
```

Baseline: 18410 pairs/s.

## Fuse fp32-to-f16 split of activations into split GEMM A-tile staging

Adds a GEMM variant that loads fp32 activation rows straight into LDS and splits them into hi/lo f16 halves in-kernel, using a per-row abs-max published by the preceding LayerNorm or GELU epilogue. This removes the separate split_f16i2 pass over activations and its extra global write and read. The Q-Former wires this in through a row-max cache keyed on storage, and it is on by default via a new host option. The trade-off is extra conversion work and LDS traffic inside the GEMM main loop, plus atomics in the epilogue.

```diff
diff --git a/include/psg_hip.h b/include/psg_hip.h
--- a/include/psg_hip.h
+++ b/include/psg_hip.h
@@ -23,7 +23,7 @@
 
 enum psg_xattn_variant { PSG_XATTN_MFMA = 0, PSG_XATTN_SIMPLE = 1, PSG_XATTN_MFMA_V1 = 2 };
 
-#define PSG_ABI_VERSION 609
+#define PSG_ABI_VERSION 610
 int psg_version(void);
 const char* psg_last_error(void);
 int psg_create(int device, psg_ctx** out);
@@ -266,6 +266,12 @@
 int psg_interleave_gate_up(psg_ctx*, const void* gate_up, void* out, int inter, int K, void* stream);
 int psg_dense_gemm_split(psg_ctx*, const void* x2, const void* w2, const float* bias, int epilogue, float* out, int64_t M,
                          int N, int K2, const float* row_scale, const float* col_scale, int tile, void* stream);
+int psg_dense_gemm_split_a32(psg_ctx*, const float* x, int64_t row_stride, const uint32_t* row_max, const void* w2,
+                             const float* bias, int epilogue, float* out, int64_t M, int N, int K, const float* col_scale,
+                             uint32_t* out_row_max, int tile, void* stream);
+int psg_add_layernorm_rowmax(psg_ctx*, const float* x, const float* residual, int res_period, const int32_t* res_index,
+                             const float* bias, const float* gamma, const float* beta, float eps, int64_t rows, int hidden,
+                             float* out, uint32_t* row_max, void* stream);
 
 int psg_greedy_step(psg_ctx*, const void* logits, int splits, int K, int vocab, int step, int max_new,
                     int eos, int suppress_token, int32_t* tokens, int32_t* done, int32_t* next_ids, int32_t* tok_pos,
diff --git a/openpsg_amd/_lib.py b/openpsg_amd/_lib.py
--- a/openpsg_amd/_lib.py
+++ b/openpsg_amd/_lib.py
@@ -6,7 +6,7 @@
 _HERE = os.path.dirname(os.path.abspath(__file__))
 LIB_PATH = os.path.join(_HERE, "libpsg_hip.so")
 
-PSG_ABI_VERSION = 609
+PSG_ABI_VERSION = 610
 PSG_F32, PSG_BF16, PSG_F16 = 0, 1, 2
 PSG_EMPTY_UNIFORM, PSG_EMPTY_UNMASKED = 0, 1
 PSG_XATTN_MFMA, PSG_XATTN_SIMPLE, PSG_XATTN_MFMA_V1 = 0, 1, 2
@@ -124,6 +124,8 @@
     "psg_dense_gemm_tiled": [_vp, _vp, _vp, _vp, _i, _vp, _i64, _i, _i, _i, _i, _vp, _vp, _i, _vp],
     "psg_interleave_gate_up": [_vp, _vp, _vp, _i, _i, _vp],
     "psg_dense_gemm_split": [_vp, _vp, _vp, _vp, _i, _vp, _i64, _i, _i, _vp, _vp, _i, _vp],
+    "psg_dense_gemm_split_a32": [_vp, _vp, _i64, _vp, _vp, _vp, _i, _vp, _i64, _i, _i, _vp, _vp, _i, _vp],
+    "psg_add_layernorm_rowmax": [_vp, _vp, _vp, _i, _vp, _vp, _vp, _vp, _f, _i64, _i, _vp, _vp, _vp],
     "psg_train_layernorm_fwd": [_vp, _vp, _vp, _vp, _f, _i64, _i, _vp, _vp, _vp, _vp],
     "psg_train_layernorm_bwd": [_vp, _vp, _vp, _vp, _vp, _vp, _i64, _i, _vp, _vp, _vp, _vp],
     "psg_train_rmsnorm_fwd": [_vp, _vp, _vp, _f, _i64, _i, _vp, _vp, _vp],
diff --git a/openpsg_amd/csrc/build.py b/openpsg_amd/csrc/build.py
--- a/openpsg_amd/csrc/build.py
+++ b/openpsg_amd/csrc/build.py
@@ -9,7 +9,7 @@
 PKG = os.path.dirname(HERE)
 LIB = os.path.join(PKG, "libpsg_hip.so")
 SOURCES = ["psg_core.hip", "psg_rowops.hip", "psg_attn.hip", "psg_attn_f32.hip", "psg_xattn_mfma.hip", "psg_xattn_dma.hip", "psg_gemm.hip", "psg_gemm_f32.hip", "psg_batch_gemm.hip", "psg_gemm_w8.hip", "psg_gemm_w4.hip", "psg_gemm_int4.hip", "psg_batch_gemm_q.hip", "psg_expand.hip", "psg_decode_layer.hip", "psg_split.hip", "psg_dense_gemm.hip", "psg_patch_embed.hip", "psg_selfattn_mfma.hip", "psg_prefill_attn_mfma.hip", "psg_pool.hip", "psg_train.hip", "psg_train_bwd.hip", "psg_train_bf16.hip", "psg_tree.hip"]
-HEADERS = ["psg_common.h", "psg_wave.h", "psg_decode_math.h", "psg_train_rows.h", "psg_xattn_tile.h", os.path.join("..", "..", "include", "psg_hip.h")]
+HEADERS = ["psg_common.h", "psg_wave.h", "psg_decode_math.h", "psg_train_rows.h", "psg_xattn_tile.h", "psg_split_scale.h", os.path.join("..", "..", "include", "psg_hip.h")]
 
 
 def _hipcc() -> str:
diff --git a/openpsg_amd/csrc/psg_core.hip b/openpsg_amd/csrc/psg_core.hip
--- a/openpsg_amd/csrc/psg_core.hip
+++ b/openpsg_amd/csrc/psg_core.hip
@@ -46,6 +46,25 @@
     {"llm_fuse_rmsnorm", &psg_opts::llm_fuse_rmsnorm}, {"prefill_attn_scalar", &psg_opts::prefill_attn_scalar},
 };
 
+struct HostOpt {
+  const char* name;
+  int def;
+};
+static const HostOpt kHostOpts[] = {{"split_a32", 1}};
+#define PSG_HOST_OPT_DEVICES 64
+static int g_host_opt[PSG_HOST_OPT_DEVICES][sizeof(kHostOpts) / sizeof(kHostOpts[0])];
+static bool g_host_opt_set[PSG_HOST_OPT_DEVICES][sizeof(kHostOpts) / sizeof(kHostOpts[0])];
+static int* host_opt(psg_ctx* ctx, const char* name, bool** is_set, int* def) {
+  const int dev = ctx->device >= 0 && ctx->device < PSG_HOST_OPT_DEVICES ? ctx->device : 0;
+  for (size_t i = 0; i < sizeof(kHostOpts) / sizeof(kHostOpts[0]); ++i)
+    if (!strcmp(kHostOpts[i].name, name)) {
+      *is_set = &g_host_opt_set[dev][i];
+      *def = kHostOpts[i].def;
+      return &g_host_opt[dev][i];
+    }
+  return nullptr;
+}
+
 static int parse_opt(const char* name, const char* text) {
   int a = 0, b = 0, c = 3;
   if (!strcmp(name, "skinny_dma") && sscanf(text, "%dx%dx%d", &a, &b, &c) >= 2) return a * 100 + b * 10 + c;
@@ -59,6 +78,13 @@
       ctx->opt.*(o.field) = value;
       return PSG_OK;
     }
+  bool* is_set;
+  int def;
+  if (int* h = host_opt(ctx, name, &is_set, &def)) {
+    *h = value;
+    *is_set = true;
+    return PSG_OK;
+  }
   psg_set_error("psg_set_option: unknown option '%s'", name);
   return PSG_ERR_INVALID;
 }
@@ -70,6 +96,12 @@
       *value = ctx->opt.*(o.field);
       return PSG_OK;
     }
+  bool* is_set;
+  int def;
+  if (int* h = host_opt(ctx, name, &is_set, &def)) {
+    *value = *is_set ? *h : def;
+    return PSG_OK;
+  }
   psg_set_error("psg_get_option: unknown option '%s'", name);
   return PSG_ERR_INVALID;
 }
diff --git a/openpsg_amd/csrc/psg_dense_gemm.hip b/openpsg_amd/csrc/psg_dense_gemm.hip
--- a/openpsg_amd/csrc/psg_dense_gemm.hip
+++ b/openpsg_amd/csrc/psg_dense_gemm.hip
@@ -1,4 +1,5 @@
 #include "psg_common.h"
+#include "psg_split_scale.h"
 #include "psg_wave.h"
 
 #define DG_BK 64
@@ -20,11 +21,14 @@
 __global__ void __launch_bounds__(WM * WN * 64, (WM * WN >= 8 ? 2 : 1))
 dense_gemm_kernel(const uint16_t* __restrict__ x, const uint16_t* __restrict__ w, const float* __restrict__ bias,
                   uint16_t* __restrict__ out, int M, int N, int K, const float* __restrict__ row_scale,
-                  const float* __restrict__ col_scale) {
+                  const float* __restrict__ col_scale, int64_t lda, uint32_t* __restrict__ pub_max) {
   using v8 = typename E::v8;
   constexpr int NW = WM * WN, BM = WM * TI * 32, BN = WN * TJ * 32;
   constexpr int A_BYTES = BM * 128, BUF_BYTES = (BM + BN) * 128;
   constexpr int AI = BM / 8 / NW, BI = BN / 8 / NW;
+  constexpr bool A32 = SPL == 2;
+  constexpr int AR = A32 ? BM / 16 / NW : 1;
+  static_assert(!A32 || (OUT32 && BM % (16 * NW) == 0), "fp32 A: fp32 output, tile rows in 16-row passes per wave");
   static_assert(BM % (8 * NW) == 0 && BN % (8 * NW) == 0, "tile rows must split into 8-row DMA instructions per wave");
   constexpr bool GELU = EPI == PSG_EPI_GELU, SWIGLU = EPI == PSG_EPI_SWIGLU;
   static_assert(!(SWIGLU && OUT32), "the SwiGLU epilogue writes the 16-bit activation");
@@ -75,6 +79,69 @@
     }
   };
 
+  const float* x32 = reinterpret_cast<const float*>(x);
+  const uint32_t* rmax = reinterpret_cast<const uint32_t*>(row_scale);
+  const int a_r = lane >> 2, a_kq = lane & 3;
+  static_assert(!A32 || AI == 2 * AR, "fp32 A: a wave converts the rows of its own DMAs");
+  uint32_t amax[AR];
+  float ascale[AR];
+  auto set_scale = [&]() {
+#pragma unroll
+    for (int i = 0; i < AR; ++i) ascale[i] = sp_row_scale(__uint_as_float(amax[i]), nullptr);
+  };
+  auto load_amax = [&](int m0) {
+#pragma unroll
+    for (int i = 0; i < AR; ++i) {
+      int gr = m0 + (wid * AR + i) * 16 + a_r;
+      gr = gr < M ? gr : M - 1;
+      amax[i] = rmax[gr];
+    }
+  };
+  auto stage_a32 = [&](int m0, int kt, int buf) {
+    unsigned char* ab = smem + buf * BUF_BYTES;
+#pragma unroll
+    for (int i = 0; i < AI; ++i) {
+      int gr = m0 + (wid * AI + i) * 8 + srow;
+      gr = gr < M ? gr : M - 1;
+      __builtin_amdgcn_global_load_lds(
+          (const __attribute__((address_space(1))) void*)(x32 + (int64_t)gr * lda + kt * 32 + sslot * 4),
+          (__attribute__((address_space(3))) void*)(ab + (wid * AI + i) * 1024), 16, 0, 0);
+    }
+  };
+  psg_u32x4 raw[AR][2];
+  auto read_raw = [&](int buf) {
+#pragma unroll
+    for (int i = 0; i < AR; ++i) {
+      const uint32_t row = smem_lds + (uint32_t)(buf * BUF_BYTES + ((wid * AR + i) * 16 + a_r) * 128);
+      raw[i][0] = psg_lds_read128(row + (uint32_t)(a_kq * 32));
+      raw[i][1] = psg_lds_read128(row + (uint32_t)(a_kq * 32 + 16));
+    }
+  };
+  auto split_write = [&](int buf) {
+#pragma unroll
+    for (int i = 0; i < AR; ++i) {
+      const int r = (wid * AR + i) * 16 + a_r;
+      const float scale = ascale[i];
+      uint32_t hw[4], lw[4];
+#pragma unroll
+      for (int e = 0; e < 4; ++e) {
+        uint16_t hb[2], lb[2];
+#pragma unroll
+        for (int u = 0; u < 2; ++u) {
+          const float s = __uint_as_float(raw[i][e >> 1][2 * (e & 1) + u]) * scale;
+          hb[u] = f32_to_f16(s);
+          lb[u] = f32_to_f16(s - f16_to_f32(hb[u]));
+        }
+        hw[e] = (uint32_t)hb[0] | ((uint32_t)hb[1] << 16);
+        lw[e] = (uint32_t)lb[0] | ((uint32_t)lb[1] << 16);
+      }
+      const uint32_t row = smem_lds + (uint32_t)(buf * BUF_BYTES + r * 128);
+      const uint32_t swz = (uint32_t)((r >> 1) & 7);
+      psg_lds_write128(row + (((uint32_t)a_kq ^ swz) << 4), (psg_u32x4){hw[0], hw[1], hw[2], hw[3]});
+      psg_lds_write128(row + (((uint32_t)(a_kq + 4) ^ swz) << 4), (psg_u32x4){lw[0], lw[1], lw[2], lw[3]});
+    }
+  };
+
   const int l31 = lane & 31, hi = lane >> 5;
   const int nk = K / DG_BK;
   int t = blockIdx.x, mb, nb;
@@ -84,8 +151,20 @@
     if (mb < MB && nb < NB) break;
   }
   int par = 0;
-  stage_x(mb * BM, 0, 0);
-  stage_w(nb * BN, 0, 0);
+  if constexpr (A32) {
+    load_amax(mb * BM);
+    stage_a32(mb * BM, 0, 0);
+    stage_w(nb * BN, 0, 0);
+    psg_vmwait<BI>();
+    set_scale();
+    read_raw(0);
+    psg_lgkmwait<0>();
+    __builtin_amdgcn_sched_barrier(0);
+    split_write(0);
+  } else {
+    stage_x(mb * BM, 0, 0);
+    stage_w(nb * BN, 0, 0);
+  }
   uint32_t arow[TI], brow[TJ], aswz[TI], bswz[TJ];
 #pragma unroll
   for (int i = 0; i < TI; ++i) {
@@ -157,7 +236,14 @@
         };
         read_frags(0, af[0], bf[0]);
         read_frags(1, af[1], bf[1]);
-        if (pf) stage_x(pm0, pkt, buf ^ 1);
+        if constexpr (A32) {
+          if (pf) {
+            if (!more_k) load_amax(pm0);
+            stage_a32(pm0, pkt, buf ^ 1);
+          }
+        } else {
+          if (pf) stage_x(pm0, pkt, buf ^ 1);
+        }
         psg_lgkmwait<TI + TJ>();
         __builtin_amdgcn_sched_barrier(0);
         __builtin_amdgcn_s_setprio(1);
@@ -180,12 +266,22 @@
         DG_MMA(af[1], bl[1])
         __builtin_amdgcn_sched_barrier(0);
         read_a(3, af[1]);
-        psg_lgkmwait<TI>();
+        if constexpr (A32) {
+          psg_vmwait<BI>();
+          read_raw(buf ^ 1);
+          psg_lgkmwait<TI + 2 * AR>();
+        } else {
+          psg_lgkmwait<TI>();
+        }
         __builtin_amdgcn_sched_barrier(0);
         DG_MMA(af[0], bf[0])
         psg_lgkmwait<0>();
         __builtin_amdgcn_sched_barrier(0);
+        if constexpr (A32) {
+          if (!more_k && pf) set_scale();
+        }
         DG_MMA(af[1], bf[1])
+        if constexpr (A32) split_write(buf ^ 1);
         __builtin_amdgcn_s_setprio(0);
       } else {
       read_frags(0, af[0], bf[0]);
@@ -266,7 +362,9 @@
 #pragma unroll
       for (int i = 0; i < TI; ++i) {
         const int m = m0 + wm * (TI * 32) + i * 32 + l31;
-        const float rs = (row_scale && m < M) ? row_scale[m] : 1.f;
+        float rs = (row_scale && m < M) ? row_scale[m] : 1.f;
+        if constexpr (A32) sp_row_scale(__uint_as_float(rmax[m < M ? m : M - 1]), &rs);
+        float mx = 0.f;
 #pragma unroll
         for (int j = 0; j < TJ; ++j)
 #pragma unroll
@@ -278,9 +376,17 @@
               for (int e = 0; e < 4; ++e) v[e] = dg_gelu(v[e]);
             }
             const int n = cw + j * 32 + 8 * q + 4 * hi;
-            if (m < M && n + 4 <= N)
+            if (m < M && n + 4 <= N) {
               *reinterpret_cast<float4*>(out32 + (int64_t)m * N + n) = make_float4(v[0], v[1], v[2], v[3]);
+              if constexpr (A32) mx = fmaxf(fmaxf(mx, fmaxf(fabsf(v[0]), fabsf(v[1]))), fmaxf(fabsf(v[2]), fabsf(v[3])));
+            }
           }
+        if constexpr (A32) {
+          if (pub_max) {
+            mx = psg_xchg32_max(mx);
+            if (hi == 0 && m < M) atomicMax(pub_max + m, __float_as_uint(mx));
+          }
+        }
       }
     } else {
 #pragma unroll
@@ -330,7 +436,8 @@
 
 template <typename E, int EPI, int VAR, int OUT32, int WM, int WN, int TI, int TJ, int SPL = 0>
 static int dg_launch(psg_ctx* ctx, const void* x, const void* w, const float* bias, void* out, int64_t M, int N, int K,
-                     const float* row_scale, const float* col_scale, void* stream) {
+                     const float* row_scale, const float* col_scale, void* stream, int64_t lda = 0,
+                     uint32_t* pub_max = nullptr) {
   constexpr int BM = WM * TI * 32, BN = WN * TJ * 32;
   const int NB = (N + BN - 1) / BN, MB = (int)((M + BM - 1) / BM);
   const int ntile = MB >= 8 ? (MB + 7) / 8 * 8 * NB : MB * ((NB + 7) / 8 * 8);
@@ -344,7 +451,8 @@
     return PSG_ERR_HIP;
   }
   k<<<(unsigned)grid_i, WM * WN * 64, lds, (hipStream_t)stream>>>((const uint16_t*)x, (const uint16_t*)w, bias,
-                                                                   (uint16_t*)out, (int)M, N, K, row_scale, col_scale);
+                                                                   (uint16_t*)out, (int)M, N, K, row_scale, col_scale, lda,
+                                                                   pub_max);
   PSG_CHECK_LAUNCH("psg_dense_gemm");
   return PSG_OK;
 }
@@ -485,6 +593,49 @@
   return PSG_ERR_INVALID;
 }
 
+extern "C" int psg_dense_gemm_split_a32(psg_ctx* ctx, const float* x, int64_t row_stride, const uint32_t* row_max,
+                                        const void* w2, const float* bias, int epilogue, float* out, int64_t M, int N, int K,
+                                        const float* col_scale, uint32_t* out_row_max, int tile, void* stream) {
+  PSG_REQUIRE(ctx && x && row_max && w2 && out && col_scale, PSG_ERR_INVALID, "psg_dense_gemm_split_a32: NULL argument");
+  PSG_REQUIRE(M >= 0 && N > 0 && K > 0 && M < (1ll << 31), PSG_ERR_INVALID, "psg_dense_gemm_split_a32: M=%lld N=%d K=%d",
+              (long long)M, N, K);
+  PSG_REQUIRE(N % 16 == 0 && K % 32 == 0 && K < (1 << 30), PSG_ERR_UNSUPPORTED,
+              "psg_dense_gemm_split_a32: N=%d must be a multiple of 16 and K=%d of 32", N, K);
+  PSG_REQUIRE(row_stride >= K && row_stride % 4 == 0 && ((uintptr_t)x & 15) == 0, PSG_ERR_UNSUPPORTED,
+              "psg_dense_gemm_split_a32: row_stride=%lld (>= K, a multiple of 4 floats) and x must allow 16-byte loads",
+              (long long)row_stride);
+  PSG_REQUIRE(epilogue == PSG_EPI_NONE || epilogue == PSG_EPI_GELU, PSG_ERR_INVALID, "psg_dense_gemm_split_a32: epilogue=%d",
+              epilogue);
+  if (M == 0) return PSG_OK;
+  if (tile == PSG_TILE_AUTO) tile = dg_auto_tile(ctx, M, N, true);
+  if (out_row_max) {
+    hipError_t e = hipMemsetAsync(out_row_max, 0, (size_t)M * sizeof(uint32_t), (hipStream_t)stream);
+    if (e != hipSuccess) {
+      psg_set_error("psg_dense_gemm_split_a32: hipMemsetAsync: %s", hipGetErrorString(e));
+      return PSG_ERR_HIP;
+    }
+  }
+  const float* rmx = reinterpret_cast<const float*>(row_max);
+#define DGA(WM, WN, TI, TJ)                                                                                             \
+  do {                                                                                                                  \
+    if (epilogue == PSG_EPI_GELU)                                                                                       \
+      return dg_launch<EF16, PSG_EPI_GELU, 0, 1, WM, WN, TI, TJ, 2>(ctx, x, w2, bias, out, M, N, 2 * K, rmx, col_scale, \
+                                                                    stream, row_stride, out_row_max);                  \
+    return dg_launch<EF16, PSG_EPI_NONE, 0, 1, WM, WN, TI, TJ, 2>(ctx, x, w2, bias, out, M, N, 2 * K, rmx, col_scale,   \
+                                                                  stream, row_stride, out_row_max);                    \
+  } while (0)
+  switch (tile) {
+    case PSG_TILE_256x256: DGA(2, 4, 4, 2);
+    case PSG_TILE_256x128: DGA(4, 2, 2, 2);
+    case PSG_TILE_256x64: DGA(8, 1, 1, 2);
+    case PSG_TILE_128x128: DGA(2, 2, 2, 2);
+    default: break;
+  }
+#undef DGA
+  psg_set_error("psg_dense_gemm_split_a32: tile %d (256x256, 256x128, 256x64, 128x128 or auto)", tile);
+  return PSG_ERR_INVALID;
+}
+
 __global__ void __launch_bounds__(256) interleave_gate_up_kernel(const uint16_t* __restrict__ gu, uint16_t* __restrict__ out,
                                                                  int inter, int K) {
   const int orow = blockIdx.x;
diff --git a/openpsg_amd/csrc/psg_rowops.hip b/openpsg_amd/csrc/psg_rowops.hip
--- a/openpsg_amd/csrc/psg_rowops.hip
+++ b/openpsg_amd/csrc/psg_rowops.hip
@@ -84,7 +84,7 @@
 __global__ void add_layernorm_kernel(const T* __restrict__ x, const T* __restrict__ res, const float* __restrict__ bias,
                                      const float* __restrict__ gamma, const float* __restrict__ beta, float eps,
                                      int64_t rows, int hidden, T* __restrict__ out, int res_period,
-                                     const int32_t* __restrict__ res_index) {
+                                     const int32_t* __restrict__ res_index, uint32_t* __restrict__ row_max = nullptr) {
   const int64_t row = ((int64_t)blockIdx.x * blockDim.x + threadIdx.x) >> 6;
   const int lane = threadIdx.x & 63;
   if (row >= rows) return;
@@ -109,6 +109,14 @@
   ln_row<NCH>(v, hidden, eps, gamma, beta, lane);
 #pragma unroll
   for (int c = 0; c < NCH; ++c) Act<T>::st4(out, row * hidden + c * 256 + lane * 4, v[c]);
+  if (row_max) {
+    float mx = 0.f;
+#pragma unroll
+    for (int c = 0; c < NCH; ++c)
+      mx = fmaxf(fmaxf(mx, fmaxf(fabsf(v[c][0]), fabsf(v[c][1]))), fmaxf(fabsf(v[c][2]), fabsf(v[c][3])));
+    mx = wave_max(mx);
+    if (lane == 0) row_max[row] = __float_as_uint(mx);
+  }
 }
 
 template <typename E>
@@ -305,6 +313,22 @@
               "psg_add_layernorm_indexed: group=%d rows=%lld", group, (long long)rows);
   return add_layernorm_launch("psg_add_layernorm_indexed", ctx, x, residual_table, group, block_index, bias, gamma, beta,
                               eps, rows, hidden, out, dtype, stream);
+}
+
+extern "C" int psg_add_layernorm_rowmax(psg_ctx* ctx, const float* x, const float* residual, int res_period,
+                                        const int32_t* res_index, const float* bias, const float* gamma, const float* beta,
+                                        float eps, int64_t rows, int hidden, float* out, uint32_t* row_max, void* stream) {
+  PSG_REQUIRE(ctx && x && gamma && beta && out && row_max, PSG_ERR_INVALID, "psg_add_layernorm_rowmax: NULL argument");
+  PSG_REQUIRE(hidden == 768, PSG_ERR_UNSUPPORTED, "psg_add_layernorm_rowmax: hidden=%d (kernel is built for 768)", hidden);
+  PSG_REQUIRE(rows >= 0 && res_period >= 0 && (!res_index || (res_period > 0 && rows % res_period == 0)) &&
+                  (res_period == 0 || residual),
+              PSG_ERR_INVALID, "psg_add_layernorm_rowmax: res_period=%d rows=%lld", res_period, (long long)rows);
+  if (rows == 0) return PSG_OK;
+  dim3 grid((unsigned)((rows + 3) / 4));
+  add_layernorm_kernel<float, 3><<<grid, 256, 0, (hipStream_t)stream>>>(x, residual, bias, gamma, beta, eps, rows, hidden, out,
+                                                                       res_period, res_index, row_max);
+  PSG_CHECK_LAUNCH("psg_add_layernorm_rowmax");
+  return PSG_OK;
 }
 
 template <typename T>
diff --git a/openpsg_amd/csrc/psg_split.hip b/openpsg_amd/csrc/psg_split.hip
--- a/openpsg_amd/csrc/psg_split.hip
+++ b/openpsg_amd/csrc/psg_split.hip
@@ -1,4 +1,5 @@
 #include "psg_common.h"
+#include "psg_split_scale.h"
 
 #define SP_ORDER_HHL 0
 #define SP_ORDER_HLH 1
@@ -106,7 +107,6 @@
   }
 }
 
-__device__ __forceinline__ float sp_row_scale(float mx, float* inv_scale_out);
 __device__ __forceinline__ void sp_store2(uint16_t* oh, uint16_t* ol, int c, const float (&x)[4], float scale, int wt = 0);
 template <int NCH>
 __global__ void __launch_bounds__(1024) split_f16x2_small_kernel(const float* __restrict__ x, int64_t row_stride, int K,
@@ -190,14 +190,6 @@
 
 #include "psg_decode_math.h"
 
-__device__ __forceinline__ float sp_row_scale(float mx, float* inv_scale_out) {
-  int e = (int)((__float_as_uint(mx) >> 23) & 255u) - 127;
-  if (!(mx > 0.f) || e == 128) e = 13;
-  int se = 127 + 13 - e;
-  se = se < 1 ? 1 : (se > 253 ? 253 : se);
-  if (inv_scale_out) *inv_scale_out = __uint_as_float((uint32_t)(254 - se) << 23);
-  return __uint_as_float((uint32_t)se << 23);
-}
 __device__ __forceinline__ void sp_store2(uint16_t* oh, uint16_t* ol, int c, const float (&x)[4], float scale, int wt);
 __device__ __forceinline__ void sp_store3(uint16_t* o0, int K, int c, const float (&x)[4], float scale) {
   ushort4 h, l;
diff --git a/openpsg_amd/csrc/psg_split_scale.h b/openpsg_amd/csrc/psg_split_scale.h
--- /dev/null
+++ b/openpsg_amd/csrc/psg_split_scale.h
@@ -0,0 +1,11 @@
+#pragma once
+#include <stdint.h>
+
+__device__ __forceinline__ float sp_row_scale(float mx, float* inv_scale_out) {
+  int e = (int)((__float_as_uint(mx) >> 23) & 255u) - 127;
+  if (!(mx > 0.f) || e == 128) e = 13;
+  int se = 127 + 13 - e;
+  se = se < 1 ? 1 : (se > 253 ? 253 : se);
+  if (inv_scale_out) *inv_scale_out = __uint_as_float((uint32_t)(254 - se) << 23);
+  return __uint_as_float((uint32_t)se << 23);
+}
diff --git a/openpsg_amd/csrc/psg_wave.h b/openpsg_amd/csrc/psg_wave.h
--- a/openpsg_amd/csrc/psg_wave.h
+++ b/openpsg_amd/csrc/psg_wave.h
@@ -41,6 +41,9 @@
 __device__ __forceinline__ void psg_lds_write64(uint32_t a, psg_u32x2 v) {
   asm volatile("ds_write_b64 %0, %1" ::"v"(a), "v"(v) : "memory");
 }
+__device__ __forceinline__ void psg_lds_write128(uint32_t a, psg_u32x4 v) {
+  asm volatile("ds_write_b128 %0, %1" ::"v"(a), "v"(v) : "memory");
+}
 __device__ __forceinline__ void psg_lds_write32(uint32_t a, uint32_t v) {
   asm volatile("ds_write_b32 %0, %1" ::"v"(a), "v"(v) : "memory");
 }
diff --git a/openpsg_amd/ops.py b/openpsg_amd/ops.py
--- a/openpsg_amd/ops.py
+++ b/openpsg_amd/ops.py
@@ -1084,6 +1084,40 @@
     return out
 
 
+def dense_gemm_split_a32(x, row_max, w2, bias, col_scale, gelu=False, out=None, tile="auto", out_row_max=None):
+    lib, ctx, st = _env(x)
+    M, K = x.shape
+    N = w2.shape[0]
+    assert x.dtype == torch.float32 and x.stride(1) == 1 and w2.shape[1] == 2 * K and w2.dtype == torch.float16
+    assert row_max.dtype == torch.int32 and row_max.numel() == M
+    out = torch.empty((M, N), device=x.device, dtype=torch.float32) if out is None else out
+    assert out.shape == (M, N) and out.dtype == torch.float32
+    assert out_row_max is None or (out_row_max.dtype == torch.int32 and out_row_max.numel() == M)
+    check(lib.psg_dense_gemm_split_a32(ctx, x.data_ptr(), x.stride(0) if M > 1 else max(x.stride(0), K),
+                                       _p(row_max, torch.int32, "row_max"), _p(w2, name="w2"),
+                                       _p(bias, torch.float32, "bias"), 1 if gelu else 0, _p(out, torch.float32), M, N, K,
+                                       _p(col_scale, torch.float32, "col_scale"), _p(out_row_max, torch.int32, "out_row_max"),
+                                       TILES[tile], st), "psg_dense_gemm_split_a32")
+    return out
+
+
+def add_layernorm_rowmax(x, residual, bias, gamma, beta, eps, row_max, out=None, period=0, index=None):
+    lib, ctx, st = _env(x)
+    out = x if out is None else out
+    rows, hidden = x.shape
+    assert x.dtype == torch.float32 and row_max.dtype == torch.int32 and row_max.numel() == rows
+    if residual is not None:
+        assert residual.dtype == torch.float32 and residual.shape[1] == hidden
+        assert period > 0 or residual.shape[0] == rows
+    if index is not None:
+        assert period > 0 and rows % period == 0 and index.numel() == rows // period
+    check(lib.psg_add_layernorm_rowmax(ctx, _p(x), _p(residual), int(period), _p(index, torch.int32, "index"),
+                                       _p(bias, torch.float32), _p(gamma, torch.float32), _p(beta, torch.float32),
+                                       float(eps), rows, hidden, _p(out, torch.float32), _p(row_max, torch.int32, "row_max"),
+                                       st), "psg_add_layernorm_rowmax")
+    return out
+
+
 def interleave_gate_up(w_gate_up):
     lib, ctx, st = _env(w_gate_up)
     n2, K = w_gate_up.shape
diff --git a/openpsg_amd/qformer.py b/openpsg_amd/qformer.py
--- a/openpsg_amd/qformer.py
+++ b/openpsg_amd/qformer.py
@@ -18,6 +18,7 @@
         self.split = bool(split) and dtype == torch.float32
         self.split_i2 = bool(_lib.get_option(self.device.index or 0, "split_i2")) if self.split else False
         self._split_w, self._bias32 = {}, {}
+        self._rowmax = {}
         self.own_gemm = int(_lib.get_option(self.device.index or 0, "qformer_own_gemm"))
         self.xattn_variant = xattn_variant
         self._xidx_cache = {}
@@ -112,8 +113,39 @@
                 X.copy_(X32)
         return X, X32, shared0
 
+    def _a32(self):
+        return self.split and self.split_i2 and bool(_lib.get_option(self.device.index or 0, "split_a32"))
+
+    def _rowmax_reset(self):
+        self._rowmax.clear()
+
+    def _rowmax_of(self, t):
+        if t.dim() != 2 or t.dtype != torch.float32 or t.stride(1) != 1 or t.shape[0] == 0:
+            return None
+        for start, rows, stride, vec, _ in self._rowmax.get(t.untyped_storage().data_ptr(), ()):
+            off = t.data_ptr() - start
+            if off < 0 or off % (4 * stride) or t.shape[1] != stride or (t.shape[0] > 1 and t.stride(0) != stride):
+                continue
+            r0 = off // (4 * stride)
+            if r0 + t.shape[0] <= rows:
+                return vec[r0:r0 + t.shape[0]]
+        return None
+
+    def _rowmax_for(self, t):
+        vec = self._rowmax_of(t)
+        if vec is None:
+            vec = torch.empty(t.shape[0], device=self.device, dtype=torch.int32)
+            self._rowmax.setdefault(t.untyped_storage().data_ptr(), []).append(
+                (t.data_ptr(), t.shape[0], t.shape[1], vec, t))
+        return vec
+
     def _ln(self, x, r16, r32, bias, ln, out16=None, out32=None, period=0, index=None, want32=True):
         eps = self.cfg.qformer.ln_eps
+        if x.dtype == torch.float32 and x.shape[1] == 768 and self._a32():
+            out = x if out16 is None else out16
+            if out.is_contiguous():
+                return ops.add_layernorm_rowmax(x, r16, bias, ln[0], ln[1], eps, self._rowmax_for(out), out=out,
+                                                period=period, index=index), None
         if self.res32:
             return ops.add_layernorm_res32(x, r32, bias, ln[0], ln[1], eps, out16=out16, out32=out32, period=period,
                                            index=index, want32=want32)
@@ -225,6 +257,8 @@
         else:
             Xn = torch.empty((RQ if last else R, H), device=self.device, dtype=self.dtype)
         Xn32 = torch.empty((Xn.shape[0], H), device=self.device, dtype=torch.float32) if self.res32 else None
+        if not last and self._a32():
+            self._rowmax_for(Xn)
         self._query_tail(li, A[:RQ], self._s(A32, 0, RQ), nq, img, out16=Xn[:RQ], out32=self._s(Xn32, 0, RQ))
         if not last and T > 0:
             self._text_ffn(L, A[RQ:], self._s(A32, RQ), out16=Xn[RQ:], out32=self._s(Xn32, RQ))
@@ -245,6 +279,7 @@
 
     def forward_pairs(self, kv, bits, num_objects, pair_index, ids, text_mask, hidden_out=None, segments=None, mc=None):
         P, T = ids.shape
+        self._rowmax_reset()
         img = (kv, bits, num_objects, pair_index, segments)
         X, X32, shared0 = self._embed(ids)
         for li in range(len(self.layers)):
@@ -261,6 +296,7 @@
 
     def forward_pairs_cls(self, kv, bits, num_objects, pair_index, ids, text_mask, segments=None, prompts=None, mc=None):
         P, T = ids.shape
+        self._rowmax_reset()
         RQ = P * self.cfg.qformer.q_rows
         nl = len(self.layers)
         img = (kv, bits, num_objects, pair_index, segments)
@@ -340,6 +376,7 @@
         nq = self.cfg.qformer.q_rows
         P, T = state["P"], state["T"]
         assert segments is not None or state["segments"] is None, "pair_hidden: pass the slots' segments"
+        self._rowmax_reset()
         xq, xq32, xt, xt32, tix, img = self._state_rows(state, segments)
         s64 = sel.to(torch.int64).clamp(min=0)
         K = s64.numel()
@@ -367,6 +404,7 @@
         nq = self.cfg.qformer.q_rows
         T = state["T"]
         assert state["segments"] is None
+        self._rowmax_reset()
         xq, xq32, xt, xt32, tix, img = self._state_rows(state)
         sel = sel.to(torch.int32).contiguous()
         Xs, tm, pi, mine = ops.gather_pair_rows(xq, xt, tix, state["text_mask"], img[3], sel, first, count, slot_off, nq, T)
@@ -436,6 +474,11 @@
                 ws = self._split_w[key] = ops.split_f16i2(w) if i2 else ops.split_f16x3(w, weights=True)
             tile = self._tile(x.shape[0])
             if i2:
+                rmax = self._rowmax_of(x) if x.stride(0) % 4 == 0 and self._a32() else None
+                if rmax is not None:
+                    out = torch.empty((x.shape[0], N), device=self.device, dtype=torch.float32)
+                    return ops.dense_gemm_split_a32(x, rmax, ws[0], b, ws[1], gelu=gelu, out=out, tile=tile,
+                                                    out_row_max=self._rowmax_for(out) if gelu else None)
                 a2, inv_r = ops.split_f16i2(x)
                 return ops.dense_gemm_split(a2, ws[0], b, inv_r, ws[1], gelu=gelu, tile=tile)
             a3, inv_r = ops.split_f16x3(x)
```

Measured after the change: 18470 pairs/s, median of 6. No clear change (+0.3%).
